# smdogroup/paropt

Hardware: AMD Instinct MI355X
Metric: IP iterations/sec (KKT solve+line search), n=50M vars m=32, 1/2/4/8 GPUs (higher is better)
Workload: dtype f64

## Files before the change

paropt_amd/csrc/capi.cpp:

```cpp
#include <string.h>

#include "ip.hpp"
#include "problem.hpp"
#include "qn.hpp"

namespace po {
const char *last_error();
int ctx_create(int device, Ctx **out);
int ctx_destroy(Ctx *c);
int rccl_unique_id(void *id128);
int comm_init_rccl(Ctx *c, int rank, int size, const void *id128);
int comm_bench(Ctx *c, int count, int pure_sum, int reps, double out_us[3]);
int comm_allreduce_host(Ctx *c, double *values, int count, int op);
int rccl_version();
int comm_init_callback(Ctx *c, int rank, int size, po_allgather_fn fn, void *user);
}

using namespace po;

#define PO_CHECK_PTR(p)                         \
  do {                                          \
    if (!(p)) {                                 \
      po::set_error("null argument: %s", #p);   \
      return PO_ERR_ARG;                        \
// ... 927 lines not shown
  PO_CHECK_PTR(ip);
  return ip->ip->setQuasiNewton(qn ? qn->qn : nullptr);
}
int po_ip_reset_problem_instance(po_ip ip, po_problem prob) {
  PO_CHECK_PTR(ip);
  PO_CHECK_PTR(prob);
  return ip->ip->resetProblemInstance(prob->p);
}
int po_ip_get_hvec_count(po_ip ip, int *nhvec) {
  PO_CHECK_PTR(ip);
  PO_CHECK_PTR(nhvec);
  *nhvec = ip->ip->nhvec;
  return PO_OK;
}
int po_ip_reset_design_and_bounds(po_ip ip) {
  PO_CHECK_PTR(ip);
  return ip->ip->resetDesignAndBounds();
}
int po_ip_reset_quasi_newton(po_ip ip) {
  PO_CHECK_PTR(ip);
  ip->ip->resetQuasiNewtonHessian();
  return PO_OK;
}
int po_ip_get_quasi_newton(po_ip ip, po_qn *qn) {
  PO_CHECK_PTR(ip);
  PO_CHECK_PTR(qn);
  *qn = ip->ip->qn ? &ip->ip->qn_handle : nullptr;
  return PO_OK;
}
int po_ip_write_solution_file(po_ip ip, const char *filename) {
  PO_CHECK_PTR(ip);
  PO_CHECK_PTR(filename);
  return ip->ip->writeSolutionFile(filename);
}
int po_ip_read_solution_file(po_ip ip, const char *filename) {
  PO_CHECK_PTR(ip);
  PO_CHECK_PTR(filename);
  return ip->ip->readSolutionFile(filename);
}
int po_ip_set_iteration_callback(po_ip ip, po_ip_iteration_fn fn, void *user) {
  PO_CHECK_PTR(ip);
  ip->ip->iter_cb = fn;
  ip->ip->iter_cb_user = user;
  return PO_OK;
}
int po_ip_get_history(po_ip ip, const char **text) {
  PO_CHECK_PTR(ip);
  *text = ip->ip->history.c_str();
  return PO_OK;
}
int po_ip_set_callback_timing(po_ip ip, int on) {
  PO_CHECK_PTR(ip);
  ip->ip->user_timing = on != 0;
  return PO_OK;
}
int po_ip_get_phase_times(po_ip ip, const char **names, const double **seconds, int *count) {
  PO_CHECK_PTR(ip);
  InteriorPoint *p = ip->ip;
  p->phase_names_joined.clear();
  for (size_t i = 0; i < p->phase_names.size(); i++) {
    if (i) p->phase_names_joined += ";";
    p->phase_names_joined += p->phase_names[i];
  }
  if (names) *names = p->phase_names_joined.c_str();
  if (seconds) *seconds = p->phase_seconds.data();
  if (count) *count = (int)p->phase_seconds.size();
  return PO_OK;
}
int po_ip_get_debug_ints(po_ip ip, const int **gpiv, int *ngpiv, int *check_flag, int64_t clamped[8]) {
  PO_CHECK_PTR(ip);
  InteriorPoint *p = ip->ip;
  if (gpiv) *gpiv = p->gPivots().data();
  if (ngpiv) *ngpiv = (int)p->gPivots().size();
  if (check_flag) *check_flag = p->checkFlag();
  if (clamped) {
    double out[8];
    PO_TRY(p->clampCounts(out));
    for (int i = 0; i < 8; i++) clamped[i] = (int64_t)(out[i] + 0.5);
  }
  return PO_OK;
}
int po_ip_get_bounds(po_ip ip, po_vec *lb, po_vec *ub) {
  PO_CHECK_PTR(ip);
  if (lb) *lb = static_cast<po_vec>(ip->ip->lowerBounds());
  if (ub) *ub = static_cast<po_vec>(ip->ip->upperBounds());
  return PO_OK;
}
int po_ip_debug_kkt_step(po_ip ip, double mu, po_vec *px, po_vec *pzl, po_vec *pzu,
                         const double **pz, const double **ps, const double **pt,
                         const double **pzs, const double **pzt) {
  PO_CHECK_PTR(ip);
  InteriorPoint *p = ip->ip;
  PO_TRY(p->debugKKTStep(mu));
  if (px) *px = static_cast<po_vec>(p->px);
  if (pzl) *pzl = static_cast<po_vec>(p->pzl);
  if (pzu) *pzu = static_cast<po_vec>(p->pzu);
  if (pz) *pz = p->step.z.data();
  if (ps) *ps = p->step.s.data();
  if (pt) *pt = p->step.t.data();
  if (pzs) *pzs = p->step.zs.data();
  if (pzt) *pzt = p->step.zt.data();
  return PO_OK;
}

int po_ip_debug_set_state(po_ip ip, const double *z, const double *s, const double *t, const double *zs,
                          const double *zt, double mu) {
  PO_CHECK_PTR(ip);
  InteriorPoint *p = ip->ip;
  if (p->c > 0) {
    PO_CHECK_PTR(z);
    PO_CHECK_PTR(s);
    PO_CHECK_PTR(t);
    PO_CHECK_PTR(zs);
    PO_CHECK_PTR(zt);
  }
  return p->debugSetState(z, s, t, zs, zt, mu);
}
int po_ip_debug_kkt(po_ip ip, double mu, int mode, double tau, po_ip_kkt_dump *out) {
  PO_CHECK_PTR(ip);
  PO_CHECK_PTR(out);
  InteriorPoint *p = ip->ip;
  if (mode < 0 || mode > 2) return PO_ERR_ARG;
  PO_TRY(p->debugKKT(mu, mode, tau));
  memset(out, 0, sizeof(*out));
  out->c = p->c;
  out->k = (int)p->cPivots().size();
  out->Dinv = static_cast<po_vec>(p->dinvVec());
  out->res_x = static_cast<po_vec>(p->rxVec());
  out->res_z = p->res.z.data();
  out->res_s = p->res.s.data();
  out->res_t = p->res.t.data();
  out->res_zs = p->res.zs.data();
  out->res_zt = p->res.zt.data();
  for (int i = 0; i < 4; i++) out->res_norms[i] = p->debug_norms[i];
  out->W = p->gramMatrix().data();
  out->G = p->Gmat0.data();
  out->Ce = p->Ce0.data();
  out->gpiv = p->gPivots().data();
  out->cpiv = p->cPivots().data();
  out->px = static_cast<po_vec>(p->px);
  out->pzl = static_cast<po_vec>(p->pzl);
  out->pzu = static_cast<po_vec>(p->pzu);
  out->pz = p->step.z.data();
  out->ps = p->step.s.data();
  out->pt = p->step.t.data();
  out->pzs = p->step.zs.data();
  out->pzt = p->step.zt.data();
  out->step_mins[0] = p->stepMins()[0];
  out->step_mins[1] = p->stepMins()[1];
  return PO_OK;
}

int po_ip_debug_kkt_step_sparse(po_ip ip, po_vec *pzw, po_vec *psw, po_vec *ptw, po_vec *pzsw, po_vec *pztw) {
  PO_CHECK_PTR(ip);
  InteriorPoint *p = ip->ip;
  po_vec *out[5] = {pzw, psw, ptw, pzsw, pztw};
  for (int i = 0; i < 5; i++) {
    if (out[i]) *out[i] = p->has_w ? static_cast<po_vec>(p->wstepv[i]) : nullptr;
  }
  return PO_OK;
}

static int gather_ptrs(po_vec ref, const po_vec *vecs, int nvecs, std::vector<const double *> &p) {
  p.resize(nvecs > 0 ? nvecs : 1);
  for (int j = 0; j < nvecs; j++) {
    PO_CHECK_PTR(vecs[j]);
// ... 128 lines not shown
```

paropt_amd/csrc/context.cpp:

```cpp
#include <dlfcn.h>
#include <math.h>
#include <stdarg.h>
#include <execinfo.h>
#include <stdio.h>
#include <stdlib.h>
#include <string.h>
#include <time.h>

#include <algorithm>

#include "core.hpp"

namespace po {

static thread_local char g_err[1024] = "";
thread_local int g_last_code = 0;

void set_error(const char *fmt, ...) {
  va_list ap;
  va_start(ap, fmt);
  vsnprintf(g_err, sizeof(g_err), fmt, ap);
  va_end(ap);
  fprintf(stderr, "paropt_amd: %s\n", g_err);
}
const char *last_error() { return g_err; }

static int g_dbg_switch[SW_COUNT] = {-1, -1, -1, -1, -1, -1, -1, -1, -1, -1, -1, -1, -1, -1, -1, -1, -1};
double host_now() {
  struct timespec t;
  clock_gettime(CLOCK_MONOTONIC, &t);
  return (double)t.tv_sec + 1e-9 * (double)t.tv_nsec;
}
int dbg_switch(int id, const char *env, int dflt) {
  if (id >= 0 && id < SW_COUNT && g_dbg_switch[id] >= 0) return g_dbg_switch[id];
  const char *e = env ? getenv(env) : nullptr;
  return e ? atoi(e) : dflt;
}
void dbg_switch_set(int id, int value) {
  if (id >= 0 && id < SW_COUNT) g_dbg_switch[id] = value;
}

int launch_reduce_final(Ctx *c, int nblocks, int nslots, int nsum, int nmin, int dst_off);
int launch_reduce_final_multi(Ctx *c, const Ctx::PendingRed *pend, int count);
int launch_red_publish(Ctx *c, const double *src, int count);
static int alloc_h_red(Ctx *c, size_t doubles) {
  if (c->h_red) (void)hipHostFree(c->h_red);
  c->h_red = nullptr;
  c->h_red_dev = nullptr;
  if (hipHostMalloc((void **)&c->h_red, sizeof(double) * doubles, hipHostMallocMapped | hipHostMallocCoherent) !=
      hipSuccess) {
    (void)hipGetLastError();
    c->h_red = nullptr;
    PO_HIP(hipHostMalloc((void **)&c->h_red, sizeof(double) * doubles, hipHostMallocDefault));
    c->h_red_coherent = 0;
  } else {
    c->h_red_coherent = 1;
  }
  if (getenv("PAROPT_AMD_NO_DIRECT_RED") ||
      hipHostGetDevicePointer((void **)&c->h_red_dev, c->h_red, 0) != hipSuccess) {
    (void)hipGetLastError();
    c->h_red_dev = nullptr;
  }
  if (c->h_flag && (!c->h_red_coherent || !c->h_red_dev)) {
    (void)hipHostFree(c->h_flag);
    c->h_flag = c->h_flag_dev = nullptr;
    if (c->d_ticket) (void)hipFree(c->d_ticket);
    c->d_ticket = nullptr;
  }
  if (c->h_red_dev && !c->h_flag && c->h_red_coherent && !getenv("PAROPT_AMD_NO_FLAG_POLL")) {
    if (hipHostMalloc((void **)&c->h_flag, 64, hipHostMallocMapped | hipHostMallocCoherent) == hipSuccess &&
        hipHostGetDevicePointer((void **)&c->h_flag_dev, c->h_flag, 0) == hipSuccess &&
        hipMalloc((void **)&c->d_ticket, sizeof(unsigned)) == hipSuccess &&
        hipMemset(c->d_ticket, 0, sizeof(unsigned)) == hipSuccess) {
      *c->h_flag = 0;
    } else {
      (void)hipGetLastError();
      if (c->h_flag) (void)hipHostFree(c->h_flag);
      if (c->d_ticket) (void)hipFree(c->d_ticket);
      c->h_flag = c->h_flag_dev = nullptr;
      c->d_ticket = nullptr;
    }
  }
  return PO_OK;
}


static int comm_self_test(Ctx *c);
static void free_overflow(Ctx *c, const double *keep);

struct Id128 {
  char b[PO_RCCL_ID_BYTES];
};
struct RcclApi {
  void *handle = nullptr;
  int (*GetUniqueId)(void *) = nullptr;
  int (*CommInitRank)(void **, int, Id128, int) = nullptr;
  int (*AllGather)(const void *, void *, size_t, int, void *, hipStream_t) = nullptr;
  int (*AllReduce)(const void *, void *, size_t, int, int, void *, hipStream_t) = nullptr;
  int (*CommDestroy)(void *) = nullptr;
  const char *(*GetErrorString)(int) = nullptr;
  int (*GetVersion)(int *) = nullptr;
  int version = 0;
};
static RcclApi g_rccl;

static int load_rccl() {
  if (g_rccl.handle) return PO_OK;
  const char *names[] = {getenv("PAROPT_AMD_RCCL_LIB"), "librccl.so", "librccl.so.1", "/opt/rocm/lib/librccl.so"};
  void *h = nullptr;
  for (const char *nm : names) {
// ... 432 lines not shown
  out_us[2] = t.back();
  return PO_OK;
}

int comm_allreduce_host(Ctx *c, double *values, int count, int op) {
  if (count < 0 || count > kMaxRed || op < 0 || op > 2) {
    set_error("po_ctx_allreduce: count %d (max %d) / op %d out of range", count, kMaxRed, op);
    return PO_ERR_ARG;
  }
  if (count == 0 || c->comm_kind == COMM_SELF) return PO_OK;
  PO_TRY(batch_flush(c));
  memcpy(c->h_red, values, sizeof(double) * count);
  PO_HIP(hipMemcpyAsync(c->d_red, c->h_red, sizeof(double) * count, hipMemcpyHostToDevice, c->stream));
  const double *parts = nullptr;
  int nparts = 1;
  PO_TRY(exchange_reduced(c, count, op == 0, &parts, &nparts));
  std::vector<double> out((size_t)count);
  combine_segment(parts, nparts, count, 0, op == 0 ? count : 0, op == 1 ? count : 0, op == 2 ? count : 0, out.data());
  memcpy(values, out.data(), sizeof(double) * count);
  return PO_OK;
}

static void combine_segment(const double *parts, int nparts, int stride, int off, int nsum, int nmin, int nmax,
                            double *host_out) {
  const int nslots = nsum + nmin + nmax;
  for (int s = 0; s < nslots; s++) {
    double acc = parts[off + s];
    for (int r = 1; r < nparts; r++) {
      const double v = parts[(size_t)r * stride + off + s];
      if (s < nsum) {
        acc += v;
      } else if (s < nsum + nmin) {
        acc = fmin(acc, v);
      } else {
        acc = fmax(acc, v);
      }
    }
    host_out[s] = acc;
  }
}

void batch_abort(Ctx *c) {
  if (!c->partials_overflow.empty()) {
    (void)hipStreamSynchronize(c->stream);
    free_overflow(c, nullptr);
  }
  c->batch_pend.clear();
  c->batch_after.clear();
  c->batch_cursor = 0;
  c->partials_cursor = 0;
  c->mdot_timing_pending = false;
}

int batch_flush(Ctx *c, const double *keep_partials, size_t keep_len) {
  size_t cursor0 = 0;
  if (keep_partials && keep_partials >= c->partials_base && keep_partials < c->partials_base + c->partials_cap)
    cursor0 = (size_t)(keep_partials - c->partials_base) + keep_len;
  if (c->batch_pend.empty()) {
    std::vector<std::function<void()>> after;
    after.swap(c->batch_after);
    for (auto &f : after) f();
    return PO_OK;
  }
  std::vector<Ctx::PendingRed> pend;
  pend.swap(c->batch_pend);
  std::vector<std::function<void()>> after;
  after.swap(c->batch_after);
  const int total = c->batch_cursor;
  c->batch_cursor = 0;
  c->partials_cursor = cursor0;
  PO_TRY(launch_reduce_final_multi(c, pend.data(), (int)pend.size()));
  bool pure_sum = true;
  for (const Ctx::PendingRed &p : pend) pure_sum = pure_sum && p.nmin == 0 && p.nmax == 0;
  const double *parts = nullptr;
  int nparts = 1;
  PO_TRY(exchange_reduced(c, total, pure_sum, &parts, &nparts));
  c->n_batched += (long)pend.size() - 1;
  for (const Ctx::PendingRed &p : pend) combine_segment(parts, nparts, total, p.off, p.nsum, p.nmin, p.nmax, p.host_out);
  if (!c->partials_overflow.empty()) free_overflow(c, keep_partials);
  for (auto &f : after) f();
  return PO_OK;
}

int reduce_finish(Ctx *c, int nblocks, int nsum, int nmin, int nmax, double *host_out, bool now) {
  const int nslots = nsum + nmin + nmax;
  if (nslots > kMaxRed) {
    set_error("reduction of %d slots exceeds kMaxRed=%d", nslots, kMaxRed);
    return PO_ERR_ARG;
  }
  const bool queued = c->batch_depth > 0 || !c->batch_pend.empty();
  const double *part = c->d_partials;
  if (queued && c->batch_cursor + nslots > kMaxRed) {
    const size_t len = c->partials_last;
    PO_TRY(batch_flush(c, part, len));
    if (part >= c->partials_base && part < c->partials_base + c->partials_cap) {
      const size_t end = (size_t)(part - c->partials_base) + len;
      if (c->partials_cursor < end) c->partials_cursor = end;
    }
  }
  if (c->batch_depth > 0 || !c->batch_pend.empty()) {
    c->batch_pend.push_back(Ctx::PendingRed{c->batch_cursor, nsum, nmin, nmax, host_out, part, nblocks});
    c->batch_cursor += nslots;
    if (now || c->batch_depth == 0) return batch_flush(c);
    return PO_OK;
  }
  PO_TRY(launch_reduce_final(c, nblocks, nslots, nsum, nmin, 0));
  const double *parts = nullptr;
  int nparts = 1;
  PO_TRY(exchange_reduced(c, nslots, nmin == 0 && nmax == 0, &parts, &nparts));
  combine_segment(parts, nparts, nslots, 0, nsum, nmin, nmax, host_out);
  return PO_OK;
}

}
```

paropt_amd/csrc/core.hpp:

```cpp
#pragma once
#include <hip/hip_runtime.h>
#include <stdint.h>

#include <functional>
#include <string>
#include <vector>

#include "../../include/paropt_amd.h"

namespace po {

void set_error(const char *fmt, ...);
extern thread_local int g_last_code;

#define PO_HIP(expr)                                                                     \
  do {                                                                                   \
    hipError_t _e = (expr);                                                              \
    if (_e != hipSuccess) {                                                              \
      po::set_error("%s failed: %s (%s:%d)", #expr, hipGetErrorString(_e), __FILE__,     \
                    __LINE__);                                                           \
      return PO_ERR_HIP;                                                                 \
    }                                                                                    \
  } while (0)

// ... 15 lines not shown
  hipStream_t stream = nullptr;
  int num_cu = 256;
  int max_blocks = 2048;
  int rank = 0, size = 1;
  CommKind comm_kind = COMM_SELF;
  void *rccl_comm = nullptr;
  int rccl_allreduce = 1;
  long n_allreduce = 0, n_allgather = 0;
  po_allgather_fn cb_allgather = nullptr;
  void *cb_user = nullptr;
  double *d_partials = nullptr;
  double *partials_base = nullptr;
  size_t partials_cap = 0;
  size_t partials_cursor = 0;
  size_t partials_last = 0;
  double *d_red = nullptr;
  double *d_gather = nullptr;
  double *h_red = nullptr;
  double *h_red_dev = nullptr;
  unsigned long long *h_flag = nullptr, *h_flag_dev = nullptr;
  unsigned *d_ticket = nullptr;
  unsigned long long red_seq = 0, red_seq_seen = 0;
  int h_red_coherent = 0;
  long n_flag_waits = 0, n_flag_timeouts = 0;
  bool host_trace = false, host_gap_open = false;
  double host_t_sync = 0.0, host_gap_s = 0.0, host_launch_s = 0.0, host_wait_s = 0.0;
  long host_gap_n = 0, host_launch_n = 0, host_gap_n20 = 0, host_gap_long_n = 0;
  double host_gap_long_s = 0.0, host_t_launch_end = 0.0, host_inter_s = 0.0, host_inter_s30 = 0.0;
  long host_inter_n = 0, host_inter_n30 = 0;
  std::vector<double *> partials_overflow;
  hipEvent_t ev0 = nullptr, ev1 = nullptr;
  double *wide_scratch[2] = {nullptr, nullptr};
  int64_t wide_n = 0;
  hipEvent_t ev_mdot0 = nullptr, ev_mdot1 = nullptr;
  long n_reductions = 0;
  struct PendingRed {
    int off, nsum, nmin, nmax;
    double *host_out;
    const double *part;
    int nblocks;
  };
  int batch_enabled = 1;
  int batch_depth = 0;
  int batch_cursor = 0;
  std::vector<PendingRed> batch_pend;
  std::vector<std::function<void()>> batch_after;
  long n_batched = 0;
  long n_launches = 0;
  double alg_bytes = 0.0, alg_bytes_user = 0.0;
  int in_user = 0;
  int time_mdot_nv = 0;
  double mdot_ms = 0.0;
  long mdot_count = 0;
  bool mdot_timing_pending = false;
  int time_wgram = 0;
  double wgram_ms[2] = {0.0, 0.0};
  long wgram_count[2] = {0, 0};
  int wgram_cols[2] = {0, 0};
  double wgram_bytes[2] = {0.0, 0.0};
};

struct Vec {
  Ctx *ctx;
  int64_t n;
  double *d;
  int ref;
  double *h;
  int h_live = 0;
};

struct PtrTable {
  const double *p[kMaxPanel];
};
struct CoefTable {
  double a[kMaxPanel];
};
constexpr int kMaxVirt = 12;
struct VirtCols {
  const double *s[kMaxVirt];
  int count;
  double b0;
};

int reduce_finish(Ctx *c, int nblocks, int nsum, int nmin, int nmax, double *host_out, bool now = false);
bool red_direct(const Ctx *c);
int batch_flush(Ctx *c, const double *keep_partials = nullptr, size_t keep_len = 0);
void batch_abort(Ctx *c);
template <class F>
inline void after_reduce(Ctx *c, F &&f) {
  if (c->batch_depth > 0 && !c->batch_pend.empty()) {
    c->batch_after.emplace_back(std::forward<F>(f));
  } else {
    f();
  }
}
struct BatchScope {
  Ctx *c;
  bool open;
  explicit BatchScope(Ctx *c_, bool on = true) : c(c_), open(on && c_->batch_enabled) {
    if (open) c->batch_depth++;
  }
  void begin() {
    if (!open && c->batch_enabled) {
      open = true;
      c->batch_depth++;
    }
  }
  int end() {
    if (!open) return PO_OK;
    open = false;
    c->batch_depth--;
    return batch_flush(c);
  }
  int end_nested() {
    if (!open) return PO_OK;
    open = false;
    c->batch_depth--;
    return c->batch_depth > 0 ? PO_OK : batch_flush(c);
  }
  template <class F>
  int end_then(F &&post) {
    if (open) {
      open = false;
      c->batch_depth--;
      if (c->batch_depth > 0) {
        after_reduce(c, std::forward<F>(post));
        return PO_OK;
      }
      PO_TRY(batch_flush(c));
    }
    post();
    return PO_OK;
  }
  ~BatchScope() {
    if (open) {
      c->batch_depth--;
      batch_abort(c);
    }
  }
  BatchScope(const BatchScope &) = delete;
  BatchScope &operator=(const BatchScope &) = delete;
};
enum DbgSwitch { SW_WGRAM_RS = 0, SW_LINCOMB_2D = 1, SW_REDO_DT = 2, SW_LEAN_STEP = 3, SW_WGRAM_PRIO = 4,
                 SW_WGRAM_ABLATE = 5, SW_FUSED_MERIT = 6, SW_REDO_DT1 = 7, SW_BPC3 = 8, SW_BPC4 = 9, SW_LINCOMB_BPC = 10,
                 SW_PERTURB_W = 11, SW_GS_PRODUCER = 12, SW_S2D_TWO = 13, SW_MPC_FUSE = 14, SW_MPC_POLY = 15, SW_SPEC_DT = 16, SW_COUNT = 17 };
int dbg_switch(int id, const char *env, int dflt);
double host_now();
inline double host_trace_begin(Ctx *c);
inline void host_trace_end(Ctx *c, double t0);
void dbg_switch_set(int id, int value);
int ensure_partials(Ctx *c, size_t doubles);
inline double host_trace_begin(Ctx *c) {
  if (!c->host_trace) return 0.0;
  const double t = host_now();
  if (!c->host_gap_open && c->host_t_launch_end > 0.0) {
    const double g = t - c->host_t_launch_end;
    if (g < 500e-6) {
      c->host_inter_s += g;
      c->host_inter_n++;
      if (g > 30e-6) {
        c->host_inter_n30++;
        c->host_inter_s30 += g;
      }
    }
  }
  if (c->host_gap_open) {
    const double g = t - c->host_t_sync;
    if (g < 500e-6) {
      c->host_gap_s += g;
      c->host_gap_n++;
      if (g > 20e-6) c->host_gap_n20++;
    } else {
      c->host_gap_long_s += g;
      c->host_gap_long_n++;
    }
    c->host_gap_open = false;
  }
  return t;
}
inline void host_trace_end(Ctx *c, double t0) {
  if (!c->host_trace) return;
  c->host_t_launch_end = host_now();
  c->host_launch_s += c->host_t_launch_end - t0;
  c->host_launch_n++;
}
inline void count_bytes(Ctx *c, double streams, int64_t n) {
  const double b = 8.0 * streams * (double)n;
  c->alg_bytes += b;
  if (c->in_user) c->alg_bytes_user += b;
}
constexpr int kBpcPanel = 2;
constexpr int kBpcStream = 4;
int grid_for(Ctx *c, int64_t n);
int grid_for(Ctx *c, int64_t n, int bpc);

struct GroupCol {
  const double *w = nullptr;
  double scale = 0.0;
  unsigned period = 1, nw = 0;
  long long nwcon = 0;
};

struct GroupCols2 {
  GroupCol g[2];
  double ca[2] = {0.0, 0.0}, cb[2] = {0.0, 0.0};
  int count = 0;
};

int k_fill(Ctx *c, double *y, int64_t n, double alpha);
int k_fill_hash(Ctx *c, double *y, int64_t n, uint64_t seed, uint64_t aid, int64_t offset,
                double scale, double shift);
int k_copy(Ctx *c, double *y, const double *x, int64_t n);
int k_sign(Ctx *c, double *y, const double *x, int64_t n);
int k_scale(Ctx *c, double *y, int64_t n, double alpha);
int k_axpy(Ctx *c, double *y, double alpha, const double *x, int64_t n);
int k_panel_axpy(Ctx *c, double *y, double a, const double *x, double b, const double *alpha,
                 const double *const *V, int nv, int64_t n, const GroupCol *ybase = nullptr);
int k_panel_axpy2(Ctx *c, double *y1, double a1, const double *x1, const double *c1, double *y2, double a2,
                  const double *x2, const double *c2, const double *const *V, int nv, int64_t n);
int k_panel_lincomb(Ctx *c, double *const *dst, double a, const double *const *X, double b,
                    const double *const *Y, int nv, int64_t n);
enum Red1 { RED_DOT = 0, RED_SUMSQ = 1, RED_ASUM = 2, RED_AMAX = 3 };
int k_reduce1(Ctx *c, int kind, const double *x, const double *y, int64_t n, double *out);
int k_mdot(Ctx *c, const double *x, const double *const *V, int nv, int64_t n, double *out);
int k_minmax(Ctx *c, const double *x, int64_t n, double out[2]);
int k_stream_launch(Ctx *c, int kind, double *x, double *y, int64_t n);
int k_mdot_launch(Ctx *c, const double *x, const double *const *V, int nv, int64_t n, int *nblocks);
struct GramGroups {
  int64_t nwcon = 0, start = 0;
  int nw = 0, skip = 0;
  double alpha = 1.0;
  int ncols = 0;
  double *const *U = nullptr;
};
int k_wgram(Ctx *c, const double *d, const double *const *V, int nv, int64_t n, double *W,
            const double *const *S = nullptr, double *const *Zout = nullptr, int kpend = 0,
            double b0 = 0.0, int preweighted_last = 0, bool may_defer = false,
            const GramGroups *groups = nullptr, bool *groups_done = nullptr);
int wgram_debug_stamps(double out[8]);
int k_wgram_launch(Ctx *c, const double *d, const double *const *V, int nv, int64_t n,
                   int *nblocks, int *nslots, const double *const *S = nullptr,
                   double *const *Zout = nullptr, int kpend = 0, double b0 = 0.0,
                   int preweighted_last = 0, const GramGroups *groups = nullptr, bool *groups_done = nullptr);

struct Bounds {
  const double *x, *lb, *ub, *zl, *zu;
  double max_bound;
  int use_lower, use_upper;
};
int k_kkt_res(Ctx *c, const Bounds &b, const double *g, const double *const *A, const double *z,
              int nc, double beta_mu, int64_t n, double *rx, double *out, double *yqn = nullptr,
              double beta_mu2 = -1.0, const GroupCol *gcol = nullptr, double gcoef = 0.0);
int k_kkt_res_update(Ctx *c, const Bounds &b, const double *g, const double *const *A, const double *z, int nc,
                     double beta_mu, int64_t n, double *rx, double *out, double *yqn, double *zl,
                     const double *pzl, double *zu, const double *pzu, double a, double eps, const double *va,
                     double az, double *acz, double az_acz,
                     const double *pxs = nullptr, const double *xold = nullptr, double beta_mu_step = 0.0,
                     double beta_mu2 = -1.0,
                     const GroupCol *gcol = nullptr, double gcoef = 0.0,
                     double *dinv_out = nullptr, double *t_out = nullptr, double spec_diag = 0.0,
                     double spec_beta_mu = 0.0);
int k_res_norms(Ctx *c, const Bounds &b, double beta_mu, int64_t n, double out[11]);
int k_dinv(Ctx *c, const Bounds &b, double diag, int64_t n, double *dinv,
           const double *hdiag = nullptr);
int k_d1s(Ctx *c, const Bounds &b, const double *bx, const double *dinv, double alpha, double beta_mu,
          int64_t n, double *t);
int k_solve2s(Ctx *c, const Bounds &b, const double *t, const double *dinv, const double *coef,
              const double *const *P, int nv, double alpha, double beta_mu, int full, double tau, int64_t n,
              double *px, double *pzl, double *pzu, double out[2]);
int k_d1(Ctx *c, const Bounds &b, const double *rx, const double *dinv, double beta_mu, int64_t n,
         double *t, const double *cl = nullptr, const double *cu = nullptr);
int k_dinv_d1(Ctx *c, const Bounds &b, double diag, const double *hdiag, const double *rx, double beta_mu,
              int64_t n, double *dinv, double *t, int raw = 0);
int k_corrector(Ctx *c, const Bounds &b, const double *px, const double *pzl, const double *pzu,
                int64_t n, double *cl, double *cu);
constexpr int kCorrDotsMax = 15;
int k_corr_d1_dots(Ctx *c, const Bounds &b, const double *px, const double *pzl, const double *pzu, const double *rx,
                   const double *dinv, double beta_mu, const double *const *V, int nv, int64_t n, double *t,
                   double *out);
int k_solve2c(Ctx *c, const Bounds &b, const double *t, const double *dinv, const double *alpha,
              const double *const *P, int nv, double beta_mu, double tau, int64_t n, double *px, double *pzl,
              double *pzu, double *va, int nca, const double *g, int want_logs, double out[12]);
int k_solve2(Ctx *c, const Bounds &b, const double *t, const double *dinv, const double *alpha,
             const double *const *P, int nv, double beta_mu, int refine, double tau, int64_t n,
             double *px, double *pzl, double *pzu, double out[2], const double *coef2 = nullptr,
             const double *rx = nullptr, double diag = 0.0, double *tout = nullptr,
             double *va = nullptr, int nca = 0, const double *cl = nullptr,
             const double *cu = nullptr);
int k_solve2_dots(Ctx *c, const Bounds &b, const double *t, const double *dinv, const double *alpha,
                  const double *coef2, const double *const *P, int nv, double beta_mu, double tau,
                  const double *rx, double diag, int64_t n, double *px, double *pzl, double *pzu,
                  double *tout, double *va, int nca, double *out, double *traw = nullptr,
                  int store_step = 1,
                  int ca0 = 0,
                  const double *const *vs = nullptr, int nvirt = 0, double b0v = 0.0,
                  double dinv_diag = 0.0,
                  const GroupCols2 *gcols = nullptr);
int k_solve2r(Ctx *c, const Bounds &b, const double *t1, const double *t2, const double *dinv, const double *a1,
              const double *a2, const double *const *P, int nv, double beta_mu, double tau, int64_t n, double *px,
              double *pzl, double *pzu, double *va, int nca, double out[2], const double *ar = nullptr,
              const double *rx = nullptr, double diag = 0.0,
              int ca0 = 0,
              const double *const *vs = nullptr, int nvirt = 0, double b0v = 0.0,
              const double *g = nullptr, double *merit_out = nullptr,
              double dinv_diag = 0.0,
              const GroupCol *gcol = nullptr, double gc1 = 0.0, double gc2 = 0.0);
int k_form_pz(Ctx *c, const Bounds &b, const double *px, double beta_mu, int64_t n, double *pzl, double *pzu);
int k_update_mult_yqn(Ctx *c, double *zl, const double *pzl, double *zu, const double *pzu, double a,
                      double eps, int use_lower, int use_upper, const double *rx, const double *va,
                      double az, int64_t n, double *yqn, double *acz = nullptr);
int k_res_step(Ctx *c, const Bounds &b, const double *rx, const double *px, const double *pzl,
               const double *pzu, const double *dinv, const double *coef, const double *const *P,
               int nv, double diag, double beta_mu, int64_t n, double *tprime);
int k_step_check(Ctx *c, const Bounds &b, const double *rx, const double *px, const double *pzl, const double *pzu,
                 const double *coef, const double *const *P, int nv, double diag, double beta_mu, int64_t n,
                 double out[3]);
int k_comp_step(Ctx *c, const Bounds &b, const double *px, const double *pzl, const double *pzu,
                double ax, double az, int64_t n, double out[2]);
int k_comp_merit(Ctx *c, const Bounds &b, const double *px, const double *pzl, const double *pzu, double ax,
                 double az, const double *g, int64_t n, double out[9]);
int k_merit0(Ctx *c, const Bounds &b, const double *px, double sx, const double *g, int64_t n,
             double out[6]);
int k_trial(Ctx *c, const Bounds &b, const double *px, double a, double eps, int64_t n, double *xt,
            double out[2], double *sout = nullptr);
int k_update_mult(Ctx *c, double *zl, const double *pzl, double *zu, const double *pzu, double a,
                  double eps, int use_lower, int use_upper, int64_t n);
int k_affine_mult(Ctx *c, const Bounds &b, double *zl, const double *pzl, double *zu,
                  const double *pzu, double amin, int64_t n);
int k_check_bounds(Ctx *c, double *x, double *lb, double *ub, double *zl, double *zu,
                   double max_bound, double rel_bound, int both, int64_t n, int *flag);
int k_bounds_mode(Ctx *c, double *x, double *lb, double *ub, int mode, int64_t offset, int64_t n);
int k_clamp_count(Ctx *c, const double *x, const double *lb, const double *ub, const double *zl, const double *zu,
                  double eps, int64_t n, double out[4]);
int k_zero_inactive(Ctx *c, const double *lb, const double *ub, double *zl, double *zu,
                    double max_bound, int64_t n);

int k_quadratic_f(Ctx *c, const double *q, const double *b, const double *x, int64_t n, double *f);
int k_quadratic_g(Ctx *c, const double *q, const double *b, const double *x, int64_t n, double *g);
int k_convex_f(Ctx *c, const double *b, const double *x, int64_t n, double *f);
int k_convex_g(Ctx *c, const double *b, const double *x, int64_t n, double *g);
int k_rosen_f(Ctx *c, const double *x, int64_t n, double out[3]);
int k_rosen_g(Ctx *c, const double *x, int64_t n, double *g, double *a0, double *a1);
int k_sep_hess(Ctx *c, int kind, const double *q, const double *b, const double *x, const double *px,
               int64_t n, double *h);
int k_rosen_hess(Ctx *c, const double *x, double z0, const double *px, int64_t n, double *h);

int lu_factor(int n, double *A, int lda, int *piv);
void lu_solve(int n, const double *A, int lda, const int *piv, double *b);

}

struct po_ctx_s : po::Ctx {};
struct po_vec_s : po::Vec {};
```

paropt_amd/csrc/ip.cpp:

```cpp
#include "ip.hpp"

#include <math.h>
#include <stdio.h>
#include <stdlib.h>
#include <string.h>

#include <algorithm>
#include <chrono>

namespace po {

static const int LS_SUCCESS = 1, LS_FAILURE = 2, LS_MIN_STEP = 4, LS_MAX_ITERS = 8,
                 LS_NO_IMPROVEMENT = 16, LS_SHORT_STEP = 32;

InteriorPoint::InteriorPoint(Problem *p)
    : prob(p), ctx(p->ctx), n(p->nlocal), c(p->ncon), qn(nullptr), x(nullptr), zl(nullptr),
      zu(nullptr), lb(nullptr), ub(nullptr), g(nullptr), fobj(0.0), barrier_param(0.1),
      rho_penalty_search(0.0), niter(0), neval(0), ngeval(0), analytic_panel_dots(true),
      iter_cb(nullptr),
      iter_cb_user(nullptr), px(nullptr), pzl(nullptr), pzu(nullptr), Dinv(nullptr), rx(nullptr),
      tvec(nullptr), xt(nullptr), y_qn(nullptr), s_qn(nullptr), vA(nullptr), qn_created(false), qn_owned(true), wk(0),
      comp_prod(0), comp_count(0), max_rx(0), max_rzl(0), max_rzu(0), sx(1.0), sz(1.0),
      ptpx_valid(false), residual_fused(false), residual_cached(false), corrector_active(false),
      norm_type(0), tdots_valid(false), fused_dots(true), phase_t0(0) {
// ... 68 lines not shown
    vec_decref(wresv[i]);
    vec_decref(wstepv[i]);
    vec_decref(wscalev[i]);
  }
  for (Vec *v : Uw) vec_decref(v);
  for (Vec *v : gmresW) vec_decref(v);
  vec_decref(hdiag);
  if (qn_owned) delete qn;
  if (user_events_ready)
    for (int i = 0; i < 2 * kUserRing; i++) (void)hipEventDestroy(user_ev[i]);
}

void InteriorPoint::setPenaltyGamma(double gamma) {
  if (gamma < 0.0) return;
  gamma_s.assign(c, gamma);
  gamma_t.assign(c, gamma);
  for (int i = 0; i < c && i < prob->ninequality; i++) gamma_s[i] = 0.0;
  if (has_w) k_w_gamma(ctx, gsw->d, gtw->d, gamma, prob->nwinequality, nw);
}

int InteriorPoint::setQuasiNewton(CompactQuasiNewton *qn_) {
  if (qn_owned) delete qn;
  qn = qn_;
  qn_owned = false;
  qn_created = true;
  qn_handle.qn = qn;
  return PO_OK;
}

int InteriorPoint::resetProblemInstance(Problem *p) {
  if (p->nlocal != prob->nlocal || p->ncon != prob->ncon || p->nwcon != prob->nwcon ||
      p->ninequality != prob->ninequality || p->nwinequality != prob->nwinequality) {
    set_error("ParOpt: Incompatible problem instance");
    return PO_ERR_ARG;
  }
  prob = p;
  ac_valid = false;
  acz_valid = false;
  cwx_valid = false;
  return PO_OK;
}

void InteriorPoint::setPenaltyGammaArray(const double *gamma) {
  for (int i = 0; i < c; i++) {
    if (gamma[i] >= 0.0) {
      gamma_s[i] = i < prob->ninequality ? 0.0 : gamma[i];
      gamma_t[i] = gamma[i];
    }
  }
}

int InteriorPoint::createQuasiNewton() {
  if (qn_created) return PO_OK;
  qn_created = true;
  const std::string qt = options.str("qn_type");
  const int msub = options.integer("qn_subspace_size");
  if (qt == "bfgs") {
    LBFGS *b = new LBFGS(ctx, n, msub);
    b->setBFGSUpdateType(std::string(options.str("qn_update_type")) == "damped_update"
                             ? PO_BFGS_DAMPED_UPDATE
                             : PO_BFGS_SKIP_NEGATIVE_CURVATURE);
    qn = b;
  } else if (qt == "sr1") {
    qn = new LSR1(ctx, n, msub);
  }
  if (qn) {
    const std::string dt = options.str("qn_diag_type");
    qn->setInitDiagonalType(dt == "yts_over_sts" ? PO_QN_YTS_OVER_STS : PO_QN_YTY_OVER_YTS);
  }
  qn_handle.qn = qn;
  return PO_OK;
}

Bounds InteriorPoint::bounds() const {
  Bounds b;
  b.x = x->d;
  b.lb = lb->d;
  b.ub = ub->d;
  b.zl = zl->d;
  b.zu = zu->d;
  b.max_bound = options.real("max_bound_value");
  b.use_lower = use_lower;
  b.use_upper = use_upper;
  return b;
}

std::vector<const double *> InteriorPoint::panel(bool use_qn, int *k) const {
  std::vector<const double *> p;
  for (Vec *a : Ac) p.push_back(a->d);
  *k = 0;
  if (qn && use_qn) {
    std::vector<const double *> z = qn->zPointers();
    *k = (int)z.size();
    p.insert(p.end(), z.begin(), z.end());
  }
  return p;
}

void InteriorPoint::phaseBegin() {
  phase_t0 = std::chrono::duration<double>(std::chrono::steady_clock::now().time_since_epoch()).count();
}
void InteriorPoint::phaseEnd(const char *name) {
  const double t1 =
      std::chrono::duration<double>(std::chrono::steady_clock::now().time_since_epoch()).count();
  for (size_t i = 0; i < phase_names.size(); i++) {
    if (phase_names[i] == name) {
      phase_seconds[i] += t1 - phase_t0;
      phase_t0 = t1;
      return;
    }
  }
  phase_names.push_back(name);
  phase_seconds.push_back(t1 - phase_t0);
  phase_t0 = t1;
}

void InteriorPoint::userBegin() {
  ctx->in_user = 1;
  if (!user_timing) return;
  if (!user_events_ready) {
    for (int i = 0; i < 2 * kUserRing; i++)
      if (hipEventCreate(&user_ev[i]) != hipSuccess) return;
    user_events_ready = true;
  }
  if (user_pending == kUserRing) userHarvest();
  (void)hipEventRecord(user_ev[2 * user_pending], ctx->stream);
}
void InteriorPoint::userEnd() {
  ctx->in_user = 0;
  if (!user_timing || !user_events_ready) return;
  (void)hipEventRecord(user_ev[2 * user_pending + 1], ctx->stream);
  user_pending++;
}
void InteriorPoint::userHarvest() {
  for (int i = 0; i < user_pending; i++) {
    float ms = 0.0f;
    if (hipEventSynchronize(user_ev[2 * i + 1]) == hipSuccess &&
        hipEventElapsedTime(&ms, user_ev[2 * i], user_ev[2 * i + 1]) == hipSuccess)
      user_seconds += 1e-3 * ms;
  }
  user_pending = 0;
}

int InteriorPoint::initAndCheckDesignAndBounds() {
  int rc = prob->getVarsAndBounds(x, lb, ub);
  if (rc != 0) {
    set_error("getVarsAndBounds failed with code %d", rc);
    return PO_ERR_USER;
  }
  const double rel_bound = 0.001 * barrier_param;
  int flag = 0;
  PO_TRY(k_check_bounds(ctx, x->d, lb->d, ub->d, zl->d, zu->d, options.real("max_bound_value"),
                        rel_bound, use_lower && use_upper, n, &flag));
  check_flag |= flag;
  if (ctx->rank == 0) {
    if (flag & 1) history += "ParOpt Warning: Variable bounds are inconsistent\n";
    if (flag & 2) history += "ParOpt Warning: Variables may be too close to lower bound\n";
    if (flag & 4) history += "ParOpt Warning: Variables may be too close to upper bound\n";
  }
  return PO_OK;
}

int InteriorPoint::clampCounts(double out[8]) {
  const double eps = options.real("design_precision");
  PO_TRY(k_clamp_count(ctx, x->d, lb->d, ub->d, use_lower ? zl->d : nullptr, use_upper ? zu->d : nullptr, eps, n,
                       out));
  for (int j = 4; j < 8; j++) out[j] = 0.0;
  for (int i = 0; i < c; i++) {
    if (vars.s[i] == eps) out[4] += 1.0;
    if (vars.t[i] == eps) out[5] += 1.0;
    if (vars.zs[i] == eps) out[6] += 1.0;
    if (vars.zt[i] == eps) out[7] += 1.0;
  }
  return PO_OK;
}

static int refreshLiveMirror(Vec *v) {
  if (!v || !v->h_live || !v->h || v->n <= 0) return PO_OK;
  PO_HIP(hipMemcpyAsync(v->h, v->d, sizeof(double) * (size_t)v->n, hipMemcpyDeviceToHost, v->ctx->stream));
  PO_HIP(hipStreamSynchronize(v->ctx->stream));
  return PO_OK;
}

int InteriorPoint::resetDesignAndBounds() {
  cwx_valid = false;
  int rc = prob->getVarsAndBounds(x, lb, ub);
  if (rc != 0) return PO_ERR_USER;
  PO_TRY(refreshLiveMirror(x));
  PO_TRY(refreshLiveMirror(lb));
  return refreshLiveMirror(ub);
}

void InteriorPoint::resetQuasiNewtonHessian() {
  if (qn) qn->reset();
}

int InteriorPoint::initLeastSquaresMultipliers() {
  acz_valid = false;
  const double mu0 = options.real("init_barrier_param");
  PO_TRY(k_fill(ctx, zl->d, n, mu0));
  PO_TRY(k_fill(ctx, zu->d, n, mu0));
  for (int i = 0; i < c; i++) vars.z[i] = vars.s[i] = vars.t[i] = vars.zs[i] = vars.zt[i] = mu0;
  PO_TRY(k_zero_inactive(ctx, lb->d, ub->d, zl->d, zu->d, options.real("max_bound_value"), n));
  if (has_w) return initLeastSquaresMultipliersW();
  if (c == 0) return PO_OK;
  const double small = 1e-4;
  PO_TRY(k_fill(ctx, Dinv->d, n, 1.0));
  int k = 0;
  std::vector<const double *> A = panel(false, &k);
  std::vector<double> G((size_t)c * c, 0.0);
  PO_TRY(k_wgram(ctx, Dinv->d, A.data(), c, n, G.data()));
  for (int i = 0; i < c; i++) G[(size_t)i * (c + 1)] += small;
  std::vector<int> piv(c);
  lu_factor(c, G.data(), c, piv.data());
  const double al[2] = {1.0, -1.0};
  const double *vv[2] = {zl->d, zu->d};
  PO_TRY(k_panel_axpy(ctx, tvec->d, -1.0, g->d, 0.0, al, vv, 2, n));
  std::vector<double> z(c, 0.0);
  PO_TRY(k_mdot(ctx, tvec->d, A.data(), c, n, z.data()));
  for (int i = 0; i < c; i++) z[i] = -z[i];
  lu_solve(c, G.data(), c, piv.data(), z.data());
  for (int i = 0; i < c; i++) {
    const double gam = 10.0 * std::max(gamma_s[i], gamma_t[i]);
    vars.z[i] = (z[i] < -gam || z[i] > gam) ? 0.0 : z[i];
  }
  return PO_OK;
}

int InteriorPoint::initAffineStepMultipliers() {
  const double amin = options.real("start_affine_multiplier_min");
  PO_TRY(initLeastSquaresMultipliers());
  PO_TRY(k_zero_inactive(ctx, lb->d, ub->d, zl->d, zu->d, options.real("max_bound_value"), n));
  PO_TRY(computeResidual(0.0, true));
  bool use_qn = !(options.integer("sequential_linear_method") ||
                  !options.integer("use_qn_gmres_precon") || options.integer("use_diag_hessian"));
  if (options.integer("use_diag_hessian")) PO_TRY(ensureHdiag());
  PO_TRY(setUpKKTSystem(use_qn));
  denseResidual(0.0, res);
  if (has_w) {
    PO_TRY(solveKKTW(res, 0.0, use_qn, false, 1.0, step));
    PO_TRY(k_w_affine(ctx, wv(), wp(), amin, nw));
  } else {
    PO_TRY(solveKKT(res, 0.0, use_qn, false, 1.0, step));
  }
  acz_valid = false;
  for (int i = 0; i < c; i++) {
    vars.z[i] = vars.z[i] + step.z[i];
    vars.s[i] = std::max(amin, fabs(vars.s[i] + step.s[i]));
    vars.t[i] = std::max(amin, fabs(vars.t[i] + step.t[i]));
    vars.zs[i] = std::max(amin, fabs(vars.zs[i] + step.zs[i]));
    vars.zt[i] = std::max(amin, fabs(vars.zt[i] + step.zt[i]));
  }
  PO_TRY(k_affine_mult(ctx, bounds(), zl->d, pzl->d, zu->d, pzu->d, amin, n));
  double comp = 0.0;
  PO_TRY(getComplementarity(&comp));
  barrier_param = comp;
  return PO_OK;
}

void InteriorPoint::denseResidual(double mu, Dense &r) const {
  for (int i = 0; i < c; i++) {
    r.z[i] = -(cvals[i] - vars.s[i] + vars.t[i]);
    r.s[i] = -(gamma_s[i] - vars.zs[i] + vars.z[i]);
    r.t[i] = -(gamma_t[i] - vars.zt[i] - vars.z[i]);
    r.zs[i] = -(vars.s[i] * vars.zs[i] - mu);
    r.zt[i] = -(vars.t[i] * vars.zt[i] - mu);
  }
}
// ... 607 lines not shown
    r2.resize(c);
    denseResidual(mu, r2);
    for (int i = 0; i < c; i++) {
      r2.z[i] -= (dots[i] - step.s[i] + step.t[i]);
      r2.s[i] += (step.zs[i] - step.z[i]);
      r2.t[i] += (step.zt[i] + step.z[i]);
      r2.zs[i] -= (step.s[i] * vars.zs[i] + vars.s[i] * step.zs[i]);
      r2.zt[i] -= (step.t[i] * vars.zt[i] + vars.t[i] * step.zt[i]);
    }
    PO_TRY(solveKKT(r2, mu, use_qn, true, tau, refine));
    for (int i = 0; i < c; i++) {
      step.z[i] += refine.z[i];
      step.s[i] += refine.s[i];
      step.t[i] += refine.t[i];
      step.zs[i] += refine.zs[i];
      step.zt[i] += refine.zt[i];
    }
  }
  sx = sz = 1.0;
  return PO_OK;
}

int InteriorPoint::checkKKTStep(int iteration, double mu) {
  const double beta_mu = options.real("rel_bound_barrier") * mu;
  if (!pz_stored) {
    PO_TRY(k_form_pz(ctx, bounds(), px->d, step_beta_mu, n, pzl->d, pzu->d));
    pz_stored = true;
  }
  const bool seq_lin = options.integer("sequential_linear_method");
  int kq = 0;
  std::vector<const double *> Pq = panel(qn && !seq_lin, &kq);
  const int mq = c + kq;
  std::vector<double> dots(mq > 0 ? mq : 1, 0.0), coef(mq > 0 ? mq : 1, 0.0);
  if (mq > 0) PO_TRY(k_mdot(ctx, px->d, Pq.data(), mq, n, dots.data()));
  for (int i = 0; i < c; i++) coef[i] = step.z[i];
  double diag = options.real("qn_sigma");
  if (qn && !seq_lin && !options.integer("use_diag_hessian")) {
    diag += qn->diag();
    if (kq > 0) {
      std::vector<double> rz(dots.begin() + c, dots.begin() + c + kq);
      qn->applyCompactInverse(rz.data());
      for (int j = 0; j < kq; j++) coef[c + j] = rz[j];
    }
  }
  if (has_w) {
    if (prob->setSparseJacobianTranspose(1.0, x, wstepv[0], xt) != 0) return PO_ERR_USER;
    Pq.push_back(xt->d);
    coef.push_back(1.0);
  }
  double mx[3];
  PO_TRY(computeResidual(mu, true));
  PO_TRY(k_step_check(ctx, bounds(), rx->d, px->d, pzl->d, pzu->d, coef.data(), Pq.data(), (int)Pq.size(), diag,
                      beta_mu, n, mx));
  Dense r;
  r.resize(c);
  denseResidual(mu, r);
  double mz = 0.0, ms = 0.0, mt = 0.0, mzs = 0.0, mzt = 0.0;
  for (int i = 0; i < c; i++) {
    mz = std::max(mz, fabs(r.z[i] - (dots[i] - step.s[i] + step.t[i])));
    ms = std::max(ms, fabs(r.s[i] + (step.zs[i] - step.z[i])));
    mt = std::max(mt, fabs(r.t[i] + (step.zt[i] + step.z[i])));
    mzs = std::max(mzs, fabs(r.zs[i] - (step.s[i] * vars.zs[i] + vars.s[i] * step.zs[i])));
    mzt = std::max(mzt, fabs(r.zt[i] - (step.t[i] * vars.zt[i] + vars.t[i] * step.zt[i])));
  }
  if (ctx->rank == 0) {
    char line[640];
    snprintf(line, sizeof(line),
             "\nResidual step check for iteration %d:\n"
             "max |stationarity (x block)|:             %10.4e\n"
             "max |dense constraints (z block)|:        %10.4e\n"
             "max |slack duals (s block)|:              %10.4e\n"
             "max |slack duals (t block)|:              %10.4e\n"
             "max |slack complementarity (zs block)|:   %10.4e\n"
             "max |slack complementarity (zt block)|:   %10.4e\n"
             "max |lower-bound complementarity (zl)|:   %10.4e\n"
             "max |upper-bound complementarity (zu)|:   %10.4e\n",
             iteration, mx[0], mz, ms, mt, mzs, mzt, mx[1], mx[2]);
    history += line;
  }
  return PO_OK;
}

int InteriorPoint::checkGradients(double dh, std::string *report) {
  return prob->checkGradients(dh, x, options.integer("use_hvec_product"), xt, tvec, report);
}

int InteriorPoint::checkMeritFuncGradient(Vec *xpt, double dh, double out[2]) {
  if (xpt) PO_TRY(k_copy(ctx, x->d, xpt->d, n));
  cwx_valid = false;
  if (prob->evalObjCon(x, &fobj, cvals.data()) != 0) {
    fprintf(stderr, "ParOpt: Function and constraint evaluation failed\n");
    return PO_ERR_USER;
  }
  neval++;
  if (prob->evalObjConGradient(x, g, Ac.data()) != 0) {
    fprintf(stderr, "ParOpt: Gradient evaluation failed\n");
    return PO_ERR_USER;
  }
  ngeval++;
  ac_valid = true;
  acz_valid = false;
  if (!pz_stored) {
    pz_stored = true;
  }
  if (xpt) {
    double g2 = 0.0;
    PO_TRY(k_reduce1(ctx, RED_SUMSQ, g->d, nullptr, n, &g2));
    PO_TRY(k_panel_axpy(ctx, px->d, g2 > 0.0 ? -1.0 / sqrt(g2) : 0.0, g->d, 0.0, nullptr, nullptr, 0, n));
    for (int i = 0; i < c; i++) {
      step.s[i] = -0.259 * (1 + (i % 3));
      step.t[i] = -0.349 * (4 - (i % 2));
    }
    if (has_w && nw > 0) {
      std::vector<double> hs((size_t)nw), ht((size_t)nw);
      for (int64_t i = 0; i < nw; i++) {
        hs[i] = -0.419 * (1 + (i % 5));
        ht[i] = -0.7513 * (1 + (i % 19));
      }
      PO_HIP(hipMemcpyAsync(wstepv[1]->d, hs.data(), sizeof(double) * (size_t)nw, hipMemcpyHostToDevice, ctx->stream));
      PO_HIP(hipMemcpyAsync(wstepv[2]->d, ht.data(), sizeof(double) * (size_t)nw, hipMemcpyHostToDevice, ctx->stream));
      PO_HIP(hipStreamSynchronize(ctx->stream));
    }
  }
  sx = sz = 1.0;
  ptpx_valid = false;
  merit_cache_valid = false;
  fused_merit_valid = false;
  w_comp_valid = w_merit_cache_valid = false;
  px_amax_valid = false;
  double m0 = 0.0, dm0 = 0.0;
  PO_TRY(evalMeritInitDeriv(1.0, &m0, &dm0));
  const double eps = 0.0;
  double sums[2], wsums[5];
  std::vector<double> rs(c), rt(c), cs(cvals);
  for (int i = 0; i < c; i++) {
    rs[i] = vars.s[i] + dh * step.s[i];
    rt[i] = vars.t[i] + dh * step.t[i];
  }
  {
    PO_TRY(k_trial(ctx, bounds(), px->d, dh, eps, n, xt->d, sums));
    trial_logs_valid = false;
    s_qn_from_trial = false;
  }
  double ftemp = 0.0;
  if (prob->evalObjCon(xt, &ftemp, cs.data()) != 0) {
    fprintf(stderr, "ParOpt: Function and constraint evaluation failed\n");
    return PO_ERR_USER;
  }
  neval++;
  if (has_w) {
    if (prob->evalSparseCon(xt, wtmp) != 0) return PO_ERR_USER;
    PO_TRY(k_w_trial(ctx, wv(), wp(), dh, eps, gsw->d, gtw->d, wtmp->d, nw, wsums));
  }
  const double m1 = evalMeritFromSums(ftemp, cs.data(), rs.data(), rt.data(), sums[0], sums[1], has_w ? wsums : nullptr);
  const double fd = (m1 - m0) / dh;
  if (ctx->rank == 0) {
    fprintf(stdout, "Merit function test\n");
    fprintf(stdout, "dm FD: %15.8e  Actual: %15.8e  Err: %8.2e  Rel err: %8.2e\n", fd, dm0, fabs(fd - dm0),
            fabs((fd - dm0) / fd));
    fflush(stdout);
  }
  if (out) {
    out[0] = fd;
    out[1] = dm0;
  }
  return PO_OK;
// ... 757 lines not shown
  const bool seq_lin = options.integer("sequential_linear_method");
  const double min_frac = options.real("min_fraction_to_boundary");
  const bool use_line_search = options.integer("use_line_search");
  const int write_freq = options.integer("write_output_frequency");
  const int step_verification_frequency = options.integer("step_verification_frequency");
  const int gradient_verification_frequency = options.integer("gradient_verification_frequency");
  const std::string start = options.str("starting_point_strategy");
  niter = neval = ngeval = nhvec = 0;
  cwx_valid = trial_cw_valid = false;
  residual_cached = false;
  iterate_logs_valid = trial_logs_valid = fused_merit_valid = false;
  spec_dt_valid = spec_dt_want = false;
  w_comp_valid = w_merit_cache_valid = false;
  px_first_only = false;
  spec_enabled = spec_valid = false;
  history.clear();
  phase_names.clear();
  phase_seconds.clear();
  user_seconds = 0.0;
  user_pending = 0;
  ac_valid = false;
  acz_valid = false;
  if (!seq_lin && !qn && !use_diag_hessian) {
    if (ctx->rank == 0)
      fprintf(stderr,
              "ParOpt Error: Must use a sequential linear method if no quasi-Newton approximation "
              "is defined\n");
    return 1;
  }
  phaseBegin();
  PO_TRY(initAndCheckDesignAndBounds());
  userBegin();
  int fail_obj = prob->evalObjCon(x, &fobj, cvals.data());
  userEnd();
  neval++;
  if (fail_obj) {
    fprintf(stderr, "ParOpt: Initial function and constraint evaluation failed\n");
    return fail_obj;
  }
  userBegin();
  int fail_g = prob->evalObjConGradient(x, g, Ac.data());
  userEnd();
  ngeval++;
  if (fail_g) {
    fprintf(stderr, "ParOpt: Initial gradient evaluation failed\n");
    return fail_g;
  }
  ac_valid = true;
  if (start == "affine_step") {
    PO_TRY(initAffineStepMultipliers());
  } else if (start == "least_squares_multipliers") {
    PO_TRY(initLeastSquaresMultipliers());
  }
  if (qn && !use_qnu) {
    if (qn->updateMult(x, vars.z.data(), has_w ? wvar[0] : nullptr) != 0) return PO_ERR_USER;
  }
  phaseEnd("init");

  double fobj_prev = 0.0, alpha_prev = 0.0, alpha_xprev = 0.0, alpha_zprev = 0.0, dm0_prev = 0.0;
  double res_norm_prev = 0.0;
  int no_merit_function_improvement = 0, line_search_test = 0, line_search_failed = 0;
  char info[64];
  memset(info, 0, sizeof(info));
  char line[512];

  for (int k = 0; k < max_major_iters; k++, niter++) {
    int qn_hessian_reset = 0;
    if (qn && !seq_lin) {
      if (k > 0 && k % hessian_reset_freq == 0 && use_qnu) {
        qn->reset();
        qn_hessian_reset = 1;
      }
    }
    if (write_freq > 0 && k % write_freq == 0) {
      if (checkpoint) {
        if (writeSolutionFile(checkpoint) != PO_OK) checkpoint = nullptr;
      }
      prob->writeOutput(k, x);
    }
    if (iter_cb) iter_cb(iter_cb_user, k);
    if (gradient_verification_frequency > 0 && (k % gradient_verification_frequency) == 0) {
      std::string rep;
      PO_TRY(prob->checkGradients(options.real("gradient_check_step_length"), x, use_hvec_product, xt, tvec, &rep));
      if (ctx->rank == 0) history += rep;
    }

    const bool rel_function_test =
        (alpha_xprev == 1.0 && alpha_zprev == 1.0 && (fabs(fobj - fobj_prev) < rel_func_tol * fabs(fobj_prev)));
    if (no_merit_function_improvement) {
      line_search_test += 1;
    } else {
      line_search_test = 0;
    }
    double max_prime = 0.0, max_dual = 0.0, max_infeas = 0.0, res_norm = 0.0;
    int monotone_barrier_converged = 0;
    double comp = 0.0;
    spec_enabled = barrier_strategy == B_MONOTONE && norm_type == 0 && !has_w && !use_hvec_product;
    if (barrier_strategy == B_MONOTONE) {
      if (!residual_cached) PO_TRY(computeResidual(barrier_param, true));
      residual_cached = false;
      comp = compFromSums(comp_prod, comp_count, vars, w_sums[0]);
      denseResidual(barrier_param, res);
      resNorms(res, &max_prime, &max_dual, &max_infeas, &res_norm);
      if (k > 0 && ((res_norm < 10.0 * barrier_param) || rel_function_test || (line_search_test >= 2))) {
        monotone_barrier_converged = 1;
      }
      if (monotone_barrier_converged) {
        if (barrier_param > 0.1 * abs_res_tol) line_search_test = 0;
        const double mu_frac = options.real("monotone_barrier_fraction") * barrier_param;
        const double mu_pow = pow(barrier_param, options.real("monotone_barrier_power"));
        double new_mu = mu_frac;
        if (mu_pow < mu_frac) new_mu = mu_pow;
        if (new_mu < 0.1 * abs_res_tol) new_mu = 0.09999 * abs_res_tol;
        if (spec_valid && spec_mu == new_mu && norm_type == 0) {
          max_rzl = spec_max[0];
          max_rzu = spec_max[1];
          spec_valid = false;
        } else {
          PO_TRY(computeResidual(new_mu, false));
        }
        denseResidual(new_mu, res);
        resNorms(res, &max_prime, &max_dual, &max_infeas, &res_norm);
        rho_penalty_search = options.real("min_rho_penalty_search");
        barrier_param = new_mu;
      }
    } else if (barrier_strategy == B_MEHROTRA || barrier_strategy == B_MPC) {
      if (!residual_cached) PO_TRY(computeResidual(barrier_param, true));
      residual_cached = false;
      comp = compFromSums(comp_prod, comp_count, vars, w_sums[0]);
      denseResidual(barrier_param, res);
      resNorms(res, &max_prime, &max_dual, &max_infeas, &res_norm);
    } else {
      if (!residual_cached) PO_TRY(computeResidual(barrier_param, true));
      residual_cached = false;
      comp = compFromSums(comp_prod, comp_count, vars, w_sums[0]);
      barrier_param = options.real("monotone_barrier_fraction") * comp;
      if (barrier_param < 0.1 * abs_res_tol) barrier_param = 0.1 * abs_res_tol;
      PO_TRY(computeResidual(barrier_param, false));
      denseResidual(barrier_param, res);
      resNorms(res, &max_prime, &max_dual, &max_infeas, &res_norm);
    }
    phaseEnd("residual");

    if (ctx->rank == 0) {
      if (k == 0 || options.integer("output_level") > 0) {
        const char *inform = prob->sparseFactorInfo();
        if (inform) history += std::string("MatInfo: ") + inform + "\n";
      }
      if (k % 10 == 0) {
        snprintf(line, sizeof(line),
                 "\n%4s %4s %4s %4s %7s %7s %7s %12s %7s %7s %7s %7s %7s %8s %7s info\n", "iter",
                 "nobj", "ngrd", "nhvc", "alpha", "alphx", "alphz", "fobj", "|opt|", "|infes|",
                 "|dual|", "mu", "comp", "dmerit", "rho");
        history += line;
      }
      if (k == 0) {
        snprintf(line, sizeof(line),
                 "%4d %4d %4d %4d %7s %7s %7s %12.5e %7.1e %7.1e %7.1e %7.1e %7.1e %8s %7s %s\n", k,
                 neval, ngeval, nhvec, "--", "--", "--", fobj, max_prime, max_infeas, max_dual,
                 barrier_param, comp, "--", "--", info);
      } else {
        snprintf(line, sizeof(line),
                 "%4d %4d %4d %4d %7.1e %7.1e %7.1e %12.5e %7.1e %7.1e %7.1e %7.1e %7.1e %8.1e %7.1e %s\n",
                 k, neval, ngeval, nhvec, alpha_prev, alpha_xprev, alpha_zprev, fobj, max_prime,
                 max_infeas, max_dual, barrier_param, comp, dm0_prev, rho_penalty_search, info);
      }
// ... 389 lines not shown
```

paropt_amd/csrc/ip.hpp:

```cpp
#pragma once
#include <stdlib.h>
#include <map>
#include <string>
#include <vector>

#include "problem.hpp"
#include "qn.hpp"

namespace po {

class Options {
 public:
  enum Type { STR = 1, BOOL = 2, INT = 3, FLOAT = 4, ENUM = 5 };
  struct Entry {
    Type type;
    std::string s;
    int i = 0, ilo = 0, ihi = 0;
    double f = 0, flo = 0, fhi = 0;
    std::vector<std::string> choices;
  };
  Options();
  void addTrustRegionDefaults();
  void addMMADefaults();
  int set(const char *name, const char *value);
  int set(const char *name, int value);
  int set(const char *name, double value);
  const char *str(const char *name) const;
  int integer(const char *name) const;
  double real(const char *name) const;
  bool has(const char *name) const { return e.count(name) > 0; }
  int visit(const Options *skip, po_option_visitor fn, void *user) const;
  void adoptExtras(const Options &src, const Options &base);

 private:
  std::map<std::string, Entry> e;
};

struct Dense {
  std::vector<double> z, s, t, zs, zt;
  void resize(int c) {
    z.assign(c, 0.0);
    s.assign(c, 0.0);
    t.assign(c, 0.0);
    zs.assign(c, 0.0);
    zt.assign(c, 0.0);
  }
};

class InteriorPoint {
 public:
  InteriorPoint(Problem *prob);
  ~InteriorPoint();
  int allocate();
  const std::vector<int> &gPivots() const { return gpiv; }
  Vec *lowerBounds() { return lb; }
  Vec *upperBounds() { return ub; }
  int checkFlag() const { return check_flag; }
  int clampCounts(double out[8]);
  int checkKKTStep(int iteration, double mu);

  Options options;
  int optimize(const char *checkpoint);
  void getOptimizedPoint(Vec **x, const double **z, Vec **zl, Vec **zu);
  void getOptimizedSlacks(const double **s, const double **t, const double **zs, const double **zt);
  void getOptimizedSparse(Vec *v[5]);
  void getIterationCounters(int *niter_, int *neval_, int *ngeval_);
  double getBarrierParameter() const { return barrier_param; }
  int getComplementarity(double *comp);
  void setPenaltyGamma(double gamma);
  void setPenaltyGammaArray(const double *gamma);
  int resetDesignAndBounds();
  void resetQuasiNewtonHessian();
  int setQuasiNewton(CompactQuasiNewton *qn_);
  int resetProblemInstance(Problem *p);
  int writeSolutionFile(const char *filename);
  int readSolutionFile(const char *filename);
  int debugKKTStep(double mu);
  int debugSetState(const double *z, const double *s, const double *t, const double *zs, const double *zt, double mu);
  int debugKKT(double mu, int mode, double tau);
  std::vector<double> Gmat0, Ce0;
  bool debug_keep_schur = false;
  double debug_norms[4] = {0, 0, 0, 0};
  const std::vector<double> &gramMatrix() const { return W; }
  const std::vector<int> &cPivots() const { return cpiv; }
  const double *stepMins() const { return step_mins; }
  Vec *dinvVec() { return Dinv; }
  Vec *rxVec() { return rx; }
  void flushHistory();
  int checkGradients(double dh, std::string *report);
  int checkMeritFuncGradient(Vec *xpt, double dh, double out[2]);

  Problem *prob;
  Ctx *ctx;
  int64_t n;
  int c;
  CompactQuasiNewton *qn;
  po_qn_s qn_handle;

  Vec *x, *zl, *zu, *lb, *ub, *g;
  std::vector<Vec *> Ac;
  Dense vars, res, step, refine;
  double fobj, barrier_param, rho_penalty_search;
  std::vector<double> cvals;
  int niter, neval, ngeval, nhvec;

  bool analytic_panel_dots;
  po_ip_iteration_fn iter_cb;
  void *iter_cb_user;
  std::string history;
  std::vector<std::string> phase_names;
  std::vector<double> phase_seconds;
  std::string phase_names_joined;
  bool user_timing = getenv("PAROPT_AMD_USER_TIMING") != nullptr;

  Vec *px, *pzl, *pzu;

  int64_t nw;
  bool has_w;
  double nw_global;
  Vec *wvar[5], *wresv[5], *wstepv[5];

 private:
  Vec *Dinv, *rx, *tvec, *xt, *y_qn, *s_qn;
  Vec *vA;
  std::vector<double> gamma_s, gamma_t;
  int use_lower, use_upper;
  bool qn_created;
  bool qn_owned;

  std::vector<double> W;
  int wk;
  std::vector<double> Gf, Cef;
  std::vector<int> gpiv, cpiv;
  double comp_prod, comp_count, max_rx, max_rzl, max_rzu;
  double l1_rx = 0, l1_rzl = 0, l1_rzu = 0, l2_rx = 0, l2_rzl = 0, l2_rzu = 0;
  double sx, sz;
  double step_mins[2];
  std::vector<double> ptpx;
  bool ptpx_valid;
// ... 27 lines not shown
  double trial_logs[2] = {0, 0}, iterate_logs[2] = {0, 0};
  bool trial_logs_valid = false, iterate_logs_valid = false;
  int gatherCounts(int64_t mine, std::vector<int64_t> *all);
  int solutionFileOffsets(int64_t *nvars_total, int64_t *var_off, int64_t *nw_total, int64_t *w_off);
  int ensureHdiag();
  int solveKKTAlpha(const double *bx, double alpha, const Dense &b, double mu, bool use_qn, bool full,
                    double tau, Dense &out);
  int evalObjBarrierDeriv(const Dense &p, double *pmerit);
  int solveKKTAlphaW(const double *bx, double alpha, const Dense &b, double mu, bool use_qn, bool full,
                     double tau, Dense &out);
  Vec *wscalev[5];
  double w_merit_last[10];
  int computeKKTGMRESStep(double rtol, double atol, bool use_qn, double tau, int *gmres_iters);

  Vec *gsw, *gtw, *Cw, *wd2, *wyw, *wtmp, *wtmp2;
  Vec *cwx = nullptr;
  bool cwx_valid = false, trial_cw_valid = false;
  int sparseConAtIterate(const double **cw);
  Vec *d1v;
  std::vector<Vec *> Uw;
  bool panel_plain = false;
  bool panel_valid = false;
  double w_sums[7], w_maxs[5];
  double res_out[13] = {0}, wres_out[12] = {0};
  bool spec_mu_on = true, spec_enabled = false, spec_valid = false;
  double spec_mu = 0.0, spec_max[2] = {0.0, 0.0};
  double nextMonotoneMu() const;
  WVars wv() const;
  WVars wr() const;
  WVars wp() const;
  int allocateW();
  int applyK0(const double *bx, const double *bw, Vec *yx, Vec *yw);
  int computeResidualW(double mu, bool norms = true, bool with_d2 = false);
  bool wd2_ready = false;
  int sparseGramCorrection(const std::vector<const double *> &P, int m, Vec *work = nullptr, bool may_defer = false,
                           bool panel_done = false);
  int panelImageVectors(int m, std::vector<double *> &U);
  int solveKKTW(const Dense &b, double mu, bool use_qn, bool refine_pass, double tau, Dense &out,
                bool fuse_residual = false);
  int computeKKTStepWithRefinementW(double mu, bool use_qn, double tau);
  int initLeastSquaresMultipliersW();
  int wCompStep(double ax, double az, double *prod);

  Bounds bounds() const;
  std::vector<const double *> panel(bool use_qn, int *k) const;

  int createQuasiNewton();
  int initAndCheckDesignAndBounds();
  int initLeastSquaresMultipliers();
  int initAffineStepMultipliers();
  void denseResidual(double mu, Dense &r) const;
  struct MultUpdate {
    double a = 0.0, az = 0.0, eps = 0.0;
    bool acz_follow = false;
  };
  int computeResidual(double mu, bool vectors, Vec *yqn_complete = nullptr, const MultUpdate *upd = nullptr);
  void resNorms(const Dense &r, double *max_prime, double *max_dual, double *max_infeas,
                double *res_norm) const;
  double compFromSums(double prod, double count, const Dense &v, double wprod = 0.0) const;
  int setUpKKTSystem(bool use_qn, bool diag_only = false, const double *rhs_mu = nullptr);
  int solveKKT(const Dense &b, double mu, bool use_qn, bool refine_pass, double tau, Dense &out,
               bool fuse_residual = false);
  int computeKKTStepWithRefinement(double mu, bool use_qn, double tau);
  int mehrotraStep(bool use_qn, double comp, bool corrector, double min_frac, double abs_res_tol, double *tau_out);
  int scaleKKTStep(double tau, double comp, double *alpha_x, double *alpha_z, int *ceq,
                   bool inexact = false);
  int evalMeritInitDeriv(double max_x, double *merit, double *pmerit);
  double evalMeritFromSums(double fk, const double *ck, const double *sk, const double *tk,
                           double pos, double neg, const double *wsums = nullptr) const;
  int lineSearch(double alpha_min, double *alpha, double m0, double dm0, int *fail);
  int computeStepAndUpdate(double alpha, int eval_obj_con, int perform_qn_update, int *update_type);
  void phaseBegin();
  void phaseEnd(const char *name);
  double phase_t0;
  static const int kUserRing = 16;
  hipEvent_t user_ev[2 * kUserRing];
  int user_pending = 0;
  bool user_events_ready = false;
  double user_seconds = 0.0;
  void userBegin();
  void userEnd();
  void userHarvest();
  int check_flag = 0;
  bool ac_valid = false;
  static const int kAczRefresh = 16;
  Vec *acz = nullptr;
  bool acz_valid = false, use_acz = true, use_ztpx_hint = true;
  int acz_age = 0;
  bool fuse_mult_update = true;
  bool fast_yqn_w = true;
  bool w_lean = true, px_first_only = false;
  double w_step_out[5] = {0, 0, 0, 0, 0}, w_comp_poly[3] = {0, 0, 0}, w_merit_cache[10] = {0};
  bool w_comp_valid = false, w_merit_cache_valid = false;
  bool s_qn_from_trial = false;
  double s_qn_a = 0.0;
  bool recompute_first_step = true, step_deferred = false;
  std::vector<double> alpha_first, coef_first;
  double diag_first = 0.0;
  bool recompute_rhs = true;
  bool virtual_z = true, virt_first = false, allow_virtual_z = false;
  bool fused_tdots = true, t0_valid = false;
  double t0_mu = 0.0;
  std::vector<double> t0dots;
};

}

struct po_ip_s {
  po::InteriorPoint *ip;
};
```

paropt_amd/csrc/kernels.hip:

```cpp
#include "core.hpp"

#include <math.h>
#include <stdlib.h>

namespace po {

#define PO_PAIR_LOOP(q, n)                                                                 \
  const int64_t _npairs = ((n) + 1) >> 1;                                                  \
  for (int64_t q = (int64_t)blockIdx.x * blockDim.x + threadIdx.x; q < _npairs;            \
       q += (int64_t)gridDim.x * blockDim.x)

typedef double f64x2l __attribute__((ext_vector_type(2)));
__device__ __forceinline__ double2 ld2(const double *__restrict__ p, int64_t q, int64_t n) {
#ifndef PO_LD2_PLAIN
  const f64x2l v = __builtin_nontemporal_load(reinterpret_cast<const f64x2l *>(p + 2 * q));
  return make_double2(v.x, v.y);
#else
  return *reinterpret_cast<const double2 *>(p + 2 * q);
#endif
}
#ifndef PO_ST2_PLAIN
#define PO_ST2_NT 1
#endif
typedef double f64x2s __attribute__((ext_vector_type(2)));
__device__ __forceinline__ void st2(double *__restrict__ p, int64_t q, int64_t n, double2 v) {
  if (2 * q + 1 >= n) v.y = 0.0;
#ifdef PO_ST2_NT
  __builtin_nontemporal_store((f64x2s){v.x, v.y}, reinterpret_cast<f64x2s *>(p + 2 * q));
#else
  *reinterpret_cast<double2 *>(p + 2 * q) = v;
#endif
}

typedef double f64x4 __attribute__((ext_vector_type(4)));
typedef double f64x2 __attribute__((ext_vector_type(2)));

__device__ __forceinline__ f64x2 ld_stream(const double *p) {
  return __builtin_nontemporal_load(reinterpret_cast<const f64x2 *>(p));
}

enum { OP_SUM = 0, OP_MIN = 1, OP_MAX = 2 };

template <int OP>
__device__ __forceinline__ double combine(double a, double b) {
  if (OP == OP_SUM) return a + b;
  if (OP == OP_MIN) return fmin(a, b);
  return fmax(a, b);
}

template <int OP>
__device__ __forceinline__ double wave_reduce(double v) {
#pragma unroll
  for (int o = 32; o > 0; o >>= 1) v = combine<OP>(v, __shfl_xor(v, o, 64));
  return v;
}

template <int N, int OP>
__device__ __forceinline__ void block_reduce_store(double (&a)[N], double *__restrict__ partials,
                                                   int slot0, double *sm) {
  const int lane = threadIdx.x & 63, wave = threadIdx.x >> 6;
#pragma unroll
  for (int j = 0; j < N; j++) {
    double v = wave_reduce<OP>(a[j]);
    if (lane == 0) sm[wave * N + j] = v;
  }
  __syncthreads();
  if (threadIdx.x < N) {
    const int j = threadIdx.x;
    double v = combine<OP>(combine<OP>(sm[j], sm[N + j]), combine<OP>(sm[2 * N + j], sm[3 * N + j]));
    partials[(size_t)(slot0 + j) * gridDim.x + blockIdx.x] = v;
  }
  __syncthreads();
}

__device__ __forceinline__ void red_raise_flag(volatile unsigned long long *flag, unsigned long long seq,
                                               unsigned *ticket) {
  if (!flag) return;
  __threadfence_system();
  __syncthreads();
  if (threadIdx.x == 0) {
    const unsigned t = atomicAdd(ticket, 1u);
    if (t == gridDim.x - 1) {
      *ticket = 0;
      __threadfence_system();
      *flag = seq;
    }
// ... 702 lines not shown
    set_error("mdot of %d vectors exceeds kMaxPanel=%d", nv, kMaxPanel);
    return PO_ERR_ARG;
  }
  const int grid = grid_for(c, n, 5);
  PO_TRY(ensure_partials(c, (size_t)grid * (nv + 32)));
  PtrTable pt;
  CoefTable ct;
  fill_tables(nullptr, V, nv, &ct, &pt);
  int j0 = 0;
  while (j0 < nv) {
    const int rem = nv - j0;
    const int w = rem >= 32 ? 32 : (rem >= 24 ? 24 : (rem >= 16 ? 16 : rem));
    switch (w) {
      PO_MDOT_CASE(1) PO_MDOT_CASE(2) PO_MDOT_CASE(3) PO_MDOT_CASE(4) PO_MDOT_CASE(5)
      PO_MDOT_CASE(6) PO_MDOT_CASE(7) PO_MDOT_CASE(8) PO_MDOT_CASE(9) PO_MDOT_CASE(10)
      PO_MDOT_CASE(11) PO_MDOT_CASE(12) PO_MDOT_CASE(13) PO_MDOT_CASE(14) PO_MDOT_CASE(15)
      PO_MDOT_CASE(16) PO_MDOT_CASE(24) PO_MDOT_CASE(32)
    }
    j0 += w;
  }
  *nblocks = grid;
  return PO_OK;
}

int k_mdot(Ctx *c, const double *x, const double *const *V, int nv, int64_t n, double *out) {
  if (nv <= 0) return PO_OK;
  if (nv > kMaxPanel) {
    for (int j0 = 0; j0 < nv; j0 += kMaxPanel)
      PO_TRY(k_mdot(c, x, V + j0, nv - j0 > kMaxPanel ? kMaxPanel : nv - j0, n, out + j0));
    return PO_OK;
  }
  int grid = 0;
  const bool timed = c->time_mdot_nv == nv;
  if (timed && c->mdot_timing_pending) PO_TRY(batch_flush(c));
  if (timed) PO_HIP(hipEventRecord(c->ev_mdot0, c->stream));
  PO_TRY(k_mdot_launch(c, x, V, nv, n, &grid));
  if (timed) PO_HIP(hipEventRecord(c->ev_mdot1, c->stream));
  const bool defer = timed && c->batch_depth > 0;
  PO_TRY(reduce_finish(c, grid, nv, 0, 0, out, timed && !defer));
  if (timed) {
    auto harvest = [c] {
      float ms = 0.0f;
      if (hipEventSynchronize(c->ev_mdot1) == hipSuccess &&
          hipEventElapsedTime(&ms, c->ev_mdot0, c->ev_mdot1) == hipSuccess) {
        c->mdot_ms += ms;
        c->mdot_count++;
      }
      c->mdot_timing_pending = false;
    };
    if (defer) c->mdot_timing_pending = true;
    after_reduce(c, harvest);
  }
  return PO_OK;
}


struct BE {
  bool L, U;
  double xl, xu, zl, zu;
};
__device__ __forceinline__ BE bound_elem(double x, double lb, double ub, double zl, double zu,
                                         double maxb, int use_lower, int use_upper) {
  BE e;
  e.L = use_lower && (lb > -maxb);
  e.U = use_upper && (ub < maxb);
  e.xl = e.L ? (x - lb) : 1.0;
  e.xu = e.U ? (ub - x) : 1.0;
  e.zl = zl;
  e.zu = zu;
  return e;
}
#define PO_MAKE_BOUNDS(b, q, n)                                                          \
  const bool _has2 = (2 * q + 1 < n);                                                    \
  const BE e0 = bound_elem(_x.x, _lb.x, _ub.x, _zl.x, _zu.x, (b).max_bound, (b).use_lower, \
                           (b).use_upper);                                               \
  BE e1 = bound_elem(_x.y, _lb.y, _ub.y, _zl.y, _zu.y, (b).max_bound, (b).use_lower,     \
                     (b).use_upper);                                                     \
  if (!_has2) {                                                                          \
    e1.L = false;                                                                        \
    e1.U = false;                                                                        \
    e1.xl = 1.0;                                                                         \
    e1.xu = 1.0;                                                                         \
  }
#define PO_LOAD_BOUNDS(b, q, n)                                                         \
  const double2 _x = ld2((b).x, q, n), _lb = ld2((b).lb, q, n), _ub = ld2((b).ub, q, n), \
                _zl = ld2((b).zl, q, n), _zu = ld2((b).zu, q, n);                        \
  PO_MAKE_BOUNDS(b, q, n)

__device__ __forceinline__ void res_bound_acc(const BE &e, double beta_mu, double *sums, double *maxs,
                                              int il1, int il2, int imax) {
  if (e.L) {
    sums[0] += e.zl * e.xl;
    sums[1] += 1.0;
    const double r = fabs(-(e.xl * e.zl - beta_mu));
    sums[il1] += r;
    sums[il2] += r * r;
    maxs[imax] = fmax(maxs[imax], r);
  }
  if (e.U) {
    sums[0] += e.zu * e.xu;
    sums[1] += 1.0;
    const double r = fabs(-(e.xu * e.zu - beta_mu));
    sums[il1 + 1] += r;
    sums[il2 + 1] += r * r;
    maxs[imax + 1] = fmax(maxs[imax + 1], r);
  }
}
__device__ __forceinline__ void res_bound_max2(const BE &e, double beta_mu2, double *m2) {
  if (e.L) m2[0] = fmax(m2[0], fabs(-(e.xl * e.zl - beta_mu2)));
  if (e.U) m2[1] = fmax(m2[1], fabs(-(e.xu * e.zu - beta_mu2)));
}
__global__ void __launch_bounds__(kBlock)
    kkt_res_kernel(Bounds b, const double *__restrict__ g, PtrTable A, CoefTable z, int nc,
                   double beta_mu, int64_t n, double *__restrict__ rx, double *__restrict__ yqn,
                   double beta_mu2, GroupCol gcol, double gcoef, double *__restrict__ partials) {
  __shared__ double sm[4 * 8];
  double sums[8] = {0.0, 0.0, 0.0, 0.0, 0.0, 0.0, 0.0, 0.0};
  double maxs[5] = {0.0, 0.0, 0.0, 0.0, 0.0};
  PO_PAIR_LOOP(q, n) {
    PO_LOAD_BOUNDS(b, q, n);
    const double2 gv = ld2(g, q, n);
    double2 yv = make_double2(0.0, 0.0);
    if (yqn) yv = ld2(yqn, q, n);
    double2 r;
    r.x = (b.use_lower ? _zl.x : 0.0);
    r.y = (b.use_lower ? _zl.y : 0.0);
    if (b.use_upper) {
      r.x += -1.0 * _zu.x;
      r.y += -1.0 * _zu.y;
    }
    r.x += -1.0 * gv.x;
    r.y += -1.0 * gv.y;
    GRaw graw;
    if (gcol.w) graw = gcol_request(gcol, q, n);
    double2 ps = panel_sum(A, z, nc, q);
    if (gcol.w) {
      const f64x2 gcv = gcol_value(gcol, graw);
      ps.x += gcoef * gcv.x;
      ps.y += gcoef * gcv.y;
    }
    r.x += ps.x;
    r.y += ps.y;
    if (!_has2) r.y = 0.0;
    st2(rx, q, n, r);
    if (yqn) {
      const double cl = b.use_lower ? 1.0 : 0.0, cu = b.use_upper ? -1.0 : 0.0;
      yv.x = __dadd_rn(yv.x, __fma_rn(-1.0, r.x, __fma_rn(cu, _zu.x, __fma_rn(cl, _zl.x, 0.0))));
      yv.y = __dadd_rn(yv.y, __fma_rn(-1.0, r.y, __fma_rn(cu, _zu.y, __fma_rn(cl, _zl.y, 0.0))));
      st2(yqn, q, n, yv);
    }
    maxs[0] = fmax(maxs[0], fmax(fabs(r.x), fabs(r.y)));
    sums[2] += fabs(r.x) + fabs(r.y);
    sums[5] += r.x * r.x + r.y * r.y;
    res_bound_acc(e0, beta_mu, sums, maxs, 3, 6, 1);
    res_bound_acc(e1, beta_mu, sums, maxs, 3, 6, 1);
    if (beta_mu2 >= 0.0) {
      res_bound_max2(e0, beta_mu2, maxs + 3);
      res_bound_max2(e1, beta_mu2, maxs + 3);
    }
  }
  block_reduce_store<8, OP_SUM>(sums, partials, 0, sm);
  if (beta_mu2 >= 0.0) {
    block_reduce_store<5, OP_MAX>(maxs, partials, 8, sm);
  } else {
    double m3[3] = {maxs[0], maxs[1], maxs[2]};
    block_reduce_store<3, OP_MAX>(m3, partials, 8, sm);
  }
}

int k_kkt_res(Ctx *c, const Bounds &b, const double *g, const double *const *A, const double *z,
              int nc, double beta_mu, int64_t n, double *rx, double *out, double *yqn, double beta_mu2,
              const GroupCol *gcol, double gcoef) {
  PO_TRY(gcol_check(gcol, n, "k_kkt_res"));
  if (nc > kMaxPanel) {
    const double *w = nullptr, one = 1.0;
    PO_TRY(collapse_range(c, 0, z, A, 0, nc, n, &w));
    return k_kkt_res(c, b, g, &w, &one, 1, beta_mu, n, rx, out, yqn, beta_mu2, gcol, gcoef);
  }
  count_bytes(c, 7 + nc + (yqn ? 2 : 0), n);
  const int grid = grid_for(c, n, kBpcPanel);
  PO_TRY(ensure_partials(c, (size_t)grid * 13));
  PtrTable pt;
  CoefTable ct;
  fill_tables(z, A, nc, &ct, &pt);
  if (gcol) count_bytes(c, 1.0, gcol->nwcon);
  PO_LAUNCH(kkt_res_kernel, grid, b, g, pt, ct, nc, beta_mu, n, rx, yqn, beta_mu2, gcol ? *gcol : GroupCol(), gcoef,
            c->d_partials);
  return reduce_finish(c, grid, 8, 0, beta_mu2 >= 0.0 ? 5 : 3, out);
}

__global__ void __launch_bounds__(kBlock)
    res_norms_kernel(Bounds b, double beta_mu, int64_t n, double *__restrict__ partials) {
  __shared__ double sm[4 * 8];
  double sums[8] = {0.0, 0.0, 0.0, 0.0, 0.0, 0.0, 0.0, 0.0};
  double maxs[3] = {0.0, 0.0, 0.0};
  PO_PAIR_LOOP(q, n) {
    PO_LOAD_BOUNDS(b, q, n);
    res_bound_acc(e0, beta_mu, sums, maxs, 3, 6, 1);
    res_bound_acc(e1, beta_mu, sums, maxs, 3, 6, 1);
  }
  block_reduce_store<8, OP_SUM>(sums, partials, 0, sm);
  block_reduce_store<3, OP_MAX>(maxs, partials, 8, sm);
}

int k_res_norms(Ctx *c, const Bounds &b, double beta_mu, int64_t n, double out[11]) {
  count_bytes(c, 5, n);
  const int grid = grid_for(c, n);
  PO_TRY(ensure_partials(c, (size_t)grid * 11));
  PO_LAUNCH(res_norms_kernel, grid, b, beta_mu, n, c->d_partials);
  return reduce_finish(c, grid, 8, 0, 3, out);
}

__device__ __forceinline__ double dinv_elem(const BE &e, double diag) {
  double v = diag;
  if (e.L) v += e.zl / e.xl;
  if (e.U) v += e.zu / e.xu;
  return 1.0 / v;
}
__global__ void __launch_bounds__(kBlock)
    dinv_kernel(Bounds b, double diag, const double *__restrict__ hdiag, int64_t n,
                double *__restrict__ dinv) {
  PO_PAIR_LOOP(q, n) {
    PO_LOAD_BOUNDS(b, q, n);
    double2 h = make_double2(0.0, 0.0);
    if (hdiag) h = ld2(hdiag, q, n);
    st2(dinv, q, n, make_double2(dinv_elem(e0, diag + h.x), dinv_elem(e1, diag + h.y)));
  }
}
int k_dinv(Ctx *c, const Bounds &b, double diag, int64_t n, double *dinv, const double *hdiag) {
  count_bytes(c, 6 + (hdiag ? 1 : 0), n);
  if (n <= 0) return PO_OK;
  PO_LAUNCH(dinv_kernel, grid_for(c, n), b, diag, hdiag, n, dinv);
  return PO_OK;
}

__device__ __forceinline__ double d1_elem(const BE &e, double rx, double beta_mu, double cl = 0.0,
                                          double cu = 0.0) {
  double d1 = rx;
  if (e.L) d1 += (-(e.xl * e.zl - beta_mu) - cl) / e.xl;
  if (e.U) d1 -= (-(e.xu * e.zu - beta_mu) + cu) / e.xu;
  return d1;
}
__global__ void __launch_bounds__(kBlock)
    d1_kernel(Bounds b, const double *__restrict__ rx, const double *__restrict__ dinv,
              double beta_mu, const double *__restrict__ cl, const double *__restrict__ cu, int64_t n,
              double *__restrict__ t) {
  PO_PAIR_LOOP(q, n) {
    PO_LOAD_BOUNDS(b, q, n);
    const double2 r = ld2(rx, q, n);
    const double2 dv = dinv ? ld2(dinv, q, n) : make_double2(1.0, 1.0);
    double2 c0 = make_double2(0.0, 0.0), c1 = c0;
    if (cl) {
      c0 = ld2(cl, q, n);
      c1 = ld2(cu, q, n);
    }
    st2(t, q, n,
        make_double2(dv.x * d1_elem(e0, r.x, beta_mu, c0.x, c1.x),
                     dv.y * d1_elem(e1, r.y, beta_mu, c0.y, c1.y)));
  }
}
int k_d1(Ctx *c, const Bounds &b, const double *rx, const double *dinv, double beta_mu, int64_t n,
         double *t, const double *cl, const double *cu) {
  count_bytes(c, 7 + (dinv ? 1 : 0) + (cl ? 2 : 0), n);
  if (n <= 0) return PO_OK;
  PO_LAUNCH(d1_kernel, grid_for(c, n), b, rx, dinv, beta_mu, cl, cu, n, t);
  return PO_OK;
}

__global__ void __launch_bounds__(kBlock)
    dinv_d1_kernel(Bounds b, double diag, const double *__restrict__ hdiag, const double *__restrict__ rx,
                   double beta_mu, int64_t n, double *__restrict__ dinv, double *__restrict__ t, int raw) {
  PO_PAIR_LOOP(q, n) {
    PO_LOAD_BOUNDS(b, q, n);
    double2 h = make_double2(0.0, 0.0);
    if (hdiag) h = ld2(hdiag, q, n);
    const double2 r = ld2(rx, q, n);
    const double2 dv = make_double2(dinv_elem(e0, diag + h.x), dinv_elem(e1, diag + h.y));
    st2(dinv, q, n, dv);
    const double w0 = raw ? 1.0 : dv.x, w1 = raw ? 1.0 : dv.y;
    st2(t, q, n, make_double2(w0 * d1_elem(e0, r.x, beta_mu), w1 * d1_elem(e1, r.y, beta_mu)));
  }
}
int k_dinv_d1(Ctx *c, const Bounds &b, double diag, const double *hdiag, const double *rx, double beta_mu,
              int64_t n, double *dinv, double *t, int raw) {
  count_bytes(c, 8 + (hdiag ? 1 : 0), n);
  if (n <= 0) return PO_OK;
  PO_LAUNCH(dinv_d1_kernel, grid_for(c, n), b, diag, hdiag, rx, beta_mu, n, dinv, t, raw);
  return PO_OK;
}

__global__ void __launch_bounds__(kBlock)
    corrector_kernel(Bounds b, const double *__restrict__ px, const double *__restrict__ pzl,
                     const double *__restrict__ pzu, int64_t n, double *__restrict__ cl,
                     double *__restrict__ cu) {
  PO_PAIR_LOOP(q, n) {
    PO_LOAD_BOUNDS(b, q, n);
    const double2 p = ld2(px, q, n), l = ld2(pzl, q, n), u = ld2(pzu, q, n);
    st2(cl, q, n, make_double2(e0.L ? p.x * l.x : 0.0, e1.L ? p.y * l.y : 0.0));
    st2(cu, q, n, make_double2(e0.U ? p.x * u.x : 0.0, e1.U ? p.y * u.y : 0.0));
  }
}
int k_corrector(Ctx *c, const Bounds &b, const double *px, const double *pzl, const double *pzu,
                int64_t n, double *cl, double *cu) {
  count_bytes(c, 8, n);
  if (n <= 0) return PO_OK;
  PO_LAUNCH(corrector_kernel, grid_for(c, n), b, px, pzl, pzu, n, cl, cu);
  return PO_OK;
}

template <int NVB>
__global__ void __launch_bounds__(kBlock)
    corr_d1_dots_kernel(Bounds b, const double *__restrict__ px, const double *__restrict__ pzl,
                        const double *__restrict__ pzu, const double *__restrict__ rx,
                        const double *__restrict__ dinv, double beta_mu, PtrTable V, int64_t n,
                        double *__restrict__ t, double *__restrict__ partials) {
  __shared__ double sm[4 * NVB];
  double acc[NVB];
  const double *vp[NVB];
#pragma unroll
  for (int j = 0; j < NVB; j++) {
    acc[j] = 0.0;
    vp[j] = V.p[j];
  }
  PO_PAIR_LOOP(q, n) {
    PO_LOAD_BOUNDS(b, q, n);
    const double2 p = ld2(px, q, n), l = ld2(pzl, q, n), u = ld2(pzu, q, n);
    const double2 r = ld2(rx, q, n), dv = ld2(dinv, q, n);
    const double c0x = e0.L ? __dmul_rn(p.x, l.x) : 0.0, c0y = e1.L ? __dmul_rn(p.y, l.y) : 0.0;
    const double c1x = e0.U ? __dmul_rn(p.x, u.x) : 0.0, c1y = e1.U ? __dmul_rn(p.y, u.y) : 0.0;
    double2 tv = make_double2(__dmul_rn(dv.x, d1_elem(e0, r.x, beta_mu, c0x, c1x)),
                              __dmul_rn(dv.y, d1_elem(e1, r.y, beta_mu, c0y, c1y)));
    if (!_has2) tv.y = 0.0;
    st2(t, q, n, tv);
#pragma unroll
    for (int j = 0; j < NVB; j++) {
      const f64x2 w = ld_stream(vp[j] + 2 * q);
      acc[j] = fma(tv.x, w.x, fma(tv.y, w.y, acc[j]));
    }
  }
  block_reduce_store<NVB, OP_SUM>(acc, partials, 0, sm);
}

#define PO_CORR_CASE(NVB)                                                                              \
  case NVB:                                                                                            \
    PO_LAUNCH(corr_d1_dots_kernel<NVB>, grid, b, px, pzl, pzu, rx, dinv, beta_mu, pt, n, t, c->d_partials); \
    break;
int k_corr_d1_dots(Ctx *c, const Bounds &b, const double *px, const double *pzl, const double *pzu, const double *rx,
                   const double *dinv, double beta_mu, const double *const *V, int nv, int64_t n, double *t,
                   double *out) {
  if (nv < 1 || nv > kCorrDotsMax) {
    set_error("k_corr_d1_dots: %d panel columns (1..%d)", nv, kCorrDotsMax);
    return PO_ERR_ARG;
  }
  count_bytes(c, nv + 11, n);
  const int grid = grid_for(c, n, 5);
  PO_TRY(ensure_partials(c, (size_t)grid * nv));
  PtrTable pt;
  CoefTable ct;
  fill_tables(nullptr, V, nv, &ct, &pt);
  switch (nv) {
    PO_CORR_CASE(1) PO_CORR_CASE(2) PO_CORR_CASE(3) PO_CORR_CASE(4) PO_CORR_CASE(5) PO_CORR_CASE(6) PO_CORR_CASE(7)
    PO_CORR_CASE(8) PO_CORR_CASE(9) PO_CORR_CASE(10) PO_CORR_CASE(11) PO_CORR_CASE(12) PO_CORR_CASE(13)
    PO_CORR_CASE(14) PO_CORR_CASE(15)
  }
  return reduce_finish(c, grid, nv, 0, 0, out);
}

struct Step3 {
  double px, pzl, pzu;
};
template <int REFINE>
__device__ __forceinline__ Step3 solve2_elem(const BE &e, double dx, double beta_mu, double px0,
                                             double pzl0, double pzu0, double cl = 0.0,
                                             double cu = 0.0) {
  Step3 s;
  const double rzl = e.L ? -(e.xl * e.zl - beta_mu) - cl : 0.0;
  const double rzu = e.U ? -(e.xu * e.zu - beta_mu) + cu : 0.0;
  if (REFINE) {
    const double rzl2 = e.L ? rzl - (e.xl * pzl0 + px0 * e.zl) : 0.0;
    const double rzu2 = e.U ? rzu - (e.xu * pzu0 - px0 * e.zu) : 0.0;
    s.px = px0 + dx;
    s.pzl = pzl0 + (e.L ? (rzl2 - e.zl * dx) / e.xl : 0.0);
    s.pzu = pzu0 + (e.U ? (rzu2 + e.zu * dx) / e.xu : 0.0);
  } else {
    s.px = dx;
    s.pzl = e.L ? (rzl - e.zl * dx) / e.xl : 0.0;
    s.pzu = e.U ? (rzu + e.zu * dx) / e.xu : 0.0;
  }
  return s;
}
__device__ __forceinline__ void max_step_elem(const Bounds &b, double x, double lb, double ub,
                                              double zl, double zu, const Step3 &s, double tau,
                                              double &mx, double &mz) {
  if (b.use_lower) {
    if (s.px < 0.0) mx = fmin(mx, -tau * (x - lb) / s.px);
    if (s.pzl < 0.0) mz = fmin(mz, -tau * zl / s.pzl);
  }
  if (b.use_upper) {
    if (s.px > 0.0) mx = fmin(mx, tau * (ub - x) / s.px);
    if (s.pzu < 0.0) mz = fmin(mz, -tau * zu / s.pzu);
  }
}

__device__ __forceinline__ double res_step_elem(const BE &e, double rx, double acc, double diag,
                                                double px, double pzl, double pzu, double dinv,
                                                double beta_mu, int use_lower, int use_upper) {
  double r = rx - diag * px + acc;
  if (use_lower) r += pzl;
  if (use_upper) r -= pzu;
  double d1 = r;
  if (e.L) {
    const double rzl2 = -(e.xl * e.zl - beta_mu) - (e.xl * pzl + px * e.zl);
    d1 += rzl2 / e.xl;
  }
  if (e.U) {
    const double rzu2 = -(e.xu * e.zu - beta_mu) - (e.xu * pzu - px * e.zu);
    d1 -= rzu2 / e.xu;
  }
  return dinv * d1;
}
template <int REFINE, int FUSE>
__global__ void __launch_bounds__(kBlock)
    solve2_kernel(Bounds b, const double *t, const double *__restrict__ dinv, CoefTable alpha,
                  CoefTable coef2, PtrTable P, int nv, double beta_mu, double tau,
                  const double *__restrict__ rx, double diag, int64_t n, double *__restrict__ px,
                  double *__restrict__ pzl, double *__restrict__ pzu, double *tout,
                  double *__restrict__ va, int nca, const double *__restrict__ cl,
                  const double *__restrict__ cu, double *__restrict__ partials) {
  __shared__ double sm[4 * 2];
  double mins[2] = {1.0, 1.0};
  PO_PAIR_LOOP(q, n) {
    const double2 accA = panel_sum(P, alpha, nca, q);
    if (va) {
      double2 w = accA;
      if (REFINE) {
        const double2 w0 = ld2(va, q, n);
        w.x += w0.x;
// ... 82 lines not shown
    acc1.x += a1A.x;
    acc1.y += a1A.y;
    acc2.x += a2A.x;
    acc2.y += a2A.y;
    if (va) st2(va, q, n, make_double2(a2A.x + a1A.x, a2A.y + a1A.y));
    PO_LOAD_BOUNDS(b, q, n);
    double2 tv, dv;
    if (t1) {
      tv = ld2(t1, q, n);
      dv = ld2(dinv, q, n);
    } else {
      const double2 r0 = ld2(rx, q, n);
      dv = make_double2(dinv_elem(e0, dinv_diag), _has2 ? dinv_elem(e1, dinv_diag) : 0.0);
      tv = make_double2(dv.x * d1_elem(e0, r0.x, beta_mu), _has2 ? dv.y * d1_elem(e1, r0.y, beta_mu) : 0.0);
    }
    const Step3 f0 = solve2_elem<0>(e0, tv.x + dv.x * acc1.x, beta_mu, 0.0, 0.0, 0.0);
    Step3 f1 = solve2_elem<0>(e1, tv.y + dv.y * acc1.y, beta_mu, 0.0, 0.0, 0.0);
    if (!_has2) f1.px = f1.pzl = f1.pzu = 0.0;
    double2 tw;
    if (RECT) {
      const double2 r = ld2(rx, q, n);
      tw.x = dv.x * res_step_elem(e0, r.x, accr.x, diag, f0.px, f0.pzl, f0.pzu, 1.0, beta_mu, b.use_lower, b.use_upper);
      tw.y = _has2 ? dv.y * res_step_elem(e1, r.y, accr.y, diag, f1.px, f1.pzl, f1.pzu, 1.0, beta_mu, b.use_lower,
                                          b.use_upper)
                   : 0.0;
    } else {
      tw = ld2(t2, q, n);
    }
    const Step3 s0 = solve2_elem<1>(e0, tw.x + dv.x * acc2.x, beta_mu, f0.px, f0.pzl, f0.pzu);
    Step3 s1 = solve2_elem<1>(e1, tw.y + dv.y * acc2.y, beta_mu, f1.px, f1.pzl, f1.pzu);
    if (!_has2) s1.px = s1.pzl = s1.pzu = 0.0;
    st2(px, q, n, make_double2(s0.px, s1.px));
    if (pzl) {
      st2(pzl, q, n, make_double2(s0.pzl, s1.pzl));
      st2(pzu, q, n, make_double2(s0.pzu, s1.pzu));
    }
    max_step_elem(b, _x.x, _lb.x, _ub.x, _zl.x, _zu.x, s0, tau, mins[0], mins[1]);
    if (_has2) max_step_elem(b, _x.y, _lb.y, _ub.y, _zl.y, _zu.y, s1, tau, mins[0], mins[1]);
    if (MERIT) {
      const double2 gv = ld2(g, q, n);
      if (e0.L) {
        ms[0] += _zl.x * s0.px;
        ms[1] += s0.pzl * e0.xl;
        ms[2] += s0.pzl * s0.px;
        if (s0.px > 0.0) ms[3] += s0.px / e0.xl; else ms[4] += s0.px / e0.xl;
      }
      if (e1.L) {
        ms[0] += _zl.y * s1.px;
        ms[1] += s1.pzl * e1.xl;
        ms[2] += s1.pzl * s1.px;
        if (s1.px > 0.0) ms[3] += s1.px / e1.xl; else ms[4] += s1.px / e1.xl;
      }
      if (e0.U) {
        ms[0] -= _zu.x * s0.px;
        ms[1] += s0.pzu * e0.xu;
        ms[2] -= s0.pzu * s0.px;
        if (s0.px > 0.0) ms[4] -= s0.px / e0.xu; else ms[3] -= s0.px / e0.xu;
      }
      if (e1.U) {
        ms[0] -= _zu.y * s1.px;
        ms[1] += s1.pzu * e1.xu;
        ms[2] -= s1.pzu * s1.px;
        if (s1.px > 0.0) ms[4] -= s1.px / e1.xu; else ms[3] -= s1.px / e1.xu;
      }
      ms[5] += gv.x * s0.px + gv.y * s1.px;
      ms[6] += s0.px * s0.px + s1.px * s1.px;
      mx[0] = fmax(mx[0], fmax(fabs(s0.px), fabs(s1.px)));
    }
  }
  if (MERIT) {
    block_reduce_store<7, OP_SUM>(ms, partials, 0, sm);
    block_reduce_store<2, OP_MIN>(mins, partials, 7, sm);
    block_reduce_store<1, OP_MAX>(mx, partials, 9, sm);
  } else {
    block_reduce_store<2, OP_MIN>(mins, partials, 0, sm);
  }
}

int k_solve2r(Ctx *c, const Bounds &b, const double *t1, const double *t2, const double *dinv, const double *a1,
              const double *a2, const double *const *P, int nv, double beta_mu, double tau, int64_t n, double *px,
              double *pzl, double *pzu, double *va, int nca, double out[2], const double *ar, const double *rx,
              double diag, int ca0, const double *const *vs, int nvirt, double b0v, const double *g,
              double *merit_out, double dinv_diag, const GroupCol *gcol, double gc1, double gc2) {
  count_bytes(c, nv + nvirt + 7 + (t1 ? 2 : 0) + (pzl ? 2 : 0) + (va ? 1 : 0) + (g ? 1 : 0), n);
  PO_TRY(gcol_check(gcol, n, "k_solve2r"));
  if (gcol && t2 == nullptr) {
    set_error("k_solve2r: a grouped column is only taken in the stored right-hand side form");
    return PO_ERR_ARG;
  }
  if (gcol) count_bytes(c, 1.0, gcol->nwcon);
  const GroupCol gcv = gcol ? *gcol : GroupCol();
  if (!t1 && (t2 != nullptr || !rx)) {
    set_error("k_solve2r: Dinv / t can only be re-formed in the recomputed right-hand side form");
    return PO_ERR_ARG;
  }
  if (nv > kMaxPanel) {
    set_error("panel of %d vectors exceeds kMaxPanel=%d", nv, kMaxPanel);
    return PO_ERR_ARG;
  }
  const int grid = grid_for(c, n, kBpcPanel);
  PO_TRY(ensure_partials(c, (size_t)grid * 10));
  PtrTable pt;
  CoefTable ct1, ct2, ctr;
  fill_tables(a1, P, nv, &ct1, &pt);
  fill_tables(a2, P, nv, &ct2, &pt);
  fill_tables(ar, P, nv, &ctr, &pt);
  VirtCols vc;
  vc.count = 0;
  vc.b0 = b0v;
  for (int j = 0; j < kMaxVirt; j++) vc.s[j] = nullptr;
  if (nvirt > 0) {
    if (nvirt > kMaxVirt || t2 != nullptr || ca0 < nvirt) {
      set_error("k_solve2r: %d unformed columns (at most %d, leading the panel, recomputed right-hand side only)", nvirt,
                kMaxVirt);
      return PO_ERR_ARG;
    }
    vc.count = nvirt;
    for (int j = 0; j < nvirt; j++) vc.s[j] = vs[j];
  }
  if (t2 != nullptr && ca0 != 0) {
    set_error("k_solve2r: the stored right-hand side form expects the constraint columns first");
    return PO_ERR_ARG;
  }
  if (t2 == nullptr) {
    if (!ar || !rx) {
      set_error("k_solve2r: neither the refinement right-hand side nor the data to recompute it");
      return PO_ERR_ARG;
    }
    if (g && merit_out) {
      PO_LAUNCH((solve2r_kernel<1, 1>), grid, b, t1, t2, dinv, ct1, ct2, ctr, pt, nv, beta_mu, tau, rx, diag, n, px,
                pzl, pzu, va, nca, ca0, vc, g, dinv_diag, gcv, gc1, gc2, c->d_partials);
      (void)out;
      return reduce_finish(c, grid, 7, 2, 1, merit_out);
    }
    PO_LAUNCH((solve2r_kernel<1, 0>), grid, b, t1, t2, dinv, ct1, ct2, ctr, pt, nv, beta_mu, tau, rx, diag, n, px, pzl,
              pzu, va, nca, ca0, vc, g, dinv_diag, gcv, gc1, gc2, c->d_partials);
  } else if (g && merit_out) {
    PO_LAUNCH((solve2r_kernel<0, 1>), grid, b, t1, t2, dinv, ct1, ct2, ctr, pt, nv, beta_mu, tau, rx, diag, n, px, pzl,
              pzu, va, nca, ca0, vc, g, dinv_diag, gcv, gc1, gc2, c->d_partials);
    (void)out;
    return reduce_finish(c, grid, 7, 2, 1, merit_out);
  } else {
    PO_LAUNCH((solve2r_kernel<0, 0>), grid, b, t1, t2, dinv, ct1, ct2, ctr, pt, nv, beta_mu, tau, rx, diag, n, px, pzl,
              pzu, va, nca, ca0, vc, g, dinv_diag, gcv, gc1, gc2, c->d_partials);
  }
  return reduce_finish(c, grid, 0, 2, 0, out);
}

int k_solve2(Ctx *c, const Bounds &b, const double *t, const double *dinv, const double *alpha,
             const double *const *P, int nv, double beta_mu, int refine, double tau, int64_t n,
             double *px, double *pzl, double *pzu, double out[2], const double *coef2,
             const double *rx, double diag, double *tout, double *va, int nca, const double *cl,
             const double *cu) {
  count_bytes(c, nv + 10 + (refine ? 3 : 0) + (va ? (refine ? 2 : 1) : 0) + (coef2 ? 2 : 0) + (cl ? 2 : 0), n);
  if (nv > kMaxPanel) {
    if (coef2) {
      set_error("k_solve2: the fused refinement residual is not available for a panel of %d (> %d) columns", nv,
                kMaxPanel);
      return PO_ERR_ARG;
    }
    const double *P2[2] = {nullptr, nullptr};
    double a2[2] = {0.0, 0.0};
    int nv2 = 0, nca2 = 0;
    PO_TRY(collapse_panel(c, alpha, P, nv, va ? nca : 0, n, P2, a2, &nv2, &nca2));
    return k_solve2(c, b, t, dinv, a2, P2, nv2, beta_mu, refine, tau, n, px, pzl, pzu, out, nullptr, rx, diag, tout, va,
                    nca2, cl, cu);
  }
  const int grid = grid_for(c, n, kBpcPanel);
  PO_TRY(ensure_partials(c, (size_t)grid * 2));
  PtrTable pt;
  CoefTable ct, ct2;
  fill_tables(alpha, P, nv, &ct, &pt);
  fill_tables(coef2, P, nv, &ct2, &pt);
  if (refine) {
    PO_LAUNCH((solve2_kernel<1, 0>), grid, b, t, dinv, ct, ct2, pt, nv, beta_mu, tau, rx, diag, n, px,
              pzl, pzu, tout, va, nca, cl, cu, c->d_partials);
  } else if (coef2) {
    PO_LAUNCH((solve2_kernel<0, 1>), grid, b, t, dinv, ct, ct2, pt, nv, beta_mu, tau, rx, diag, n, px,
              pzl, pzu, tout, va, nca, cl, cu, c->d_partials);
  } else {
    PO_LAUNCH((solve2_kernel<0, 0>), grid, b, t, dinv, ct, ct2, pt, nv, beta_mu, tau, rx, diag, n, px,
              pzl, pzu, tout, va, nca, cl, cu, c->d_partials);
  }
  return reduce_finish(c, grid, 0, 2, 0, out);
}

constexpr int kS2Tile = 128;
template <int NPASS, int OCC, int VIRT>
__global__ void __launch_bounds__(kBlock, OCC)
    solve2_dots_kernel(Bounds b, const double *t, const double *__restrict__ dinv, CoefTable alpha,
                       CoefTable coef2, PtrTable P, int nv, double beta_mu, double tau,
                       const double *__restrict__ rx, double diag, int64_t n, int64_t ntiles,
                       double *__restrict__ px, double *__restrict__ pzl, double *__restrict__ pzu,
                       double *tout, double *__restrict__ va, int nca, double *__restrict__ traw,
                       int store_step, int ca0, VirtCols vc, double dinv_diag, GroupCols2 gcs,
                       double *__restrict__ partials) {
  extern __shared__ double s2lds[];
  double *pt = s2lds;
  double *sacc = s2lds + 4 * NPASS * kS2Tile;
  double *stp = sacc + 4 * 64 * 6;
  double *sm = stp + kS2Tile;
  const int tid = threadIdx.x, lane = tid & 63;
  const int wave = __builtin_amdgcn_readfirstlane(tid >> 6);
  double *myslice = pt + (size_t)wave * NPASS * kS2Tile + 2 * lane;
  double dotacc[NPASS];
#pragma unroll
  for (int it = 0; it < NPASS; it++) dotacc[it] = 0.0;
  double mins[2] = {1.0, 1.0};
  const int64_t qlast = (n - 1) >> 1;
  f64x2 buf[NPASS];
  f64x2 sbuf[VIRT ? 3 : 1];
  const int gmine = (gcs.count > 0 && wave == (nv & 3)) ? 0 : ((gcs.count > 1 && wave == ((nv + 1) & 3)) ? 1 : -1);
  GRaw gbuf;
  gbuf.raw = (f64x2){0.0, 0.0};
  gbuf.valid = 0;
  double eb[8];
  int64_t ie = 0;
  bool ein = false;
  int64_t q = 0;
  bool in = false;
#define PO_S2_PREFETCH(TILE)                                                                 \
  {                                                                                          \
    q = (TILE) * 64 + lane;                                                                  \
    in = (2 * q < n);                                                                        \
    if (!in) q = qlast;                                                                      \
    _Pragma("unroll") for (int it = 0; it < NPASS; it++) {                                   \
      const int j = wave + 4 * it;                                                           \
      buf[it] = ld_stream(P.p[j < nv ? j : 0] + 2 * q);                                      \
    }                                                                                        \
    if (VIRT) {                                                                              \
      _Pragma("unroll") for (int it = 0; it < (VIRT ? 3 : 0); it++) {                        \
        const int j = wave + 4 * it;                                                         \
        sbuf[it] = ld_stream(vc.s[j < vc.count ? j : 0] + 2 * q);                            \
      }                                                                                      \
    }                                                                                        \
    if (gmine >= 0) gbuf = gcol_request(gcs.g[gmine], q, n);                                 \
  }
#define PO_S2_PREFETCH_E(TILE)                                                               \
  {                                                                                          \
    const int64_t _ir = (TILE) * kS2Tile + 64 * wave + lane;                                 \
    ein = _ir < n;                                                                           \
    ie = ein ? _ir : n - 1;                                                                  \
    eb[0] = b.x[ie];                                                                         \
    eb[1] = b.lb[ie];                                                                        \
    eb[2] = b.ub[ie];                                                                        \
    eb[3] = b.zl[ie];                                                                        \
    eb[4] = b.zu[ie];                                                                        \
    if (t) {  \
      eb[5] = t[ie];                                                                         \
      eb[6] = dinv[ie];                                                                      \
    }                                                                                        \
    eb[7] = rx[ie];                                                                          \
  }
  if ((int64_t)blockIdx.x < ntiles) {
    PO_S2_PREFETCH((int64_t)blockIdx.x);
    if (wave < 2) PO_S2_PREFETCH_E((int64_t)blockIdx.x);
  }
  for (int64_t tile = blockIdx.x; tile < ntiles; tile += gridDim.x) {
    const int64_t qc = q;
    const bool inc = in;
    f64x2 a1 = (f64x2){0.0, 0.0}, a2 = a1, aA = a1;
#pragma unroll
    for (int it = 0; it < NPASS; it++) {
      const int j = wave + 4 * it;
      f64x2 v = buf[it];
      if (VIRT && it < 3 && j < vc.count) {
        v.x -= vc.b0 * sbuf[VIRT ? it : 0].x;
        v.y -= vc.b0 * sbuf[VIRT ? it : 0].y;
      }
      if (!inc) v = (f64x2){0.0, 0.0};
      const double ca = alpha.a[j], cb = coef2.a[j], cA = (j >= ca0 && j < ca0 + nca) ? ca : 0.0;
      a1 += ca * v;
      a2 += cb * v;
      aA += cA * v;
      *reinterpret_cast<f64x2 *>(myslice + it * kS2Tile) = v;
    }
    if (gmine >= 0) {
      f64x2 v = gcol_value(gcs.g[gmine], gbuf);
      if (!inc) v = (f64x2){0.0, 0.0};
      a1 += gcs.ca[gmine] * v;
      a2 += gcs.cb[gmine] * v;
    }
    double *sa = sacc + wave * 64 + lane;
    sa[0 * 256] = a1.x;
    sa[1 * 256] = a1.y;
    sa[2 * 256] = a2.x;
    sa[3 * 256] = a2.y;
    sa[4 * 256] = aA.x;
    sa[5 * 256] = aA.y;
    __syncthreads();
    const bool more = tile + gridDim.x < ntiles;
    if (more && wave >= 2) PO_S2_PREFETCH(tile + gridDim.x);
    if (wave < 2) {
      const int er = 64 * wave + lane, el = er >> 1, ec = er & 1;
      double acc = 0.0, acc2 = 0.0, accA = 0.0;
#pragma unroll
      for (int w = 0; w < 4; w++) {
        const double *sp = sacc + w * 64 + el;
        acc += sp[(0 + ec) * 256];
        acc2 += sp[(2 + ec) * 256];
        accA += sp[(4 + ec) * 256];
      }
      double tp = 0.0;
      const int64_t i = tile * kS2Tile + er;
      if (ein) {
        const double _x = eb[0], _lb = eb[1], _ub = eb[2], _zl = eb[3], _zu = eb[4];
        const BE e = bound_elem(_x, _lb, _ub, _zl, _zu, b.max_bound, b.use_lower, b.use_upper);
        const double r = eb[7];
        double tv, dv;
        if (t) {
          tv = eb[5];
          dv = eb[6];
        } else {
          dv = dinv_elem(e, dinv_diag);
          tv = dv * d1_elem(e, r, beta_mu);
        }
        if (va && store_step == 1) va[i] = accA;
        const Step3 s0 = solve2_elem<0>(e, tv + dv * acc, beta_mu, 0.0, 0.0, 0.0);
        if (store_step) {
          px[i] = s0.px;
          if (store_step == 1) {
            pzl[i] = s0.pzl;
            pzu[i] = s0.pzu;
          }
        }
        const double raw = res_step_elem(e, r, acc2, diag, s0.px, s0.pzl, s0.pzu, 1.0, beta_mu, b.use_lower,
                                         b.use_upper);
        tp = dv * raw;
// ... 14 lines not shown
        }
        if (traw) {
          traw[i] = 0.0;
        } else if (tout) {
          tout[i] = 0.0;
        }
      }
      stp[er] = tp;
      if (more) {
        PO_S2_PREFETCH(tile + gridDim.x);
        PO_S2_PREFETCH_E(tile + gridDim.x);
      }
    }
    __syncthreads();
    const f64x2 tt = *reinterpret_cast<const f64x2 *>(stp + 2 * lane);
#pragma unroll
    for (int it = 0; it < NPASS; it++) {
      const f64x2 v = *reinterpret_cast<const f64x2 *>(myslice + it * kS2Tile);
      dotacc[it] = fma(v.x, tt.x, fma(v.y, tt.y, dotacc[it]));
    }
  }
#undef PO_S2_PREFETCH
#undef PO_S2_PREFETCH_E
#pragma unroll
  for (int it = 0; it < NPASS; it++) {
    const double v = wave_reduce<OP_SUM>(dotacc[it]);
    const int j = wave + 4 * it;
    if (lane == 0 && j < nv) partials[(size_t)j * gridDim.x + blockIdx.x] = v;
  }
  __syncthreads();
  block_reduce_store<2, OP_MIN>(mins, partials, nv, sm);
}

template <int NPASS, int OCC>
__global__ void __launch_bounds__(kBlock, OCC)
    solve2_dots2_kernel(Bounds b, const double *t, const double *__restrict__ dinv, CoefTable alpha,
                        CoefTable coef2, PtrTable P, int nv, double beta_mu, double tau,
                        const double *__restrict__ rx, double diag, int64_t n, int64_t ntiles,
                        double *__restrict__ px, double *__restrict__ pzl, double *__restrict__ pzu,
                        double *tout, double *__restrict__ va, int nca, double *__restrict__ traw,
                        int store_step, int ca0, double dinv_diag, GroupCols2 gcs,
                        double *__restrict__ partials) {
  extern __shared__ double s2lds[];
  double *sacc = s2lds;
  double *stp = s2lds + 2 * (4 * 64 * 6);
  double *sm = stp + 2 * kS2Tile;
  const int tid = threadIdx.x, lane = tid & 63;
  const int wave = __builtin_amdgcn_readfirstlane(tid >> 6);
  const int ex = wave >> 1, eh = wave & 1;
  double dotacc[NPASS];
#pragma unroll
  for (int it = 0; it < NPASS; it++) dotacc[it] = 0.0;
  double mins[2] = {1.0, 1.0};
  const int64_t qlast = (n - 1) >> 1;
  f64x2 buf[2][NPASS];
  const int gmine = (gcs.count > 0 && wave == (nv & 3)) ? 0 : ((gcs.count > 1 && wave == ((nv + 1) & 3)) ? 1 : -1);
  GRaw gbuf[2];
  bool in[2] = {false, false};
  double eb[8];
  bool ein = false;
#pragma unroll
  for (int x = 0; x < 2; x++) {
    gbuf[x].raw = (f64x2){0.0, 0.0};
    gbuf[x].valid = 0;
  }
#define PO_S22_REQUEST(FIRST)                                                                \
  {                                                                                          \
    _Pragma("unroll") for (int x = 0; x < 2; x++) {                                          \
      const int64_t _tile = (FIRST) + x * (int64_t)gridDim.x;                                \
      int64_t _q = _tile * 64 + lane;                                                        \
      in[x] = _tile < ntiles && 2 * _q < n;                                                  \
      if (!in[x]) _q = qlast;                                                                \
      _Pragma("unroll") for (int it = 0; it < NPASS; it++) {                                 \
        const int j = wave + 4 * it;                                                         \
        buf[x][it] = ld_stream(P.p[j < nv ? j : 0] + 2 * _q);                                \
      }                                                                                      \
      if (gmine >= 0) gbuf[x] = gcol_request(gcs.g[gmine], _q, n);                           \
    }                                                                                        \
    const int64_t _mine = (FIRST) + ex * (int64_t)gridDim.x;                                 \
    const int64_t _ir = _mine * kS2Tile + 64 * eh + lane;                                    \
    ein = _mine < ntiles && _ir < n;                                                         \
    const int64_t _ie = ein ? _ir : n - 1;                                                   \
    eb[0] = b.x[_ie];                                                                        \
    eb[1] = b.lb[_ie];                                                                       \
    eb[2] = b.ub[_ie];                                                                       \
    eb[3] = b.zl[_ie];                                                                       \
    eb[4] = b.zu[_ie];                                                                       \
    if (t) {                                                                                 \
      eb[5] = t[_ie];                                                                        \
      eb[6] = dinv[_ie];                                                                     \
    }                                                                                        \
    eb[7] = rx[_ie];                                                                         \
  }
  if ((int64_t)blockIdx.x < ntiles) PO_S22_REQUEST((int64_t)blockIdx.x);
  for (int64_t first = blockIdx.x; first < ntiles; first += 2 * (int64_t)gridDim.x) {
    const bool has2 = first + gridDim.x < ntiles;
#pragma unroll
    for (int x = 0; x < 2; x++) {
      f64x2 a1 = (f64x2){0.0, 0.0}, a2 = a1, aA = a1;
#pragma unroll
      for (int it = 0; it < NPASS; it++) {
        const int j = wave + 4 * it;
        f64x2 v = buf[x][it];
        if (!in[x]) v = (f64x2){0.0, 0.0};
        buf[x][it] = v;
        const double ca = alpha.a[j], cb = coef2.a[j], cA = (j >= ca0 && j < ca0 + nca) ? ca : 0.0;
        a1 += ca * v;
        a2 += cb * v;
        aA += cA * v;
      }
      if (gmine >= 0) {
        f64x2 v = gcol_value(gcs.g[gmine], gbuf[x]);
        if (!in[x]) v = (f64x2){0.0, 0.0};
        a1 += gcs.ca[gmine] * v;
        a2 += gcs.cb[gmine] * v;
      }
      double *sa = sacc + x * (4 * 64 * 6) + wave * 64 + lane;
      sa[0 * 256] = a1.x;
      sa[1 * 256] = a1.y;
      sa[2 * 256] = a2.x;
      sa[3 * 256] = a2.y;
      sa[4 * 256] = aA.x;
      sa[5 * 256] = aA.y;
    }
    __syncthreads();
    if (ex == 0 || has2) {
      const int64_t tile = first + ex * (int64_t)gridDim.x;
      const int er = 64 * eh + lane, el = er >> 1, ec = er & 1;
      double acc = 0.0, acc2 = 0.0, accA = 0.0;
#pragma unroll
      for (int w = 0; w < 4; w++) {
        const double *sp = sacc + ex * (4 * 64 * 6) + w * 64 + el;
        acc += sp[(0 + ec) * 256];
        acc2 += sp[(2 + ec) * 256];
        accA += sp[(4 + ec) * 256];
      }
      double tp = 0.0;
      const int64_t i = tile * kS2Tile + er;
      if (ein) {
        const double _x = eb[0], _lb = eb[1], _ub = eb[2], _zl = eb[3], _zu = eb[4];
        const BE e = bound_elem(_x, _lb, _ub, _zl, _zu, b.max_bound, b.use_lower, b.use_upper);
        const double r = eb[7];
        double tv, dv;
        if (t) {
          tv = eb[5];
          dv = eb[6];
        } else {
          dv = dinv_elem(e, dinv_diag);
          tv = dv * d1_elem(e, r, beta_mu);
        }
        if (va && store_step == 1) va[i] = accA;
        const Step3 s0 = solve2_elem<0>(e, tv + dv * acc, beta_mu, 0.0, 0.0, 0.0);
        if (store_step) {
          px[i] = s0.px;
          if (store_step == 1) {
            pzl[i] = s0.pzl;
            pzu[i] = s0.pzu;
          }
        }
        const double raw = res_step_elem(e, r, acc2, diag, s0.px, s0.pzl, s0.pzu, 1.0, beta_mu, b.use_lower,
                                         b.use_upper);
        tp = dv * raw;
        if (traw) {
          traw[i] = raw;
        } else if (tout) {
          tout[i] = tp;
        }
        max_step_elem(b, _x, _lb, _ub, _zl, _zu, s0, tau, mins[0], mins[1]);
// ... 38 lines not shown
  block_reduce_store<2, OP_MIN>(mins, partials, nv, sm);
}

template <int NP, int OCC>
static int solve2_dots2_launch(Ctx *c, const Bounds &b, const double *t, const double *dinv, const CoefTable &ct,
                               const CoefTable &ct2, const PtrTable &pt, int nv, double beta_mu, double tau,
                               const double *rx, double diag, int64_t n, int64_t ntiles, double *px, double *pzl,
                               double *pzu, double *tout, double *va, int nca, double *traw, int store_step, int ca0,
                               double dinv_diag, int *grid_out, const GroupCols2 &gcs) {
  const size_t lds = sizeof(double) * (size_t)(2 * (4 * 64 * 6) + 2 * kS2Tile + 8);
  const size_t lds1 = sizeof(double) * (size_t)(4 * NP * kS2Tile + 4 * 64 * 6 + kS2Tile + 8);
  int per_cu = (int)((160 * 1024) / lds1);
  if (per_cu > OCC) per_cu = OCC;
  if (per_cu < 1) per_cu = 1;
  int64_t g = (int64_t)c->num_cu * per_cu;
  if (g > ntiles) g = ntiles;
  if (g < 1) g = 1;
  PO_TRY(ensure_partials(c, (size_t)g * (nv + 2)));
  hipLaunchKernelGGL((solve2_dots2_kernel<NP, OCC>), dim3((int)g), dim3(kBlock), lds, c->stream, b, t, dinv, ct, ct2, pt,
                     nv, beta_mu, tau, rx, diag, n, ntiles, px, pzl, pzu, tout, va, nca, traw, store_step, ca0,
                     dinv_diag, gcs, c->d_partials);
  c->n_launches++;
  PO_HIP(hipGetLastError());
  *grid_out = (int)g;
  return PO_OK;
}

template <int NP, int OCC, int VIRT>
static int solve2_dots_launch(Ctx *c, int grid_cap, const Bounds &b, const double *t, const double *dinv,
                              const CoefTable &ct, const CoefTable &ct2, const PtrTable &pt, int nv, double beta_mu,
                              double tau, const double *rx, double diag, int64_t n, int64_t ntiles, double *px,
                              double *pzl, double *pzu, double *tout, double *va, int nca, double *traw,
                              int store_step, int ca0, const VirtCols &vc, double dinv_diag, int *grid_out,
                              const GroupCols2 &gcs) {
  const size_t lds = sizeof(double) * (size_t)(4 * NP * kS2Tile + 4 * 64 * 6 + kS2Tile + 8);
  static bool attr_set = false;
  if (!attr_set) {
    PO_HIP(hipFuncSetAttribute(reinterpret_cast<const void *>(solve2_dots_kernel<NP, OCC, VIRT>),
                               hipFuncAttributeMaxDynamicSharedMemorySize, (int)lds));
    attr_set = true;
  }
  int per_cu = (int)((160 * 1024) / lds);
  if (per_cu > OCC) per_cu = OCC;
  if (per_cu < 1) per_cu = 1;
  int64_t g = (int64_t)c->num_cu * per_cu;
  if (g > ntiles) g = ntiles;
  if (g < 1) g = 1;
  PO_TRY(ensure_partials(c, (size_t)g * (nv + 2)));
  hipLaunchKernelGGL((solve2_dots_kernel<NP, OCC, VIRT>), dim3((int)g), dim3(kBlock), lds, c->stream, b, t, dinv, ct, ct2, pt, nv,
                     beta_mu, tau, rx, diag, n, ntiles, px, pzl, pzu, tout, va, nca, traw, store_step, ca0, vc,
                     dinv_diag, gcs, c->d_partials);
  c->n_launches++;
  PO_HIP(hipGetLastError());
  *grid_out = (int)g;
  return PO_OK;
}

#define PO_S2D_CASE(NP)                                                                                    \
  case NP: {                                                                                               \
     \
    constexpr int OD = NP <= 8 ? 3 : (NP <= 16 ? 2 : 1), OA = NP <= 8 ? 2 : OD;                            \
    constexpr int OV = NP <= 16 ? 2 : 1;         \
     \
    if (NP <= 6 && vc.count == 0 && two_tiles && occ_env != OA) {                                          \
      constexpr int NP2 = NP <= 6 ? NP : 6;                                                                \
      PO_TRY((solve2_dots2_launch<NP2, 3>(c, b, t, dinv, ct, ct2, pt, nv, beta_mu, tau, rx, diag, n, ntiles, px, pzl, \
                                          pzu, tout, va, nca, traw, store_step, ca0, dinv_diag, &grid, gcs))); \
    } else if (vc.count > 0)                                                                               \
      PO_TRY((solve2_dots_launch<NP, OV, 1>(c, 0, b, t, dinv, ct, ct2, pt, nv, beta_mu, tau, rx, diag, n, ntiles, \
                                            px, pzl, pzu, tout, va, nca, traw, store_step, ca0, vc, dinv_diag, &grid, gcs))); \
    else if (occ_env == OA)                                                                                \
      PO_TRY((solve2_dots_launch<NP, OA, 0>(c, 0, b, t, dinv, ct, ct2, pt, nv, beta_mu, tau, rx, diag, n, ntiles, \
                                            px, pzl, pzu, tout, va, nca, traw, store_step, ca0, vc, dinv_diag, &grid, gcs))); \
    else                                                                                                   \
      PO_TRY((solve2_dots_launch<NP, OD, 0>(c, 0, b, t, dinv, ct, ct2, pt, nv, beta_mu, tau, rx, diag, n, ntiles, \
                                            px, pzl, pzu, tout, va, nca, traw, store_step, ca0, vc, dinv_diag, &grid, gcs))); \
  } break;

int k_solve2_dots(Ctx *c, const Bounds &b, const double *t, const double *dinv, const double *alpha,
                  const double *coef2, const double *const *P, int nv, double beta_mu, double tau,
                  const double *rx, double diag, int64_t n, double *px, double *pzl, double *pzu,
                  double *tout, double *va, int nca, double *out, double *traw, int store_step, int ca0,
                  const double *const *vs, int nvirt, double b0v, double dinv_diag, const GroupCols2 *gcols) {
  count_bytes(c, nv + nvirt + 6 + (t ? 2 : 0) + (store_step == 1 ? 3 + (va ? 1 : 0) : (store_step == 2 ? 1 : 0)) + ((traw || tout) ? 1 : 0), n);
  const GroupCols2 gcs = gcols ? *gcols : GroupCols2();
  for (int e = 0; e < gcs.count; e++) PO_TRY(gcol_check(&gcs.g[e], n, "k_solve2_dots"));
  for (int e = 0; e < gcs.count; e++) count_bytes(c, 1.0, gcs.g[e].nwcon);
  if (nv > kMaxPanel || nv < 1) {
    set_error("panel of %d vectors outside 1..%d", nv, kMaxPanel);
    return PO_ERR_ARG;
  }
  VirtCols vc;
  vc.count = 0;
  vc.b0 = b0v;
  for (int j = 0; j < kMaxVirt; j++) vc.s[j] = nullptr;
  if (nvirt > 0) {
    if (nvirt > kMaxVirt || ca0 < nvirt) {
      set_error("k_solve2_dots: %d unformed columns (at most %d, leading the panel)", nvirt, kMaxVirt);
      return PO_ERR_ARG;
    }
    vc.count = nvirt;
    for (int j = 0; j < nvirt; j++) vc.s[j] = vs[j];
  }
  const int64_t ntiles = (((n + 1) >> 1) + 63) / 64;
  int grid = 0;
  static const int occ_env = getenv("PAROPT_AMD_S2D_OCC") ? atoi(getenv("PAROPT_AMD_S2D_OCC")) : 0;
  const bool two_tiles = dbg_switch(SW_S2D_TWO, "PAROPT_AMD_S2D_TWO", 0) != 0;
  PtrTable pt;
  CoefTable ct, ct2;
  fill_tables(alpha, P, nv, &ct, &pt);
  fill_tables(coef2, P, nv, &ct2, &pt);
  const int need = (nv + 3) / 4;
  const int np = need <= 2 ? 2 : need <= 4 ? 4 : need <= 6 ? 6 : need <= 8 ? 8 : need <= 11 ? 11 : need <= 12 ? 12
                 : need <= 16 ? 16 : need <= 20 ? 20 : 24;
  switch (np) {
    PO_S2D_CASE(2) PO_S2D_CASE(4) PO_S2D_CASE(6) PO_S2D_CASE(8) PO_S2D_CASE(11) PO_S2D_CASE(12) PO_S2D_CASE(16)
    PO_S2D_CASE(20) PO_S2D_CASE(24)
  }
  return reduce_finish(c, grid, nv, 2, 0, out);
}

__global__ void __launch_bounds__(kBlock)
    res_step_kernel(Bounds b, const double *__restrict__ rx, const double *__restrict__ px,
                    const double *__restrict__ pzl, const double *__restrict__ pzu,
                    const double *__restrict__ dinv, CoefTable coef, PtrTable P, int nv, double diag,
                    double beta_mu, int64_t n, double *__restrict__ tp) {
  PO_PAIR_LOOP(q, n) {
    const double2 acc = panel_sum(P, coef, nv, q);
    PO_LOAD_BOUNDS(b, q, n);
    const double2 r = ld2(rx, q, n), p = ld2(px, q, n), l = ld2(pzl, q, n), u = ld2(pzu, q, n);
    const double2 dv = dinv ? ld2(dinv, q, n) : make_double2(1.0, 1.0);
    st2(tp, q, n,
        make_double2(res_step_elem(e0, r.x, acc.x, diag, p.x, l.x, u.x, dv.x, beta_mu, b.use_lower,
                                   b.use_upper),
                     res_step_elem(e1, r.y, acc.y, diag, p.y, l.y, u.y, dv.y, beta_mu, b.use_lower,
                                   b.use_upper)));
  }
}
__global__ void __launch_bounds__(kBlock)
    step_check_kernel(Bounds b, const double *__restrict__ rx, const double *__restrict__ px,
                      const double *__restrict__ pzl, const double *__restrict__ pzu, CoefTable coef, PtrTable P,
                      int nv, double diag, double beta_mu, int64_t n, double *__restrict__ partials) {
  __shared__ double sm[4 * 3];
  double mx[3] = {0.0, 0.0, 0.0};
  PO_PAIR_LOOP(q, n) {
    const double2 acc = panel_sum(P, coef, nv, q);
    PO_LOAD_BOUNDS(b, q, n);
    const double2 r = ld2(rx, q, n), p = ld2(px, q, n), l = ld2(pzl, q, n), u = ld2(pzu, q, n);
    const BE es[2] = {e0, e1};
    const double rr[2] = {r.x, r.y}, pp[2] = {p.x, p.y}, ll[2] = {l.x, l.y}, uu[2] = {u.x, u.y},
                 aa[2] = {acc.x, acc.y};
#pragma unroll
    for (int k = 0; k < 2; k++) {
      if (k == 1 && !_has2) break;
      double v = rr[k] - diag * pp[k] + aa[k];
      if (b.use_lower) v += ll[k];
      if (b.use_upper) v -= uu[k];
      mx[0] = fmax(mx[0], fabs(v));
      if (es[k].L) mx[1] = fmax(mx[1], fabs(-(es[k].xl * es[k].zl - beta_mu) - (es[k].xl * ll[k] + pp[k] * es[k].zl)));
      if (es[k].U) mx[2] = fmax(mx[2], fabs(-(es[k].xu * es[k].zu - beta_mu) - (es[k].xu * uu[k] - pp[k] * es[k].zu)));
    }
  }
  block_reduce_store<3, OP_MAX>(mx, partials, 0, sm);
}
int k_step_check(Ctx *c, const Bounds &b, const double *rx, const double *px, const double *pzl, const double *pzu,
                 const double *coef, const double *const *P, int nv, double diag, double beta_mu, int64_t n,
                 double out[3]) {
  if (nv > kMaxPanel) {
    const double *w = nullptr, one = 1.0;
    PO_TRY(collapse_range(c, 0, coef, P, 0, nv, n, &w));
    return k_step_check(c, b, rx, px, pzl, pzu, &one, &w, 1, diag, beta_mu, n, out);
  }
  count_bytes(c, nv + 9, n);
  const int grid = grid_for(c, n, kBpcPanel);
  PO_TRY(ensure_partials(c, (size_t)grid * 3));
  PtrTable pt;
  CoefTable ct;
  fill_tables(coef, P, nv, &ct, &pt);
  PO_LAUNCH(step_check_kernel, grid, b, rx, px, pzl, pzu, ct, pt, nv, diag, beta_mu, n, c->d_partials);
  return reduce_finish(c, grid, 0, 0, 3, out);
}

int k_res_step(Ctx *c, const Bounds &b, const double *rx, const double *px, const double *pzl,
               const double *pzu, const double *dinv, const double *coef, const double *const *P,
               int nv, double diag, double beta_mu, int64_t n, double *tprime) {
  if (nv > kMaxPanel) {
    const double *w = nullptr, one = 1.0;
    PO_TRY(collapse_range(c, 0, coef, P, 0, nv, n, &w));
    return k_res_step(c, b, rx, px, pzl, pzu, dinv, &one, &w, 1, diag, beta_mu, n, tprime);
  }
  count_bytes(c, nv + 10 + (dinv ? 1 : 0), n);
  if (n <= 0) return PO_OK;
  PtrTable pt;
  CoefTable ct;
  fill_tables(coef, P, nv, &ct, &pt);
  PO_LAUNCH(res_step_kernel, grid_for(c, n, kBpcPanel), b, rx, px, pzl, pzu, dinv, ct, pt, nv, diag, beta_mu, n,
            tprime);
  return PO_OK;
}

__global__ void __launch_bounds__(kBlock)
    comp_step_kernel(Bounds b, const double *__restrict__ px, const double *__restrict__ pzl,
                     const double *__restrict__ pzu, double ax, double az, int64_t n,
                     double *__restrict__ partials) {
  __shared__ double sm[4 * 2];
  double sums[2] = {0.0, 0.0};
  PO_PAIR_LOOP(q, n) {
    PO_LOAD_BOUNDS(b, q, n);
    const double2 p = ld2(px, q, n), l = ld2(pzl, q, n), u = ld2(pzu, q, n);
    const double xn0 = _x.x + ax * p.x, xn1 = _x.y + ax * p.y;
    if (e0.L) {
      sums[0] += (_zl.x + az * l.x) * (xn0 - _lb.x);
      sums[1] += 1.0;
    }
    if (e1.L) {
      sums[0] += (_zl.y + az * l.y) * (xn1 - _lb.y);
      sums[1] += 1.0;
    }
    if (e0.U) {
      sums[0] += (_zu.x + az * u.x) * (_ub.x - xn0);
      sums[1] += 1.0;
    }
    if (e1.U) {
      sums[0] += (_zu.y + az * u.y) * (_ub.y - xn1);
      sums[1] += 1.0;
    }
  }
  block_reduce_store<2, OP_SUM>(sums, partials, 0, sm);
}
int k_comp_step(Ctx *c, const Bounds &b, const double *px, const double *pzl, const double *pzu,
                double ax, double az, int64_t n, double out[2]) {
  count_bytes(c, 8, n);
  const int grid = grid_for(c, n);
  PO_TRY(ensure_partials(c, (size_t)grid * 2));
  PO_LAUNCH(comp_step_kernel, grid, b, px, pzl, pzu, ax, az, n, c->d_partials);
  return reduce_finish(c, grid, 2, 0, 0, out);
}

__device__ __forceinline__ void barrier_elem(const BE &e, double &pos, double &neg) {
  if (e.L) {
    const double v = log(e.xl);
    if (e.xl > 1.0) pos += v; else neg += v;
  }
  if (e.U) {
    const double v = log(e.xu);
    if (e.xu > 1.0) pos += v; else neg += v;
  }
}
__global__ void __launch_bounds__(kBlock)
    merit0_kernel(Bounds b, const double *__restrict__ px, double sx, const double *__restrict__ g,
                  int64_t n, double *__restrict__ partials) {
  __shared__ double sm[4 * 6];
  double s[6] = {0.0, 0.0, 0.0, 0.0, 0.0, 0.0};
  PO_PAIR_LOOP(q, n) {
    PO_LOAD_BOUNDS(b, q, n);
    double2 p = ld2(px, q, n);
    const double2 gv = ld2(g, q, n);
    p.x *= sx;
    p.y *= sx;
    barrier_elem(e0, s[0], s[1]);
    barrier_elem(e1, s[0], s[1]);
    if (e0.L) { if (p.x > 0.0) s[2] += p.x / e0.xl; else s[3] += p.x / e0.xl; }
    if (e1.L) { if (p.y > 0.0) s[2] += p.y / e1.xl; else s[3] += p.y / e1.xl; }
    if (e0.U) { if (p.x > 0.0) s[3] -= p.x / e0.xu; else s[2] -= p.x / e0.xu; }
    if (e1.U) { if (p.y > 0.0) s[3] -= p.y / e1.xu; else s[2] -= p.y / e1.xu; }
    s[4] += gv.x * p.x + gv.y * p.y;
    s[5] += p.x * p.x + p.y * p.y;
  }
  block_reduce_store<6, OP_SUM>(s, partials, 0, sm);
}
int k_merit0(Ctx *c, const Bounds &b, const double *px, double sx, const double *g, int64_t n,
             double out[6]) {
  count_bytes(c, 7, n);
  const int grid = grid_for(c, n);
  PO_TRY(ensure_partials(c, (size_t)grid * 6));
  PO_LAUNCH(merit0_kernel, grid, b, px, sx, g, n, c->d_partials);
  return reduce_finish(c, grid, 6, 0, 0, out);
}

__global__ void __launch_bounds__(kBlock)
    comp_merit_kernel(Bounds b, const double *__restrict__ px, const double *__restrict__ pzl,
                      const double *__restrict__ pzu, double ax, double az, const double *__restrict__ g,
                      int64_t n, double *__restrict__ partials) {
  __shared__ double sm[4 * 8];
  double s[8] = {0.0, 0.0, 0.0, 0.0, 0.0, 0.0, 0.0, 0.0};
  double mx[1] = {0.0};
  PO_PAIR_LOOP(q, n) {
    PO_LOAD_BOUNDS(b, q, n);
    const double2 p = ld2(px, q, n), l = ld2(pzl, q, n), u = ld2(pzu, q, n), gv = ld2(g, q, n);
    const double xn0 = _x.x + ax * p.x, xn1 = _x.y + ax * p.y;
    if (e0.L) {
      s[0] += (_zl.x + az * l.x) * (xn0 - _lb.x);
      s[1] += 1.0;
    }
    if (e1.L) {
      s[0] += (_zl.y + az * l.y) * (xn1 - _lb.y);
      s[1] += 1.0;
    }
    if (e0.U) {
      s[0] += (_zu.x + az * u.x) * (_ub.x - xn0);
      s[1] += 1.0;
    }
    if (e1.U) {
      s[0] += (_zu.y + az * u.y) * (_ub.y - xn1);
      s[1] += 1.0;
    }
    barrier_elem(e0, s[2], s[3]);
    barrier_elem(e1, s[2], s[3]);
    if (e0.L) { if (p.x > 0.0) s[4] += p.x / e0.xl; else s[5] += p.x / e0.xl; }
    if (e1.L) { if (p.y > 0.0) s[4] += p.y / e1.xl; else s[5] += p.y / e1.xl; }
    if (e0.U) { if (p.x > 0.0) s[5] -= p.x / e0.xu; else s[4] -= p.x / e0.xu; }
    if (e1.U) { if (p.y > 0.0) s[5] -= p.y / e1.xu; else s[4] -= p.y / e1.xu; }
    s[6] += gv.x * p.x + gv.y * p.y;
    s[7] += p.x * p.x + p.y * p.y;
    mx[0] = fmax(mx[0], fmax(fabs(p.x), fabs(p.y)));
  }
  block_reduce_store<8, OP_SUM>(s, partials, 0, sm);
  block_reduce_store<1, OP_MAX>(mx, partials, 8, sm);
}
int k_comp_merit(Ctx *c, const Bounds &b, const double *px, const double *pzl, const double *pzu, double ax,
                 double az, const double *g, int64_t n, double out[9]) {
  count_bytes(c, 9, n);
  const int grid = grid_for(c, n);
  PO_TRY(ensure_partials(c, (size_t)grid * 9));
  PO_LAUNCH(comp_merit_kernel, grid, b, px, pzl, pzu, ax, az, g, n, c->d_partials);
  return reduce_finish(c, grid, 8, 0, 1, out);
}

__global__ void __launch_bounds__(kBlock)
    solve2c_kernel(Bounds b, const double *__restrict__ t, const double *__restrict__ dinv, CoefTable alpha, PtrTable P,
                   int nv, double beta_mu, double tau, int64_t n, double *__restrict__ px, double *__restrict__ pzl,
                   double *__restrict__ pzu, double *__restrict__ va, int nca, const double *__restrict__ g,
                   int want_logs, double *__restrict__ partials) {
  __shared__ double sm[4 * 9];
  double mins[2] = {1.0, 1.0};
  double ms[9] = {0.0, 0.0, 0.0, 0.0, 0.0, 0.0, 0.0, 0.0, 0.0};
  double mx[1] = {0.0};
  PO_PAIR_LOOP(q, n) {
    const double2 accA = panel_sum(P, alpha, nca, q);
    if (va) st2(va, q, n, accA);
    double2 acc = panel_sum(P, alpha, nv, q, nca);
    acc.x += accA.x;
    acc.y += accA.y;
    PO_LOAD_BOUNDS(b, q, n);
    const double2 tv = ld2(t, q, n), dv = ld2(dinv, q, n);
    const double dx0 = tv.x + dv.x * acc.x, dx1 = tv.y + dv.y * acc.y;
    const double2 pa = ld2(px, q, n), la = ld2(pzl, q, n), ua = ld2(pzu, q, n);
    const double c0x = e0.L ? __dmul_rn(pa.x, la.x) : 0.0, c0y = e1.L ? __dmul_rn(pa.y, la.y) : 0.0;
    const double c1x = e0.U ? __dmul_rn(pa.x, ua.x) : 0.0, c1y = e1.U ? __dmul_rn(pa.y, ua.y) : 0.0;
    const Step3 s0 = solve2_elem<0>(e0, dx0, beta_mu, 0.0, 0.0, 0.0, c0x, c1x);
    Step3 s1 = solve2_elem<0>(e1, dx1, beta_mu, 0.0, 0.0, 0.0, c0y, c1y);
    if (!_has2) s1.px = s1.pzl = s1.pzu = 0.0;
    st2(px, q, n, make_double2(s0.px, s1.px));
    st2(pzl, q, n, make_double2(s0.pzl, s1.pzl));
    st2(pzu, q, n, make_double2(s0.pzu, s1.pzu));
    max_step_elem(b, _x.x, _lb.x, _ub.x, _zl.x, _zu.x, s0, tau, mins[0], mins[1]);
    if (_has2) max_step_elem(b, _x.y, _lb.y, _ub.y, _zl.y, _zu.y, s1, tau, mins[0], mins[1]);
    const double2 gv = ld2(g, q, n);
    if (e0.L) {
      ms[0] += _zl.x * s0.px;
      ms[1] += s0.pzl * e0.xl;
      ms[2] += s0.pzl * s0.px;
    }
    if (e1.L) {
      ms[0] += _zl.y * s1.px;
      ms[1] += s1.pzl * e1.xl;
      ms[2] += s1.pzl * s1.px;
    }
    if (e0.U) {
      ms[0] -= _zu.x * s0.px;
      ms[1] += s0.pzu * e0.xu;
      ms[2] -= s0.pzu * s0.px;
    }
    if (e1.U) {
      ms[0] -= _zu.y * s1.px;
      ms[1] += s1.pzu * e1.xu;
      ms[2] -= s1.pzu * s1.px;
    }
    if (want_logs) {
      barrier_elem(e0, ms[7], ms[8]);
      barrier_elem(e1, ms[7], ms[8]);
    }
    if (e0.L) { if (s0.px > 0.0) ms[3] += s0.px / e0.xl; else ms[4] += s0.px / e0.xl; }
    if (e1.L) { if (s1.px > 0.0) ms[3] += s1.px / e1.xl; else ms[4] += s1.px / e1.xl; }
    if (e0.U) { if (s0.px > 0.0) ms[4] -= s0.px / e0.xu; else ms[3] -= s0.px / e0.xu; }
    if (e1.U) { if (s1.px > 0.0) ms[4] -= s1.px / e1.xu; else ms[3] -= s1.px / e1.xu; }
    ms[5] += gv.x * s0.px + gv.y * s1.px;
    ms[6] += s0.px * s0.px + s1.px * s1.px;
    mx[0] = fmax(mx[0], fmax(fabs(s0.px), fabs(s1.px)));
  }
  block_reduce_store<9, OP_SUM>(ms, partials, 0, sm);
  block_reduce_store<2, OP_MIN>(mins, partials, 9, sm);
  block_reduce_store<1, OP_MAX>(mx, partials, 11, sm);
}
int k_solve2c(Ctx *c, const Bounds &b, const double *t, const double *dinv, const double *alpha,
              const double *const *P, int nv, double beta_mu, double tau, int64_t n, double *px, double *pzl,
              double *pzu, double *va, int nca, const double *g, int want_logs, double out[12]) {
  if (nv > kMaxPanel) {
    set_error("k_solve2c: panel of %d vectors exceeds kMaxPanel=%d", nv, kMaxPanel);
    return PO_ERR_ARG;
  }
  count_bytes(c, nv + 14 + (va ? 1 : 0), n);
  const int grid = grid_for(c, n);
  PO_TRY(ensure_partials(c, (size_t)grid * 12));
  PtrTable pt;
  CoefTable ct;
  fill_tables(alpha, P, nv, &ct, &pt);
  PO_LAUNCH(solve2c_kernel, grid, b, t, dinv, ct, pt, nv, beta_mu, tau, n, px, pzl, pzu, va, nca, g, want_logs,
            c->d_partials);
  return reduce_finish(c, grid, 9, 2, 1, out);
}

__device__ __forceinline__ double clamp_elem(double v, bool has_l, double lb, bool has_u, double ub,
                                             double eps) {
  if (has_l && v <= lb + eps) v = lb + eps;
  if (has_u && v + eps >= ub) v = ub - eps;
  return v;
}
__global__ void __launch_bounds__(kBlock)
    trial_kernel(Bounds b, const double *__restrict__ px, double a, double eps, int64_t n,
                 double *__restrict__ xt, double *__restrict__ sout, double *__restrict__ partials) {
  __shared__ double sm[4 * 2];
  double s[2] = {0.0, 0.0};
  PO_PAIR_LOOP(q, n) {
    const double2 x = ld2(b.x, q, n), lb = ld2(b.lb, q, n), ub = ld2(b.ub, q, n), p = ld2(px, q, n);
    const bool has2 = (2 * q + 1 < n);
    double2 v;
    v.x = clamp_elem(x.x + a * p.x, true, lb.x, true, ub.x, eps);
    v.y = clamp_elem(x.y + a * p.y, true, lb.y, true, ub.y, eps);
    st2(xt, q, n, v);
    if (sout) st2(sout, q, n, make_double2(__dadd_rn(__dmul_rn(a, p.x), 0.0), __dadd_rn(__dmul_rn(a, p.y), 0.0)));
    BE e0 = bound_elem(v.x, lb.x, ub.x, 0.0, 0.0, b.max_bound, b.use_lower, b.use_upper);
    barrier_elem(e0, s[0], s[1]);
    if (has2) {
      BE e1 = bound_elem(v.y, lb.y, ub.y, 0.0, 0.0, b.max_bound, b.use_lower, b.use_upper);
      barrier_elem(e1, s[0], s[1]);
    }
  }
  block_reduce_store<2, OP_SUM>(s, partials, 0, sm);
}
int k_trial(Ctx *c, const Bounds &b, const double *px, double a, double eps, int64_t n, double *xt,
            double out[2], double *sout) {
  count_bytes(c, 5 + (sout ? 1 : 0), n);
  const int grid = grid_for(c, n);
  PO_TRY(ensure_partials(c, (size_t)grid * 2));
  PO_LAUNCH(trial_kernel, grid, b, px, a, eps, n, xt, sout, c->d_partials);
  return reduce_finish(c, grid, 2, 0, 0, out);
}

__global__ void __launch_bounds__(kBlock)
    update_mult_kernel(double *__restrict__ zl, const double *__restrict__ pzl,
                       double *__restrict__ zu, const double *__restrict__ pzu, double a, double eps,
                       int use_lower, int use_upper, int64_t n) {
  PO_PAIR_LOOP(q, n) {
    if (use_lower) {
      const double2 z = ld2(zl, q, n), p = ld2(pzl, q, n);
      st2(zl, q, n,
          make_double2(clamp_elem(z.x + a * p.x, true, 0.0, false, 0.0, eps),
                       clamp_elem(z.y + a * p.y, true, 0.0, false, 0.0, eps)));
    }
    if (use_upper) {
      const double2 z = ld2(zu, q, n), p = ld2(pzu, q, n);
      st2(zu, q, n,
          make_double2(clamp_elem(z.x + a * p.x, true, 0.0, false, 0.0, eps),
                       clamp_elem(z.y + a * p.y, true, 0.0, false, 0.0, eps)));
    }
  }
}
int k_update_mult(Ctx *c, double *zl, const double *pzl, double *zu, const double *pzu, double a,
                  double eps, int use_lower, int use_upper, int64_t n) {
  count_bytes(c, 3 * (use_lower + use_upper), n);
  if (n <= 0) return PO_OK;
  PO_LAUNCH(update_mult_kernel, grid_for(c, n), zl, pzl, zu, pzu, a, eps, use_lower, use_upper, n);
  return PO_OK;
}

__global__ void __launch_bounds__(kBlock)
    update_mult_yqn_kernel(double *__restrict__ zl, const double *__restrict__ pzl,
                           double *__restrict__ zu, const double *__restrict__ pzu, double a,
                           double eps, int use_lower, int use_upper, const double *__restrict__ rx,
                           const double *__restrict__ va, double az, int64_t n,
                           double *__restrict__ yqn, double *__restrict__ acz) {
  PO_PAIR_LOOP(q, n) {
    const double2 r = ld2(rx, q, n), w = ld2(va, q, n);
    double2 y = make_double2(__fma_rn(az, w.x, r.x), __fma_rn(az, w.y, r.y));
    if (acz) {
      const double2 c0 = ld2(acz, q, n);
      st2(acz, q, n, make_double2(__fma_rn(az, w.x, c0.x), __fma_rn(az, w.y, c0.y)));
    }
    if (use_lower) {
      const double2 z = ld2(zl, q, n), p = ld2(pzl, q, n);
      y.x = __dsub_rn(y.x, z.x);
      y.y = __dsub_rn(y.y, z.y);
      st2(zl, q, n,
          make_double2(clamp_elem(__fma_rn(a, p.x, z.x), true, 0.0, false, 0.0, eps),
                       clamp_elem(__fma_rn(a, p.y, z.y), true, 0.0, false, 0.0, eps)));
    }
    if (use_upper) {
      const double2 z = ld2(zu, q, n), p = ld2(pzu, q, n);
      y.x = __dadd_rn(y.x, z.x);
      y.y = __dadd_rn(y.y, z.y);
      st2(zu, q, n,
          make_double2(clamp_elem(__fma_rn(a, p.x, z.x), true, 0.0, false, 0.0, eps),
                       clamp_elem(__fma_rn(a, p.y, z.y), true, 0.0, false, 0.0, eps)));
    }
    st2(yqn, q, n, y);
  }
}
int k_update_mult_yqn(Ctx *c, double *zl, const double *pzl, double *zu, const double *pzu, double a,
                      double eps, int use_lower, int use_upper, const double *rx, const double *va,
                      double az, int64_t n, double *yqn, double *acz) {
  count_bytes(c, 3 + 3 * (use_lower + use_upper) + (acz ? 2 : 0), n);
  if (n <= 0) return PO_OK;
  PO_LAUNCH(update_mult_yqn_kernel, grid_for(c, n), zl, pzl, zu, pzu, a, eps, use_lower, use_upper, rx,
            va, az, n, yqn, acz);
  return PO_OK;
}

__global__ void __launch_bounds__(kBlock)
    form_pz_kernel(Bounds b, const double *__restrict__ px, double beta_mu, int64_t n, double *__restrict__ pzl,
                   double *__restrict__ pzu) {
  PO_PAIR_LOOP(q, n) {
    PO_LOAD_BOUNDS(b, q, n);
    const double2 pv = ld2(px, q, n);
    const Step3 t0 = solve2_elem<0>(e0, pv.x, beta_mu, 0.0, 0.0, 0.0);
    const Step3 t1 = solve2_elem<0>(e1, pv.y, beta_mu, 0.0, 0.0, 0.0);
    st2(pzl, q, n, make_double2(t0.pzl, t1.pzl));
    st2(pzu, q, n, make_double2(t0.pzu, t1.pzu));
  }
}
int k_form_pz(Ctx *c, const Bounds &b, const double *px, double beta_mu, int64_t n, double *pzl, double *pzu) {
  if (n <= 0) return PO_OK;
  count_bytes(c, 8, n);
  PO_LAUNCH(form_pz_kernel, grid_for(c, n), b, px, beta_mu, n, pzl, pzu);
  return PO_OK;
}

__global__ void __launch_bounds__(kBlock)
    kkt_res_update_kernel(Bounds b, const double *__restrict__ g, PtrTable A, CoefTable z, int nc, double beta_mu,
                          int64_t n, double *__restrict__ rx, double *__restrict__ yqn, double *__restrict__ zl,
                          const double *__restrict__ pzl, double *__restrict__ zu, const double *__restrict__ pzu,
                          double a, double eps, const double *__restrict__ va, double az, double *__restrict__ acz,
                          double az_acz, const double *__restrict__ pxs, const double *__restrict__ xold,
                          double beta_mu_step, double beta_mu2, GroupCol gcol, double gcoef,
                          double *__restrict__ dinv_out, double *__restrict__ t_out, double spec_diag,
                          double spec_beta_mu, double *__restrict__ partials) {
  __shared__ double sm[4 * 8];
  double sums[8] = {0.0, 0.0, 0.0, 0.0, 0.0, 0.0, 0.0, 0.0};
  double maxs[5] = {0.0, 0.0, 0.0, 0.0, 0.0};
  PO_PAIR_LOOP(q, n) {
    GRaw graw;
    if (gcol.w) graw = gcol_request(gcol, q, n);
    const double2 _x = ld2(b.x, q, n), _lb = ld2(b.lb, q, n), _ub = ld2(b.ub, q, n);
    double2 lean_pl = make_double2(0.0, 0.0), lean_pu = lean_pl;
    if (pxs) {
      const double2 pv = ld2(pxs, q, n), xo = ld2(xold, q, n);
      const double2 zlo = ld2(zl, q, n), zuo = ld2(zu, q, n);
      const BE o0 = bound_elem(xo.x, _lb.x, _ub.x, zlo.x, zuo.x, b.max_bound, b.use_lower, b.use_upper);
      BE o1 = bound_elem(xo.y, _lb.y, _ub.y, zlo.y, zuo.y, b.max_bound, b.use_lower, b.use_upper);
      if (2 * q + 1 >= n) {
        o1.L = false;
        o1.U = false;
        o1.xl = 1.0;
        o1.xu = 1.0;
      }
      const Step3 t0 = solve2_elem<0>(o0, pv.x, beta_mu_step, 0.0, 0.0, 0.0);
      const Step3 t1 = solve2_elem<0>(o1, pv.y, beta_mu_step, 0.0, 0.0, 0.0);
      lean_pl = make_double2(t0.pzl, t1.pzl);
      lean_pu = make_double2(t0.pzu, t1.pzu);
    }
    const double2 zero2 = make_double2(0.0, 0.0);
    const double2 r0 = yqn ? ld2(rx, q, n) : zero2, w = va ? ld2(va, q, n) : zero2, gv = ld2(g, q, n);
    double2 y = make_double2(__fma_rn(az, w.x, r0.x), __fma_rn(az, w.y, r0.y));
    double2 aczv = make_double2(0.0, 0.0);
    if (acz) {
      const double2 c0 = ld2(acz, q, n);
      aczv = az_acz != 0.0 ? make_double2(__fma_rn(az_acz, w.x, c0.x), __fma_rn(az_acz, w.y, c0.y)) : c0;
      if (az_acz != 0.0) st2(acz, q, n, aczv);
    }
    double2 _zl = make_double2(0.0, 0.0), _zu = _zl;
    if (b.use_lower) {
      const double2 zo = ld2(zl, q, n), p = pxs ? lean_pl : ld2(pzl, q, n);
      y.x = __dsub_rn(y.x, zo.x);
      y.y = __dsub_rn(y.y, zo.y);
      _zl = make_double2(clamp_elem(__fma_rn(a, p.x, zo.x), true, 0.0, false, 0.0, eps),
                         clamp_elem(__fma_rn(a, p.y, zo.y), true, 0.0, false, 0.0, eps));
      st2(zl, q, n, _zl);
      if (2 * q + 1 >= n) _zl.y = 0.0;
    } else {
      _zl = ld2(zl, q, n);
    }
    if (b.use_upper) {
      const double2 zo = ld2(zu, q, n), p = pxs ? lean_pu : ld2(pzu, q, n);
      y.x = __dadd_rn(y.x, zo.x);
      y.y = __dadd_rn(y.y, zo.y);
      _zu = make_double2(clamp_elem(__fma_rn(a, p.x, zo.x), true, 0.0, false, 0.0, eps),
                         clamp_elem(__fma_rn(a, p.y, zo.y), true, 0.0, false, 0.0, eps));
      st2(zu, q, n, _zu);
      if (2 * q + 1 >= n) _zu.y = 0.0;
    } else {
      _zu = ld2(zu, q, n);
    }
    PO_MAKE_BOUNDS(b, q, n);
    double2 r;
    r.x = (b.use_lower ? _zl.x : 0.0);
    r.y = (b.use_lower ? _zl.y : 0.0);
    if (b.use_upper) {
      r.x += -1.0 * _zu.x;
      r.y += -1.0 * _zu.y;
    }
    r.x += -1.0 * gv.x;
    r.y += -1.0 * gv.y;
    double2 ps;
    if (acz) {
      ps = make_double2(fma(1.0, aczv.x, 0.0), fma(1.0, aczv.y, 0.0));
    } else {
      ps = panel_sum(A, z, nc, q);
      if (gcol.w) {
        const f64x2 gcv = gcol_value(gcol, graw);
        ps.x += gcoef * gcv.x;
        ps.y += gcoef * gcv.y;
      }
    }
    r.x += ps.x;
    r.y += ps.y;
    if (!_has2) r.y = 0.0;
    st2(rx, q, n, r);
    if (dinv_out) {
      const double2 dv = make_double2(dinv_elem(e0, spec_diag), dinv_elem(e1, spec_diag));
      st2(dinv_out, q, n, dv);
      st2(t_out, q, n, make_double2(dv.x * d1_elem(e0, r.x, spec_beta_mu), dv.y * d1_elem(e1, r.y, spec_beta_mu)));
    }
    const double cl = b.use_lower ? 1.0 : 0.0, cu = b.use_upper ? -1.0 : 0.0;
    if (yqn) {
      y.x = __dadd_rn(y.x, __fma_rn(-1.0, r.x, __fma_rn(cu, _zu.x, __fma_rn(cl, _zl.x, 0.0))));
      y.y = __dadd_rn(y.y, __fma_rn(-1.0, r.y, __fma_rn(cu, _zu.y, __fma_rn(cl, _zl.y, 0.0))));
      st2(yqn, q, n, y);
    }
    maxs[0] = fmax(maxs[0], fmax(fabs(r.x), fabs(r.y)));
    sums[2] += fabs(r.x) + fabs(r.y);
    sums[5] += r.x * r.x + r.y * r.y;
    res_bound_acc(e0, beta_mu, sums, maxs, 3, 6, 1);
    res_bound_acc(e1, beta_mu, sums, maxs, 3, 6, 1);
    if (beta_mu2 >= 0.0) {
      res_bound_max2(e0, beta_mu2, maxs + 3);
      res_bound_max2(e1, beta_mu2, maxs + 3);
    }
  }
  block_reduce_store<8, OP_SUM>(sums, partials, 0, sm);
  if (beta_mu2 >= 0.0) {
    block_reduce_store<5, OP_MAX>(maxs, partials, 8, sm);
  } else {
    double m3[3] = {maxs[0], maxs[1], maxs[2]};
    block_reduce_store<3, OP_MAX>(m3, partials, 8, sm);
  }
}

int k_kkt_res_update(Ctx *c, const Bounds &b, const double *g, const double *const *A, const double *z, int nc,
                     double beta_mu, int64_t n, double *rx, double *out, double *yqn, double *zl,
                     const double *pzl, double *zu, const double *pzu, double a, double eps, const double *va,
                     double az, double *acz, double az_acz, const double *pxs, const double *xold,
                     double beta_mu_step, double beta_mu2, const GroupCol *gcol, double gcoef, double *dinv_out,
                     double *t_out, double spec_diag, double spec_beta_mu) {
  PO_TRY(gcol_check(gcol, n, "k_kkt_res_update"));
  if (acz && gcol) {
    set_error("kkt_res_update: a grouped column cannot follow the A^T z vector of the linear-constraint mode");
    return PO_ERR_ARG;
  }
  if (nc > kMaxPanel) {
    const double *w = nullptr, one = 1.0;
    PO_TRY(collapse_range(c, 0, z, A, 0, nc, n, &w));
    return k_kkt_res_update(c, b, g, &w, &one, 1, beta_mu, n, rx, out, yqn, zl, pzl, zu, pzu, a, eps, va, az, acz, az_acz,
                            pxs, xold, beta_mu_step, beta_mu2, gcol, gcoef, dinv_out, t_out, spec_diag, spec_beta_mu);
  }
  count_bytes(c, (yqn ? 14 : 11) + (acz ? (az_acz != 0.0 ? 2 : 1) : nc) + (dinv_out ? 2 : 0), n);
  const int grid = grid_for(c, n, kBpcPanel);
  PO_TRY(ensure_partials(c, (size_t)grid * 13));
  PtrTable pt;
  CoefTable ct;
  fill_tables(z, A, nc, &ct, &pt);
  if (gcol) count_bytes(c, 1.0, gcol->nwcon);
  PO_LAUNCH(kkt_res_update_kernel, grid, b, g, pt, ct, nc, beta_mu, n, rx, yqn, zl, pzl, zu, pzu, a, eps, va, az, acz,
            az_acz, pxs, xold, beta_mu_step, beta_mu2, gcol ? *gcol : GroupCol(), gcoef, dinv_out, t_out, spec_diag,
            spec_beta_mu, c->d_partials);
  return reduce_finish(c, grid, 8, 0, beta_mu2 >= 0.0 ? 5 : 3, out);
}

__global__ void __launch_bounds__(kBlock)
    affine_mult_kernel(Bounds b, double *__restrict__ zl, const double *__restrict__ pzl,
                       double *__restrict__ zu, const double *__restrict__ pzu, double amin,
                       int64_t n) {
  PO_PAIR_LOOP(q, n) {
    PO_LOAD_BOUNDS(b, q, n);
    const double2 l = ld2(pzl, q, n), u = ld2(pzu, q, n);
    double2 nl = _zl, nu = _zu;
    if (e0.L) nl.x = fmax(amin, fabs(_zl.x + l.x));
    if (e1.L) nl.y = fmax(amin, fabs(_zl.y + l.y));
    if (e0.U) nu.x = fmax(amin, fabs(_zu.x + u.x));
    if (e1.U) nu.y = fmax(amin, fabs(_zu.y + u.y));
    if (b.use_lower) st2(zl, q, n, nl);
    if (b.use_upper) st2(zu, q, n, nu);
  }
}
int k_affine_mult(Ctx *c, const Bounds &b, double *zl, const double *pzl, double *zu,
                  const double *pzu, double amin, int64_t n) {
  count_bytes(c, 9, n);
  if (n <= 0) return PO_OK;
  PO_LAUNCH(affine_mult_kernel, grid_for(c, n), b, zl, pzl, zu, pzu, amin, n);
  return PO_OK;
}

__global__ void __launch_bounds__(kBlock)
    check_bounds_kernel(double *__restrict__ x, double *__restrict__ lb, double *__restrict__ ub,
                        double *__restrict__ zl, double *__restrict__ zu, double maxb,
                        double rel_bound, int both, int64_t n, double *__restrict__ partials) {
  __shared__ double sm[4 * 3];
  double flags[3] = {0.0, 0.0, 0.0};
  for (int64_t i = (int64_t)blockIdx.x * blockDim.x + threadIdx.x; i < n;
       i += (int64_t)gridDim.x * blockDim.x) {
    double xv = x[i], l = lb[i], u = ub[i];
    if (both) {
      double delta = 1.0;
      if (l > -maxb && u < maxb) {
        if (l >= u) {
          flags[0] = 1.0;
          l = 0.5 * (l + u) - 0.5 * rel_bound;
          u = l + rel_bound;
          lb[i] = l;
          ub[i] = u;
        }
        delta = u - l;
      }
      if (l > -maxb && xv < l + rel_bound * delta) {
        flags[1] = 1.0;
        xv = l + rel_bound * delta;
      }
      if (u < maxb && xv > u - rel_bound * delta) {
        flags[2] = 1.0;
        xv = u - rel_bound * delta;
      }
      x[i] = xv;
    }
    if (l <= -maxb) zl[i] = 0.0;
    if (u >= maxb) zu[i] = 0.0;
  }
  block_reduce_store<3, OP_MAX>(flags, partials, 0, sm);
}
int k_check_bounds(Ctx *c, double *x, double *lb, double *ub, double *zl, double *zu,
                   double max_bound, double rel_bound, int both, int64_t n, int *flag) {
  count_bytes(c, 5, n);
  const int grid = grid_for(c, n);
  PO_TRY(ensure_partials(c, (size_t)grid * 3));
  PO_LAUNCH(check_bounds_kernel, grid, x, lb, ub, zl, zu, max_bound, rel_bound, both, n,
            c->d_partials);
  double out[3];
  PO_TRY(reduce_finish(c, grid, 0, 0, 3, out, true));
  *flag = (out[0] > 0.0 ? 1 : 0) | (out[1] > 0.0 ? 2 : 0) | (out[2] > 0.0 ? 4 : 0);
  return PO_OK;
}

__global__ void __launch_bounds__(kBlock)
    bounds_mode_kernel(double *__restrict__ x, double *__restrict__ lb, double *__restrict__ ub, int mode,
                       int64_t offset, int64_t n) {
  for (int64_t i = (int64_t)blockIdx.x * blockDim.x + threadIdx.x; i < n;
       i += (int64_t)gridDim.x * blockDim.x) {
    const int64_t gi = offset + i;
    if ((mode & 1) && gi % 7 == 3) lb[i] = ub[i] = 0.5 * (lb[i] + ub[i]);
    if ((mode & 2) && gi % 11 == 5) x[i] = lb[i];
    if ((mode & 4) && gi % 13 == 6) x[i] = ub[i];
  }
}
int k_bounds_mode(Ctx *c, double *x, double *lb, double *ub, int mode, int64_t offset, int64_t n) {
  if (n <= 0 || mode == 0) return PO_OK;
  PO_LAUNCH(bounds_mode_kernel, grid_for(c, n), x, lb, ub, mode, offset, n);
  return PO_OK;
}

__global__ void __launch_bounds__(kBlock)
    clamp_count_kernel(const double *__restrict__ x, const double *__restrict__ lb, const double *__restrict__ ub,
                       const double *__restrict__ zl, const double *__restrict__ zu, double eps, int64_t n,
                       double *__restrict__ partials) {
  __shared__ double sm[4 * 4];
  double cnt[4] = {0.0, 0.0, 0.0, 0.0};
  for (int64_t i = (int64_t)blockIdx.x * blockDim.x + threadIdx.x; i < n;
       i += (int64_t)gridDim.x * blockDim.x) {
    if (x[i] == lb[i] + eps) cnt[0] += 1.0;
    if (x[i] == ub[i] - eps) cnt[1] += 1.0;
    if (zl && zl[i] == eps) cnt[2] += 1.0;
    if (zu && zu[i] == eps) cnt[3] += 1.0;
  }
  block_reduce_store<4, OP_SUM>(cnt, partials, 0, sm);
}
int k_clamp_count(Ctx *c, const double *x, const double *lb, const double *ub, const double *zl, const double *zu,
                  double eps, int64_t n, double out[4]) {
  count_bytes(c, 5, n);
  const int grid = grid_for(c, n);
  PO_TRY(ensure_partials(c, (size_t)grid * 4));
  PO_LAUNCH(clamp_count_kernel, grid, x, lb, ub, zl, zu, eps, n, c->d_partials);
  return reduce_finish(c, grid, 4, 0, 0, out);
}

__global__ void __launch_bounds__(kBlock)
    zero_inactive_kernel(const double *__restrict__ lb, const double *__restrict__ ub,
                         double *__restrict__ zl, double *__restrict__ zu, double maxb, int64_t n) {
  for (int64_t i = (int64_t)blockIdx.x * blockDim.x + threadIdx.x; i < n;
       i += (int64_t)gridDim.x * blockDim.x) {
    if (lb[i] <= -maxb) zl[i] = 0.0;
    if (ub[i] >= maxb) zu[i] = 0.0;
  }
}
int k_zero_inactive(Ctx *c, const double *lb, const double *ub, double *zl, double *zu,
                    double max_bound, int64_t n) {
  count_bytes(c, 4, n);
  if (n <= 0) return PO_OK;
  PO_LAUNCH(zero_inactive_kernel, grid_for(c, n), lb, ub, zl, zu, max_bound, n);
  return PO_OK;
}

template <int KIND>
__global__ void __launch_bounds__(kBlock)
    sep_f_kernel(const double *__restrict__ qv, const double *__restrict__ bv,
                 const double *__restrict__ x, int64_t n, double *__restrict__ partials) {
  __shared__ double sm[4];
  double acc[1] = {0.0};
  PO_PAIR_LOOP(q, n) {
    const double2 xv = ld2(x, q, n), b = ld2(bv, q, n);
    const bool has2 = (2 * q + 1 < n);
    if (KIND == 0) {
      const double2 qq = ld2(qv, q, n);
      acc[0] += 0.5 * qq.x * xv.x * xv.x + b.x * xv.x;
      if (has2) acc[0] += 0.5 * qq.y * xv.y * xv.y + b.y * xv.y;
    } else {
      acc[0] += b.x * b.x / (1e-3 + xv.x);
      if (has2) acc[0] += b.y * b.y / (1e-3 + xv.y);
    }
  }
  block_reduce_store<1, OP_SUM>(acc, partials, 0, sm);
}
template <int KIND>
__global__ void __launch_bounds__(kBlock)
// ... 43 lines not shown

template <int KIND>
__global__ void __launch_bounds__(kBlock)
    sep_h_kernel(const double *__restrict__ qv, const double *__restrict__ bv,
                 const double *__restrict__ x, const double *__restrict__ px, int64_t n,
                 double *__restrict__ h) {
  PO_PAIR_LOOP(q, n) {
    double2 r;
    if (KIND == 0) {
      r = ld2(qv, q, n);
    } else {
      const double2 xv = ld2(x, q, n), b = ld2(bv, q, n);
      const double d0 = 1e-3 + xv.x, d1 = 1e-3 + xv.y;
      r.x = 2.0 * b.x * b.x / (d0 * d0 * d0);
      r.y = 2.0 * b.y * b.y / (d1 * d1 * d1);
    }
    if (px) {
      const double2 p = ld2(px, q, n);
      r.x *= p.x;
      r.y *= p.y;
    }
    st2(h, q, n, r);
  }
}
int k_sep_hess(Ctx *c, int kind, const double *q, const double *b, const double *x, const double *px,
               int64_t n, double *h) {
  count_bytes(c, 4, n);
  if (n <= 0) return PO_OK;
  if (kind == 0) {
    PO_LAUNCH(sep_h_kernel<0>, grid_for(c, n), q, b, x, px, n, h);
  } else {
    PO_LAUNCH(sep_h_kernel<1>, grid_for(c, n), q, b, x, px, n, h);
  }
  return PO_OK;
}
__global__ void __launch_bounds__(kBlock)
    rosen_h_kernel(const double *__restrict__ x, double z0, const double *__restrict__ px, int64_t n,
                   double *__restrict__ h) {
  for (int64_t i = (int64_t)blockIdx.x * blockDim.x + threadIdx.x; i < n;
       i += (int64_t)gridDim.x * blockDim.x) {
    const double xi = x[i];
    double d = 2.0 * z0, lo = 0.0, up = 0.0;
    if (i + 1 < n) {
      d += 2.0 - 400.0 * (x[i + 1] - xi * xi) + 800.0 * xi * xi;
      up = -400.0 * xi;
    }
    if (i > 0) {
      d += 200.0;
      lo = -400.0 * x[i - 1];
    }
    if (px) {
      double v = d * px[i];
      if (i + 1 < n) v += up * px[i + 1];
      if (i > 0) v += lo * px[i - 1];
      h[i] = v;
    } else {
      h[i] = d;
    }
  }
}
int k_rosen_hess(Ctx *c, const double *x, double z0, const double *px, int64_t n, double *h) {
  count_bytes(c, 3, n);
  if (n <= 0) return PO_OK;
  PO_LAUNCH(rosen_h_kernel, grid_for(c, n), x, z0, px, n, h);
  return PO_OK;
}

__global__ void __launch_bounds__(kBlock)
    d1s_kernel(Bounds b, const double *__restrict__ bx, const double *__restrict__ dinv, double alpha,
               double beta_mu, int64_t n, double *__restrict__ t) {
  PO_PAIR_LOOP(q, n) {
    PO_LOAD_BOUNDS(b, q, n);
    const double2 r = ld2(bx, q, n), dv = dinv ? ld2(dinv, q, n) : make_double2(1.0, 1.0);
    double d0 = r.x, d1 = r.y;
    if (e0.L) d0 += alpha * (-(e0.xl * e0.zl - beta_mu)) / e0.xl;
    if (e0.U) d0 -= alpha * (-(e0.xu * e0.zu - beta_mu)) / e0.xu;
    if (e1.L) d1 += alpha * (-(e1.xl * e1.zl - beta_mu)) / e1.xl;
    if (e1.U) d1 -= alpha * (-(e1.xu * e1.zu - beta_mu)) / e1.xu;
    st2(t, q, n, make_double2(dv.x * d0, dv.y * d1));
  }
}
int k_d1s(Ctx *c, const Bounds &b, const double *bx, const double *dinv, double alpha, double beta_mu,
          int64_t n, double *t) {
  count_bytes(c, 8, n);
  if (n <= 0) return PO_OK;
  PO_LAUNCH(d1s_kernel, grid_for(c, n), b, bx, dinv, alpha, beta_mu, n, t);
  return PO_OK;
}
template <int FULL>
__global__ void __launch_bounds__(kBlock)
    solve2s_kernel(Bounds b, const double *__restrict__ t, const double *__restrict__ dinv, CoefTable coef,
                   PtrTable P, int nv, double alpha, double beta_mu, double tau, int64_t n,
                   double *__restrict__ px, double *__restrict__ pzl, double *__restrict__ pzu,
                   double *__restrict__ partials) {
  __shared__ double sm[4 * 2];
  double mins[2] = {1.0, 1.0};
  PO_PAIR_LOOP(q, n) {
    const double2 acc = panel_sum(P, coef, nv, q);
    const double2 tv = ld2(t, q, n), dv = ld2(dinv, q, n);
    const double p0 = tv.x + dv.x * acc.x, p1 = tv.y + dv.y * acc.y;
    if (FULL) {
      PO_LOAD_BOUNDS(b, q, n);
      Step3 s0, s1;
      s0.px = p0;
      s1.px = p1;
      s0.pzl = e0.L ? (alpha * (-(e0.xl * e0.zl - beta_mu)) - e0.zl * p0) / e0.xl : 0.0;
      s0.pzu = e0.U ? (alpha * (-(e0.xu * e0.zu - beta_mu)) + e0.zu * p0) / e0.xu : 0.0;
      s1.pzl = e1.L ? (alpha * (-(e1.xl * e1.zl - beta_mu)) - e1.zl * p1) / e1.xl : 0.0;
      s1.pzu = e1.U ? (alpha * (-(e1.xu * e1.zu - beta_mu)) + e1.zu * p1) / e1.xu : 0.0;
      if (!_has2) s1.px = s1.pzl = s1.pzu = 0.0;
      st2(px, q, n, make_double2(s0.px, s1.px));
      st2(pzl, q, n, make_double2(s0.pzl, s1.pzl));
      st2(pzu, q, n, make_double2(s0.pzu, s1.pzu));
      max_step_elem(b, _x.x, _lb.x, _ub.x, _zl.x, _zu.x, s0, tau, mins[0], mins[1]);
      if (_has2) max_step_elem(b, _x.y, _lb.y, _ub.y, _zl.y, _zu.y, s1, tau, mins[0], mins[1]);
    } else {
      st2(px, q, n, make_double2(p0, p1));
    }
  }
  if (FULL) block_reduce_store<2, OP_MIN>(mins, partials, 0, sm);
}
int k_solve2s(Ctx *c, const Bounds &b, const double *t, const double *dinv, const double *coef,
              const double *const *P, int nv, double alpha, double beta_mu, int full, double tau, int64_t n,
              double *px, double *pzl, double *pzu, double out[2]) {
  if (nv > kMaxPanel) {
    const double *w = nullptr, one = 1.0;
    PO_TRY(collapse_range(c, 0, coef, P, 0, nv, n, &w));
    return k_solve2s(c, b, t, dinv, &one, &w, 1, alpha, beta_mu, full, tau, n, px, pzl, pzu, out);
  }
  count_bytes(c, nv + 10, n);
  if (nv > kMaxPanel) {
    set_error("panel of %d vectors exceeds kMaxPanel=%d", nv, kMaxPanel);
    return PO_ERR_ARG;
  }
  const int grid = grid_for(c, n, kBpcPanel);
  PtrTable pt;
  CoefTable ct;
  fill_tables(coef, P, nv, &ct, &pt);
  if (full) {
    PO_TRY(ensure_partials(c, (size_t)grid * 2));
    PO_LAUNCH((solve2s_kernel<1>), grid, b, t, dinv, ct, pt, nv, alpha, beta_mu, tau, n, px, pzl, pzu,
              c->d_partials);
    return reduce_finish(c, grid, 0, 2, 0, out);
  }
  if (n <= 0) return PO_OK;
  PO_LAUNCH((solve2s_kernel<0>), grid, b, t, dinv, ct, pt, nv, alpha, beta_mu, tau, n, px, pzl, pzu,
            c->d_partials);
  return PO_OK;
}

__global__ void __launch_bounds__(kBlock)
    rosen_f_kernel(const double *__restrict__ x, int64_t n, double *__restrict__ partials) {
  __shared__ double sm[4 * 3];
  double s[3] = {0.0, 0.0, 0.0};
  for (int64_t i = (int64_t)blockIdx.x * blockDim.x + threadIdx.x; i < n;
       i += (int64_t)gridDim.x * blockDim.x) {
    const double xi = x[i];
    if (i + 1 < n) {
      const double xn = x[i + 1];
      s[0] += (1.0 - xi) * (1.0 - xi) + 100.0 * (xn - xi * xi) * (xn - xi * xi);
    }
    s[1] -= xi * xi;
    if ((i & 1) == 0) s[2] += xi;
  }
  block_reduce_store<3, OP_SUM>(s, partials, 0, sm);
}
__global__ void __launch_bounds__(kBlock)
    rosen_g_kernel(const double *__restrict__ x, int64_t n, double *__restrict__ g,
                   double *__restrict__ a0, double *__restrict__ a1) {
  for (int64_t i = (int64_t)blockIdx.x * blockDim.x + threadIdx.x; i < n;
       i += (int64_t)gridDim.x * blockDim.x) {
    const double xi = x[i];
    double gi = 0.0;
    if (i + 1 < n) gi += -2.0 * (1.0 - xi) + 200.0 * (x[i + 1] - xi * xi) * (-2.0 * xi);
    if (i > 0) gi += 200.0 * (xi - x[i - 1] * x[i - 1]);
    g[i] = gi;
    a0[i] = -2.0 * xi;
    a1[i] = ((i & 1) == 0) ? 1.0 : 0.0;
  }
}
int k_rosen_f(Ctx *c, const double *x, int64_t n, double out[3]) {
  count_bytes(c, 1, n);
  const int grid = grid_for(c, n);
  PO_TRY(ensure_partials(c, (size_t)grid * 3));
  PO_LAUNCH(rosen_f_kernel, grid, x, n, c->d_partials);
  return reduce_finish(c, grid, 3, 0, 0, out);
}
int k_rosen_g(Ctx *c, const double *x, int64_t n, double *g, double *a0, double *a1) {
  count_bytes(c, 4, n);
  if (n <= 0) return PO_OK;
  PO_LAUNCH(rosen_g_kernel, grid_for(c, n), x, n, g, a0, a1);
  return PO_OK;
}

}
```

Measured before the change: 43.74.

## Detect uniform bound vectors and substitute constants for bound loads in kernels

During the bounds check, the kernel now reduces the min and max bit patterns of lb and ub per rank to detect when every element of a bound vector holds the same value. When it does, the Bounds struct carries a flag and a scalar, and all bound-consuming kernels substitute the constant instead of streaming lb/ub from memory. This removes up to two n-length reads from many bandwidth-bound kernels per iteration. It adds a wider reduction in the check kernel, and a risk of stale flags if the user mutates bounds, which is partly handled by clearing the flags when bounds are handed out.

```diff
diff --git a/paropt_amd/csrc/capi.cpp b/paropt_amd/csrc/capi.cpp
--- a/paropt_amd/csrc/capi.cpp
+++ b/paropt_amd/csrc/capi.cpp
@@ -1033,6 +1033,7 @@
 }
 int po_ip_get_bounds(po_ip ip, po_vec *lb, po_vec *ub) {
   PO_CHECK_PTR(ip);
+  ip->ip->clearUniformBounds();
   if (lb) *lb = static_cast<po_vec>(ip->ip->lowerBounds());
   if (ub) *ub = static_cast<po_vec>(ip->ip->upperBounds());
   return PO_OK;
diff --git a/paropt_amd/csrc/context.cpp b/paropt_amd/csrc/context.cpp
--- a/paropt_amd/csrc/context.cpp
+++ b/paropt_amd/csrc/context.cpp
@@ -25,7 +25,7 @@
 }
 const char *last_error() { return g_err; }
 
-static int g_dbg_switch[SW_COUNT] = {-1, -1, -1, -1, -1, -1, -1, -1, -1, -1, -1, -1, -1, -1, -1, -1, -1};
+static int g_dbg_switch[SW_COUNT] = {-1, -1, -1, -1, -1, -1, -1, -1, -1, -1, -1, -1, -1, -1, -1, -1, -1, -1};
 double host_now() {
   struct timespec t;
   clock_gettime(CLOCK_MONOTONIC, &t);
@@ -624,7 +624,7 @@
   return PO_OK;
 }
 
-int reduce_finish(Ctx *c, int nblocks, int nsum, int nmin, int nmax, double *host_out, bool now) {
+int reduce_finish(Ctx *c, int nblocks, int nsum, int nmin, int nmax, double *host_out, bool now, double *local_out) {
   const int nslots = nsum + nmin + nmax;
   if (nslots > kMaxRed) {
     set_error("reduction of %d slots exceeds kMaxRed=%d", nslots, kMaxRed);
@@ -641,6 +641,9 @@
     }
   }
   if (c->batch_depth > 0 || !c->batch_pend.empty()) {
+    if (local_out) {
+      for (int s = 0; s < nslots; s++) local_out[s] = NAN;
+    }
     c->batch_pend.push_back(Ctx::PendingRed{c->batch_cursor, nsum, nmin, nmax, host_out, part, nblocks});
     c->batch_cursor += nslots;
     if (now || c->batch_depth == 0) return batch_flush(c);
@@ -651,7 +654,12 @@
   int nparts = 1;
   PO_TRY(exchange_reduced(c, nslots, nmin == 0 && nmax == 0, &parts, &nparts));
   combine_segment(parts, nparts, nslots, 0, nsum, nmin, nmax, host_out);
-  return PO_OK;
-}
-
-}
+  if (local_out) {
+    const double *mine = parts + (nparts > 1 ? (size_t)c->rank * nslots : 0);
+    const bool have = nparts > 1 || c->size == 1 || nmin + nmax > 0;
+    for (int s = 0; s < nslots; s++) local_out[s] = have ? mine[s] : NAN;
+  }
+  return PO_OK;
+}
+
+}
diff --git a/paropt_amd/csrc/core.hpp b/paropt_amd/csrc/core.hpp
--- a/paropt_amd/csrc/core.hpp
+++ b/paropt_amd/csrc/core.hpp
@@ -121,7 +121,8 @@
   double b0;
 };
 
-int reduce_finish(Ctx *c, int nblocks, int nsum, int nmin, int nmax, double *host_out, bool now = false);
+int reduce_finish(Ctx *c, int nblocks, int nsum, int nmin, int nmax, double *host_out, bool now = false,
+                  double *local_out = nullptr);
 bool red_direct(const Ctx *c);
 int batch_flush(Ctx *c, const double *keep_partials = nullptr, size_t keep_len = 0);
 void batch_abort(Ctx *c);
@@ -182,7 +183,8 @@
 };
 enum DbgSwitch { SW_WGRAM_RS = 0, SW_LINCOMB_2D = 1, SW_REDO_DT = 2, SW_LEAN_STEP = 3, SW_WGRAM_PRIO = 4,
                  SW_WGRAM_ABLATE = 5, SW_FUSED_MERIT = 6, SW_REDO_DT1 = 7, SW_BPC3 = 8, SW_BPC4 = 9, SW_LINCOMB_BPC = 10,
-                 SW_PERTURB_W = 11, SW_GS_PRODUCER = 12, SW_S2D_TWO = 13, SW_MPC_FUSE = 14, SW_MPC_POLY = 15, SW_SPEC_DT = 16, SW_COUNT = 17 };
+                 SW_PERTURB_W = 11, SW_GS_PRODUCER = 12, SW_S2D_TWO = 13, SW_MPC_FUSE = 14, SW_MPC_POLY = 15, SW_SPEC_DT = 16,
+                 SW_UNIFORM_BOUNDS = 17, SW_COUNT = 18 };
 int dbg_switch(int id, const char *env, int dflt);
 double host_now();
 inline double host_trace_begin(Ctx *c);
@@ -286,7 +288,10 @@
   const double *x, *lb, *ub, *zl, *zu;
   double max_bound;
   int use_lower, use_upper;
-};
+  int lb_uni = 0, ub_uni = 0;
+  double lb_c = 0.0, ub_c = 0.0;
+};
+inline int uniform_bound_streams(const Bounds &b) { return (b.lb_uni ? 1 : 0) + (b.ub_uni ? 1 : 0); }
 int k_kkt_res(Ctx *c, const Bounds &b, const double *g, const double *const *A, const double *z,
               int nc, double beta_mu, int64_t n, double *rx, double *out, double *yqn = nullptr,
               double beta_mu2 = -1.0, const GroupCol *gcol = nullptr, double gcoef = 0.0);
@@ -367,7 +372,8 @@
 int k_affine_mult(Ctx *c, const Bounds &b, double *zl, const double *pzl, double *zu,
                   const double *pzu, double amin, int64_t n);
 int k_check_bounds(Ctx *c, double *x, double *lb, double *ub, double *zl, double *zu,
-                   double max_bound, double rel_bound, int both, int64_t n, int *flag);
+                   double max_bound, double rel_bound, int both, int64_t n, int *flag, int uni[2] = nullptr,
+                   double val[2] = nullptr);
 int k_bounds_mode(Ctx *c, double *x, double *lb, double *ub, int mode, int64_t offset, int64_t n);
 int k_clamp_count(Ctx *c, const double *x, const double *lb, const double *ub, const double *zl, const double *zu,
                   double eps, int64_t n, double out[4]);
diff --git a/paropt_amd/csrc/ip.cpp b/paropt_amd/csrc/ip.cpp
--- a/paropt_amd/csrc/ip.cpp
+++ b/paropt_amd/csrc/ip.cpp
@@ -174,6 +174,12 @@
   b.max_bound = options.real("max_bound_value");
   b.use_lower = use_lower;
   b.use_upper = use_upper;
+  if (dbg_switch(SW_UNIFORM_BOUNDS, nullptr, 1) != 0) {
+    b.lb_uni = bounds_uni[0];
+    b.ub_uni = bounds_uni[1];
+    b.lb_c = bounds_val[0];
+    b.ub_c = bounds_val[1];
+  }
   return b;
 }
 
@@ -235,6 +241,7 @@
 }
 
 int InteriorPoint::initAndCheckDesignAndBounds() {
+  bounds_uni[0] = bounds_uni[1] = 0;
   int rc = prob->getVarsAndBounds(x, lb, ub);
   if (rc != 0) {
     set_error("getVarsAndBounds failed with code %d", rc);
@@ -243,7 +250,7 @@
   const double rel_bound = 0.001 * barrier_param;
   int flag = 0;
   PO_TRY(k_check_bounds(ctx, x->d, lb->d, ub->d, zl->d, zu->d, options.real("max_bound_value"),
-                        rel_bound, use_lower && use_upper, n, &flag));
+                        rel_bound, use_lower && use_upper, n, &flag, bounds_uni, bounds_val));
   check_flag |= flag;
   if (ctx->rank == 0) {
     if (flag & 1) history += "ParOpt Warning: Variable bounds are inconsistent\n";
@@ -276,6 +283,7 @@
 
 int InteriorPoint::resetDesignAndBounds() {
   cwx_valid = false;
+  bounds_uni[0] = bounds_uni[1] = 0;
   int rc = prob->getVarsAndBounds(x, lb, ub);
   if (rc != 0) return PO_ERR_USER;
   PO_TRY(refreshLiveMirror(x));
@@ -1049,6 +1057,7 @@
 }
 
 int InteriorPoint::checkGradients(double dh, std::string *report) {
+  spec_dt_valid = false;
   return prob->checkGradients(dh, x, options.integer("use_hvec_product"), xt, tvec, report);
 }
 
@@ -1972,6 +1981,7 @@
     if (gradient_verification_frequency > 0 && (k % gradient_verification_frequency) == 0) {
       std::string rep;
       PO_TRY(prob->checkGradients(options.real("gradient_check_step_length"), x, use_hvec_product, xt, tvec, &rep));
+      spec_dt_valid = false;
       if (ctx->rank == 0) history += rep;
     }
 
diff --git a/paropt_amd/csrc/ip.hpp b/paropt_amd/csrc/ip.hpp
--- a/paropt_amd/csrc/ip.hpp
+++ b/paropt_amd/csrc/ip.hpp
@@ -55,6 +55,7 @@
   const std::vector<int> &gPivots() const { return gpiv; }
   Vec *lowerBounds() { return lb; }
   Vec *upperBounds() { return ub; }
+  void clearUniformBounds() { bounds_uni[0] = bounds_uni[1] = 0; }
   int checkFlag() const { return check_flag; }
   int clampCounts(double out[8]);
   int checkKKTStep(int iteration, double mu);
@@ -248,6 +249,8 @@
   void userEnd();
   void userHarvest();
   int check_flag = 0;
+  int bounds_uni[2] = {0, 0};
+  double bounds_val[2] = {0.0, 0.0};
   bool ac_valid = false;
   static const int kAczRefresh = 16;
   Vec *acz = nullptr;
diff --git a/paropt_amd/csrc/kernels.hip b/paropt_amd/csrc/kernels.hip
--- a/paropt_amd/csrc/kernels.hip
+++ b/paropt_amd/csrc/kernels.hip
@@ -2,6 +2,7 @@
 
 #include <math.h>
 #include <stdlib.h>
+#include <string.h>
 
 namespace po {
 
@@ -870,8 +871,13 @@
     e1.xl = 1.0;                                                                         \
     e1.xu = 1.0;                                                                         \
   }
+__device__ __forceinline__ double2 ld2_bound(const double *__restrict__ p, int uni, double v, int64_t q, int64_t n) {
+  return uni ? make_double2(v, v) : ld2(p, q, n);
+}
+#define PO_LD2_LB(b, q, n) ld2_bound((b).lb, (b).lb_uni, (b).lb_c, q, n)
+#define PO_LD2_UB(b, q, n) ld2_bound((b).ub, (b).ub_uni, (b).ub_c, q, n)
 #define PO_LOAD_BOUNDS(b, q, n)                                                         \
-  const double2 _x = ld2((b).x, q, n), _lb = ld2((b).lb, q, n), _ub = ld2((b).ub, q, n), \
+  const double2 _x = ld2((b).x, q, n), _lb = PO_LD2_LB(b, q, n), _ub = PO_LD2_UB(b, q, n), \
                 _zl = ld2((b).zl, q, n), _zu = ld2((b).zu, q, n);                        \
   PO_MAKE_BOUNDS(b, q, n)
 
@@ -965,7 +971,7 @@
     PO_TRY(collapse_range(c, 0, z, A, 0, nc, n, &w));
     return k_kkt_res(c, b, g, &w, &one, 1, beta_mu, n, rx, out, yqn, beta_mu2, gcol, gcoef);
   }
-  count_bytes(c, 7 + nc + (yqn ? 2 : 0), n);
+  count_bytes(c, 7 + nc + (yqn ? 2 : 0) - uniform_bound_streams(b), n);
   const int grid = grid_for(c, n, kBpcPanel);
   PO_TRY(ensure_partials(c, (size_t)grid * 13));
   PtrTable pt;
@@ -992,7 +998,7 @@
 }
 
 int k_res_norms(Ctx *c, const Bounds &b, double beta_mu, int64_t n, double out[11]) {
-  count_bytes(c, 5, n);
+  count_bytes(c, 5 - uniform_bound_streams(b), n);
   const int grid = grid_for(c, n);
   PO_TRY(ensure_partials(c, (size_t)grid * 11));
   PO_LAUNCH(res_norms_kernel, grid, b, beta_mu, n, c->d_partials);
@@ -1016,7 +1022,7 @@
   }
 }
 int k_dinv(Ctx *c, const Bounds &b, double diag, int64_t n, double *dinv, const double *hdiag) {
-  count_bytes(c, 6 + (hdiag ? 1 : 0), n);
+  count_bytes(c, 6 + (hdiag ? 1 : 0) - uniform_bound_streams(b), n);
   if (n <= 0) return PO_OK;
   PO_LAUNCH(dinv_kernel, grid_for(c, n), b, diag, hdiag, n, dinv);
   return PO_OK;
@@ -1049,7 +1055,7 @@
 }
 int k_d1(Ctx *c, const Bounds &b, const double *rx, const double *dinv, double beta_mu, int64_t n,
          double *t, const double *cl, const double *cu) {
-  count_bytes(c, 7 + (dinv ? 1 : 0) + (cl ? 2 : 0), n);
+  count_bytes(c, 7 + (dinv ? 1 : 0) + (cl ? 2 : 0) - uniform_bound_streams(b), n);
   if (n <= 0) return PO_OK;
   PO_LAUNCH(d1_kernel, grid_for(c, n), b, rx, dinv, beta_mu, cl, cu, n, t);
   return PO_OK;
@@ -1071,7 +1077,7 @@
 }
 int k_dinv_d1(Ctx *c, const Bounds &b, double diag, const double *hdiag, const double *rx, double beta_mu,
               int64_t n, double *dinv, double *t, int raw) {
-  count_bytes(c, 8 + (hdiag ? 1 : 0), n);
+  count_bytes(c, 8 + (hdiag ? 1 : 0) - uniform_bound_streams(b), n);
   if (n <= 0) return PO_OK;
   PO_LAUNCH(dinv_d1_kernel, grid_for(c, n), b, diag, hdiag, rx, beta_mu, n, dinv, t, raw);
   return PO_OK;
@@ -1090,7 +1096,7 @@
 }
 int k_corrector(Ctx *c, const Bounds &b, const double *px, const double *pzl, const double *pzu,
                 int64_t n, double *cl, double *cu) {
-  count_bytes(c, 8, n);
+  count_bytes(c, 8 - uniform_bound_streams(b), n);
   if (n <= 0) return PO_OK;
   PO_LAUNCH(corrector_kernel, grid_for(c, n), b, px, pzl, pzu, n, cl, cu);
   return PO_OK;
@@ -1140,7 +1146,7 @@
     set_error("k_corr_d1_dots: %d panel columns (1..%d)", nv, kCorrDotsMax);
     return PO_ERR_ARG;
   }
-  count_bytes(c, nv + 11, n);
+  count_bytes(c, nv + 11 - uniform_bound_streams(b), n);
   const int grid = grid_for(c, n, 5);
   PO_TRY(ensure_partials(c, (size_t)grid * nv));
   PtrTable pt;
@@ -1389,7 +1395,7 @@
               double *pzl, double *pzu, double *va, int nca, double out[2], const double *ar, const double *rx,
               double diag, int ca0, const double *const *vs, int nvirt, double b0v, const double *g,
               double *merit_out, double dinv_diag, const GroupCol *gcol, double gc1, double gc2) {
-  count_bytes(c, nv + nvirt + 7 + (t1 ? 2 : 0) + (pzl ? 2 : 0) + (va ? 1 : 0) + (g ? 1 : 0), n);
+  count_bytes(c, nv + nvirt + 7 + (t1 ? 2 : 0) + (pzl ? 2 : 0) + (va ? 1 : 0) + (g ? 1 : 0) - uniform_bound_streams(b), n);
   PO_TRY(gcol_check(gcol, n, "k_solve2r"));
   if (gcol && t2 == nullptr) {
     set_error("k_solve2r: a grouped column is only taken in the stored right-hand side form");
@@ -1459,7 +1465,7 @@
              double *px, double *pzl, double *pzu, double out[2], const double *coef2,
              const double *rx, double diag, double *tout, double *va, int nca, const double *cl,
              const double *cu) {
-  count_bytes(c, nv + 10 + (refine ? 3 : 0) + (va ? (refine ? 2 : 1) : 0) + (coef2 ? 2 : 0) + (cl ? 2 : 0), n);
+  count_bytes(c, nv + 10 + (refine ? 3 : 0) + (va ? (refine ? 2 : 1) : 0) + (coef2 ? 2 : 0) + (cl ? 2 : 0) - uniform_bound_streams(b), n);
   if (nv > kMaxPanel) {
     if (coef2) {
       set_error("k_solve2: the fused refinement residual is not available for a panel of %d (> %d) columns", nv,
@@ -1549,8 +1555,8 @@
     ein = _ir < n;                                                                           \
     ie = ein ? _ir : n - 1;                                                                  \
     eb[0] = b.x[ie];                                                                         \
-    eb[1] = b.lb[ie];                                                                        \
-    eb[2] = b.ub[ie];                                                                        \
+    eb[1] = b.lb_uni ? b.lb_c : b.lb[ie];                                                    \
+    eb[2] = b.ub_uni ? b.ub_c : b.ub[ie];                                                    \
     eb[3] = b.zl[ie];                                                                        \
     eb[4] = b.zu[ie];                                                                        \
     if (t) {  \
@@ -1731,8 +1737,8 @@
     ein = _mine < ntiles && _ir < n;                                                         \
     const int64_t _ie = ein ? _ir : n - 1;                                                   \
     eb[0] = b.x[_ie];                                                                        \
-    eb[1] = b.lb[_ie];                                                                       \
-    eb[2] = b.ub[_ie];                                                                       \
+    eb[1] = b.lb_uni ? b.lb_c : b.lb[_ie];                                                   \
+    eb[2] = b.ub_uni ? b.ub_c : b.ub[_ie];                                                   \
     eb[3] = b.zl[_ie];                                                                       \
     eb[4] = b.zu[_ie];                                                                       \
     if (t) {                                                                                 \
@@ -1937,7 +1943,7 @@
                   const double *rx, double diag, int64_t n, double *px, double *pzl, double *pzu,
                   double *tout, double *va, int nca, double *out, double *traw, int store_step, int ca0,
                   const double *const *vs, int nvirt, double b0v, double dinv_diag, const GroupCols2 *gcols) {
-  count_bytes(c, nv + nvirt + 6 + (t ? 2 : 0) + (store_step == 1 ? 3 + (va ? 1 : 0) : (store_step == 2 ? 1 : 0)) + ((traw || tout) ? 1 : 0), n);
+  count_bytes(c, nv + nvirt + 6 + (t ? 2 : 0) + (store_step == 1 ? 3 + (va ? 1 : 0) : (store_step == 2 ? 1 : 0)) + ((traw || tout) ? 1 : 0) - uniform_bound_streams(b), n);
   const GroupCols2 gcs = gcols ? *gcols : GroupCols2();
   for (int e = 0; e < gcs.count; e++) PO_TRY(gcol_check(&gcs.g[e], n, "k_solve2_dots"));
   for (int e = 0; e < gcs.count; e++) count_bytes(c, 1.0, gcs.g[e].nwcon);
@@ -2026,7 +2032,7 @@
     PO_TRY(collapse_range(c, 0, coef, P, 0, nv, n, &w));
     return k_step_check(c, b, rx, px, pzl, pzu, &one, &w, 1, diag, beta_mu, n, out);
   }
-  count_bytes(c, nv + 9, n);
+  count_bytes(c, nv + 9 - uniform_bound_streams(b), n);
   const int grid = grid_for(c, n, kBpcPanel);
   PO_TRY(ensure_partials(c, (size_t)grid * 3));
   PtrTable pt;
@@ -2044,7 +2050,7 @@
     PO_TRY(collapse_range(c, 0, coef, P, 0, nv, n, &w));
     return k_res_step(c, b, rx, px, pzl, pzu, dinv, &one, &w, 1, diag, beta_mu, n, tprime);
   }
-  count_bytes(c, nv + 10 + (dinv ? 1 : 0), n);
+  count_bytes(c, nv + 10 + (dinv ? 1 : 0) - uniform_bound_streams(b), n);
   if (n <= 0) return PO_OK;
   PtrTable pt;
   CoefTable ct;
@@ -2085,7 +2091,7 @@
 }
 int k_comp_step(Ctx *c, const Bounds &b, const double *px, const double *pzl, const double *pzu,
                 double ax, double az, int64_t n, double out[2]) {
-  count_bytes(c, 8, n);
+  count_bytes(c, 8 - uniform_bound_streams(b), n);
   const int grid = grid_for(c, n);
   PO_TRY(ensure_partials(c, (size_t)grid * 2));
   PO_LAUNCH(comp_step_kernel, grid, b, px, pzl, pzu, ax, az, n, c->d_partials);
@@ -2126,7 +2132,7 @@
 }
 int k_merit0(Ctx *c, const Bounds &b, const double *px, double sx, const double *g, int64_t n,
              double out[6]) {
-  count_bytes(c, 7, n);
+  count_bytes(c, 7 - uniform_bound_streams(b), n);
   const int grid = grid_for(c, n);
   PO_TRY(ensure_partials(c, (size_t)grid * 6));
   PO_LAUNCH(merit0_kernel, grid, b, px, sx, g, n, c->d_partials);
@@ -2175,7 +2181,7 @@
 }
 int k_comp_merit(Ctx *c, const Bounds &b, const double *px, const double *pzl, const double *pzu, double ax,
                  double az, const double *g, int64_t n, double out[9]) {
-  count_bytes(c, 9, n);
+  count_bytes(c, 9 - uniform_bound_streams(b), n);
   const int grid = grid_for(c, n);
   PO_TRY(ensure_partials(c, (size_t)grid * 9));
   PO_LAUNCH(comp_merit_kernel, grid, b, px, pzl, pzu, ax, az, g, n, c->d_partials);
@@ -2255,7 +2261,7 @@
     set_error("k_solve2c: panel of %d vectors exceeds kMaxPanel=%d", nv, kMaxPanel);
     return PO_ERR_ARG;
   }
-  count_bytes(c, nv + 14 + (va ? 1 : 0), n);
+  count_bytes(c, nv + 14 + (va ? 1 : 0) - uniform_bound_streams(b), n);
   const int grid = grid_for(c, n);
   PO_TRY(ensure_partials(c, (size_t)grid * 12));
   PtrTable pt;
@@ -2278,7 +2284,7 @@
   __shared__ double sm[4 * 2];
   double s[2] = {0.0, 0.0};
   PO_PAIR_LOOP(q, n) {
-    const double2 x = ld2(b.x, q, n), lb = ld2(b.lb, q, n), ub = ld2(b.ub, q, n), p = ld2(px, q, n);
+    const double2 x = ld2(b.x, q, n), lb = PO_LD2_LB(b, q, n), ub = PO_LD2_UB(b, q, n), p = ld2(px, q, n);
     const bool has2 = (2 * q + 1 < n);
     double2 v;
     v.x = clamp_elem(x.x + a * p.x, true, lb.x, true, ub.x, eps);
@@ -2296,7 +2302,7 @@
 }
 int k_trial(Ctx *c, const Bounds &b, const double *px, double a, double eps, int64_t n, double *xt,
             double out[2], double *sout) {
-  count_bytes(c, 5 + (sout ? 1 : 0), n);
+  count_bytes(c, 5 + (sout ? 1 : 0) - uniform_bound_streams(b), n);
   const int grid = grid_for(c, n);
   PO_TRY(ensure_partials(c, (size_t)grid * 2));
   PO_LAUNCH(trial_kernel, grid, b, px, a, eps, n, xt, sout, c->d_partials);
@@ -2386,7 +2392,7 @@
 }
 int k_form_pz(Ctx *c, const Bounds &b, const double *px, double beta_mu, int64_t n, double *pzl, double *pzu) {
   if (n <= 0) return PO_OK;
-  count_bytes(c, 8, n);
+  count_bytes(c, 8 - uniform_bound_streams(b), n);
   PO_LAUNCH(form_pz_kernel, grid_for(c, n), b, px, beta_mu, n, pzl, pzu);
   return PO_OK;
 }
@@ -2406,7 +2412,7 @@
   PO_PAIR_LOOP(q, n) {
     GRaw graw;
     if (gcol.w) graw = gcol_request(gcol, q, n);
-    const double2 _x = ld2(b.x, q, n), _lb = ld2(b.lb, q, n), _ub = ld2(b.ub, q, n);
+    const double2 _x = ld2(b.x, q, n), _lb = PO_LD2_LB(b, q, n), _ub = PO_LD2_UB(b, q, n);
     double2 lean_pl = make_double2(0.0, 0.0), lean_pu = lean_pl;
     if (pxs) {
       const double2 pv = ld2(pxs, q, n), xo = ld2(xold, q, n);
@@ -2528,7 +2534,7 @@
     return k_kkt_res_update(c, b, g, &w, &one, 1, beta_mu, n, rx, out, yqn, zl, pzl, zu, pzu, a, eps, va, az, acz, az_acz,
                             pxs, xold, beta_mu_step, beta_mu2, gcol, gcoef, dinv_out, t_out, spec_diag, spec_beta_mu);
   }
-  count_bytes(c, (yqn ? 14 : 11) + (acz ? (az_acz != 0.0 ? 2 : 1) : nc) + (dinv_out ? 2 : 0), n);
+  count_bytes(c, (yqn ? 14 : 11) + (acz ? (az_acz != 0.0 ? 2 : 1) : nc) + (dinv_out ? 2 : 0) - uniform_bound_streams(b), n);
   const int grid = grid_for(c, n, kBpcPanel);
   PO_TRY(ensure_partials(c, (size_t)grid * 13));
   PtrTable pt;
@@ -2559,18 +2565,27 @@
 }
 int k_affine_mult(Ctx *c, const Bounds &b, double *zl, const double *pzl, double *zu,
                   const double *pzu, double amin, int64_t n) {
-  count_bytes(c, 9, n);
+  count_bytes(c, 9 - uniform_bound_streams(b), n);
   if (n <= 0) return PO_OK;
   PO_LAUNCH(affine_mult_kernel, grid_for(c, n), b, zl, pzl, zu, pzu, amin, n);
   return PO_OK;
 }
 
+__device__ __forceinline__ void bits_minmax(double v, double *mn, double *mx) {
+  const unsigned long long u = (unsigned long long)__double_as_longlong(v);
+  const double hi = (double)(unsigned)(u >> 32), lo = (double)(unsigned)(u & 0xffffffffull);
+  mn[0] = fmin(mn[0], hi);
+  mn[1] = fmin(mn[1], lo);
+  mx[0] = fmax(mx[0], hi);
+  mx[1] = fmax(mx[1], lo);
+}
 __global__ void __launch_bounds__(kBlock)
     check_bounds_kernel(double *__restrict__ x, double *__restrict__ lb, double *__restrict__ ub,
                         double *__restrict__ zl, double *__restrict__ zu, double maxb,
                         double rel_bound, int both, int64_t n, double *__restrict__ partials) {
-  __shared__ double sm[4 * 3];
-  double flags[3] = {0.0, 0.0, 0.0};
+  __shared__ double sm[4 * 7];
+  double bmin[4] = {8589934592.0, 8589934592.0, 8589934592.0, 8589934592.0};
+  double flags[7] = {0.0, 0.0, 0.0, -1.0, -1.0, -1.0, -1.0};
   for (int64_t i = (int64_t)blockIdx.x * blockDim.x + threadIdx.x; i < n;
        i += (int64_t)gridDim.x * blockDim.x) {
     double xv = x[i], l = lb[i], u = ub[i];
@@ -2598,19 +2613,34 @@
     }
     if (l <= -maxb) zl[i] = 0.0;
     if (u >= maxb) zu[i] = 0.0;
-  }
-  block_reduce_store<3, OP_MAX>(flags, partials, 0, sm);
+    bits_minmax(l, &bmin[0], &flags[3]);
+    bits_minmax(u, &bmin[2], &flags[5]);
+  }
+  block_reduce_store<4, OP_MIN>(bmin, partials, 0, sm);
+  block_reduce_store<7, OP_MAX>(flags, partials, 4, sm);
 }
 int k_check_bounds(Ctx *c, double *x, double *lb, double *ub, double *zl, double *zu,
-                   double max_bound, double rel_bound, int both, int64_t n, int *flag) {
+                   double max_bound, double rel_bound, int both, int64_t n, int *flag, int uni[2],
+                   double val[2]) {
   count_bytes(c, 5, n);
   const int grid = grid_for(c, n);
-  PO_TRY(ensure_partials(c, (size_t)grid * 3));
+  PO_TRY(ensure_partials(c, (size_t)grid * 11));
   PO_LAUNCH(check_bounds_kernel, grid, x, lb, ub, zl, zu, max_bound, rel_bound, both, n,
             c->d_partials);
-  double out[3];
-  PO_TRY(reduce_finish(c, grid, 0, 0, 3, out, true));
-  *flag = (out[0] > 0.0 ? 1 : 0) | (out[1] > 0.0 ? 2 : 0) | (out[2] > 0.0 ? 4 : 0);
+  double out[11], mine[11];
+  PO_TRY(reduce_finish(c, grid, 0, 4, 7, out, true, mine));
+  *flag = (out[4] > 0.0 ? 1 : 0) | (out[5] > 0.0 ? 2 : 0) | (out[6] > 0.0 ? 4 : 0);
+  if (uni) {
+    for (int k = 0; k < 2; k++) {
+      const double *mn = mine + 2 * k, *mx = mine + 7 + 2 * k;
+      uni[k] = mn[0] == mx[0] && mn[1] == mx[1];
+      val[k] = 0.0;
+      if (uni[k]) {
+        const unsigned long long u = ((unsigned long long)(unsigned)mn[0] << 32) | (unsigned long long)(unsigned)mn[1];
+        memcpy(&val[k], &u, sizeof(double));
+      }
+    }
+  }
   return PO_OK;
 }
 
@@ -2820,7 +2850,7 @@
 }
 int k_d1s(Ctx *c, const Bounds &b, const double *bx, const double *dinv, double alpha, double beta_mu,
           int64_t n, double *t) {
-  count_bytes(c, 8, n);
+  count_bytes(c, 8 - uniform_bound_streams(b), n);
   if (n <= 0) return PO_OK;
   PO_LAUNCH(d1s_kernel, grid_for(c, n), b, bx, dinv, alpha, beta_mu, n, t);
   return PO_OK;
@@ -2866,7 +2896,7 @@
     PO_TRY(collapse_range(c, 0, coef, P, 0, nv, n, &w));
     return k_solve2s(c, b, t, dinv, &one, &w, 1, alpha, beta_mu, full, tau, n, px, pzl, pzu, out);
   }
-  count_bytes(c, nv + 10, n);
+  count_bytes(c, nv + 10 - uniform_bound_streams(b), n);
   if (nv > kMaxPanel) {
     set_error("panel of %d vectors exceeds kMaxPanel=%d", nv, kMaxPanel);
     return PO_ERR_ARG;
```

After: 44.74 (median of 6 runs). 1.02x the previous value.
